# MaxInGaussian/SCFGP

Measured on AMD Instinct MI355X. Metric: NLML+grad evals/sec, higher is better.
Workload: dtype f32

## Files before the change

### scfgp_amd/csrc/api_ctx.h

```cpp
#pragma once
#include "../../include/scfgp_hip.h"
#include "kernels.h"
#include "api_host.h"

#include <dlfcn.h>
#if __has_include(<rccl/rccl.h>)
#include <rccl/rccl.h>
#else
extern "C" {
typedef struct ncclComm* ncclComm_t;
typedef struct { char internal[128]; } ncclUniqueId;
typedef enum { ncclSuccess = 0 } ncclResult_t;
typedef enum { ncclFloat64 = 8 } ncclDataType_t;
typedef enum { ncclSum = 0 } ncclRedOp_t;
ncclResult_t ncclGetUniqueId(ncclUniqueId*);
ncclResult_t ncclCommInitRank(ncclComm_t*, int, ncclUniqueId, int);
ncclResult_t ncclAllReduce(const void*, void*, size_t, ncclDataType_t, ncclRedOp_t, ncclComm_t, hipStream_t);
ncclResult_t ncclCommDestroy(ncclComm_t);
const char* ncclGetErrorString(ncclResult_t);
}
#endif

#include <algorithm>
#include <cmath>
#include <cstdlib>
#include <cstring>
#include <string>
#include <vector>

#define HIPCHK(ctx, call)                                                                           \
    do {                                                                                            \
        hipError_t e_ = (call);                                                                     \
        if (e_ != hipSuccess) {                                                                     \
            (ctx)->err = std::string(#call) + ": " + hipGetErrorString(e_);                         \
            return SCFGP_EHIP;                                                                      \
        }                                                                                           \
    } while (0)

static constexpr int XT = 128;
static constexpr int64_t PRED_ROWS = 32768;
#ifndef SCFGP_COND_THRESHOLD
#define SCFGP_COND_THRESHOLD 10.0
#endif
#ifndef SCFGP_COND_THRESHOLD_W
#define SCFGP_COND_THRESHOLD_W 1000.0
#endif
#ifndef SCFGP_ERR_PER_COND
#define SCFGP_ERR_PER_COND 3.0e-7
#endif

struct Roctx {
    int (*push)(const char*) = nullptr; int (*pop)() = nullptr;
    Roctx() {
        void* h = dlopen("librocprofiler-sdk-roctx.so", RTLD_LAZY | RTLD_LOCAL);
        if (!h) h = dlopen("libroctx64.so", RTLD_LAZY | RTLD_LOCAL);
        if (!h) return;
        push = (int (*)(const char*))dlsym(h, "roctxRangePushA");
        pop = (int (*)())dlsym(h, "roctxRangePop");
        if (!push || !pop) { push = nullptr; pop = nullptr; }
    }
};
inline Roctx& roctx() { static Roctx r; return r; }

struct ProfRec { std::string name; hipEvent_t e0, e1; };

struct scfgp_ctx {
    Geom g{};
    int dtype = 0, device = 0;
    hipStream_t st = nullptr; bool own_stream = false;
    hipStream_t copy_st = nullptr; hipEvent_t ev_factor = nullptr;
    int lowrank_bwd = -1; int Spp = 0, Sq = 0; bool last_lrb = false;
    bool want_lrb() const {
        const bool fits = g.lowrank && g.Jp + (int)round_up(g.S, 64) <= g.Kp;
        return fits && (lowrank_bwd == 1 || (lowrank_bwd < 0 && g.Dp >= 4 * g.Sp));
    }
    double* x3_scalars() { return d_x3 + (int64_t)Dpp * g.Jp; }
    double* xs1() { return d_xp1 + n_pk + g.Kp; }
    double* xs2() { return d_xp2 + n_pk + g.Kp; }
    bool unsettled = false; int test_deny_level = 0, test_fail_stage = 0, test_pd_group = 0, test_sobol_group = 0;
    int cap() const { return esc_denied > 0 ? esc_denied - 1 : 2; }
    double* x3_xu() { return d_x3 + (int64_t)Dpp * g.Jp + 8; }
    hipEvent_t ev_fence = nullptr;
    ncclComm_t comm = nullptr; int comm_ranks = 0, comm_rank = 0;
    double* h_pin = nullptr;
    int64_t Ncap = 0, Nglobal = 0, Nglobal_full = 0;
    bool have_params = false, have_data = false;
    int stage = 0, last_want_grad = 0;
    std::vector<double> h_params;
    double *d_params = nullptr, *d_F = nullptr, *d_Fall = nullptr, *d_Lall = nullptr, *d_Rall = nullptr; Scal* d_sc = nullptr;
    double *d_Tt = nullptr, *p_Tt = nullptr;
    double *d_Xraw = nullptr, *d_yraw = nullptr; int64_t Nstore = 0, store_cap = 0; bool work_full = false;
    int64_t* d_idx = nullptr; int64_t idx_cap = 0;
    double *d_Xt = nullptr, *d_y = nullptr, *d_p = nullptr, *d_q = nullptr, *d_mu = nullptr, *d_vpart = nullptr;
    void *d_Phi = nullptr, *d_V = nullptr;
    bool split16 = false; unsigned* d_Phi16 = nullptr; char* d_B16 = nullptr; float* d_f16scale = nullptr;
    unsigned* d_V16g = nullptr; unsigned* d_qV16g = nullptr; double* d_f16side = nullptr; float* d_f16tmp = nullptr;
    int f16gram = 1;
    bool f16_on() const { return split16 && dma() == 2; }
    int64_t f16_chunk() const {
        const int64_t top = gram_chunk > 0 ? 2 * gram_chunk : 8192, fill = g.Np * F16x3Kernels::gram_tiles(g) / 512 / 512 * 512;
        return std::max<int64_t>(std::min(top, fill), 1024);
    }
    bool f16_gram() const { return f16_on() && f16gram && !last_cform; }
    F16Operands f16ops() const { return F16Operands{d_Phi16, d_B16, d_f16scale, nullptr, d_f16tmp + 5}; }
    double *d_xp1 = nullptr, *d_xp2 = nullptr; int64_t n_xp = 0, n_pk = 0;
    double *d_x1 = nullptr, *d_x2 = nullptr, *d_x3 = nullptr; int64_t n_x1 = 0, n_x2 = 0, n_x3 = 0; int Dpp = 0;
    double *d_Li = nullptr, *d_B = nullptr, *d_T1 = nullptr, *d_T2 = nullptr, *d_Abar = nullptr;
    void *d_BT = nullptr, *d_AbarT = nullptr;
    int apply_dma = -1;
    double *d_vecs = nullptr;
    double *d_scalars = nullptr, *d_yy = nullptr; int* d_flag = nullptr;
    float* d_ws2 = nullptr;
    double *d_slabs = nullptr; size_t slabs_bytes = 0;
    double *d_partial = nullptr; int64_t n_partial = 0;
    double *d_work = nullptr, *d_grad = nullptr;
    int xs_mode = 0; double* d_xscale = nullptr;
    int ys_mode = 0; double* d_yscale = nullptr;
    double *p_Xt = nullptr, *p_vpart = nullptr, *p_mupart = nullptr; void *p_Phi = nullptr;
    int64_t p_rows = 0;
    void *p_FT = nullptr, *p_C = nullptr, *p_V = nullptr, *p_Li = nullptr;
    double *u_Li = nullptr, *u_S = nullptr, *u_Lm = nullptr, *u_Mi = nullptr, *u_Si = nullptr, *u_vec = nullptr, *u_acc = nullptr, *u_part = nullptr;
    double *u_y = nullptr, *u_r = nullptr, *u_slabs = nullptr; size_t u_slabs_bytes = 0;
    void* u_LiT = nullptr; float* u_ws2 = nullptr; int* u_flag = nullptr;
    double *l_y = nullptr, *l_r = nullptr, *l_rec = nullptr, *l_out = nullptr, *l_acc = nullptr; unsigned long long* l_bad = nullptr;
    double *f_out = nullptr, *f_w = nullptr;
    int opt_algo = -1; OptHyper opt_h{}; double *d_opt = nullptr, *d_tctr = nullptr, *d_hist = nullptr; int hist_cap = 0;
    hipGraph_t graph = nullptr; hipGraphExec_t gexec = nullptr; int64_t graph_N = -1; bool in_train = false, warm = false;
    int use_graph = 1;
    int gram_nsplit = 0, gram_taper = 1, xtz_nsplit = 0; int64_t gram_chunk = 4096;
    RowSplits splits{};
    int gram64 = 2, esc_level = 0, esc_denied = 0; double esc_thr = SCFGP_COND_THRESHOLD, escw_thr = SCFGP_COND_THRESHOLD_W; bool last_used64 = false;
    int last_level = 0; bool cond_valid = false;
    double cond[3] = {0, 0, 0};
    void* d_Phi64 = nullptr; int64_t phi64_cap = 0; RowSplits splits64{};
    int factor_form = -1; bool last_cform = false; void* d_C = nullptr; int64_t c_cap = 0;
    bool want_cform() const { return factor_form == 1 || (factor_form < 0 && level() >= 2); }
    int level() const { return dtype != SCFGP_F32 || gram64 == 0 ? 0 : (gram64 == 1 ? 1 : (gram64 == 3 ? 2 : esc_level)); }
    bool use64() const { return level() >= 1; }
    double cond_est() const { return cond[1] * cond[2]; }
    double alpha_err_fp32() const { return SCFGP_ERR_PER_COND * cond_est(); }
    int want_level(double est, double slack) const { return est > escw_thr * slack ? 2 : (est > esc_thr * slack ? 1 : 0); }
    bool roctx_on = false;
    bool prof = false; std::vector<ProfRec> recs; std::vector<hipEvent_t> pool; size_t pool_used = 0;
    std::string err;

    double* beta() { return d_vecs; }
    double* alpha() { return d_vecs + g.Kp; }
    int dma() const {
        const int auto_dma = g.K > 256 && g.Np >= 16384 ? (dtype == SCFGP_F32 && g.K >= 1024 && g.Np >= 65536 ? 2 : 1) : 0;
        return apply_dma < 0 ? auto_dma : apply_dma;
    }
    double* u() { return d_vecs + 2 * g.Kp; }
    double* ut() { return d_vecs + 3 * g.Kp; }
    double* alpha_pred() { return d_vecs + 4 * g.Kp; }
    size_t tsize() const { return dtype == SCFGP_F32 ? 4 : 8; }
    KStage kstage() {
        KStage k; k.K = g.K; k.Kp = g.Kp; k.A = d_x1; k.Li = d_Li; k.B = d_B; k.T1 = d_T1; k.T2 = d_T2;
        k.g = d_x1 + (int64_t)g.Kp * g.Kp; k.beta = beta(); k.alpha = alpha(); k.h = d_x2 + (int64_t)g.Kp * g.Kp;
        k.u = u(); k.ut = ut(); k.scalars = d_scalars; k.flag = d_flag;
        return k;
    }
};

struct ProfScope {
    scfgp_ctx* c; size_t idx = (size_t)-1; bool ranged = false;
    ProfScope(scfgp_ctx* c_, const char* name) : c(c_) {
        if (g_scfgp_capturing) return;
        if (c->roctx_on && roctx().push) { roctx().push(name); ranged = true; }
        if (!c->prof) return;
        auto get = [&]() {
            if (c->pool_used == c->pool.size()) { hipEvent_t e; hipEventCreate(&e); c->pool.push_back(e); }
            return c->pool[c->pool_used++];
        };
        ProfRec r; r.name = name; r.e0 = get(); r.e1 = get();
        hipEventRecord(r.e0, c->st);
        c->recs.push_back(r); idx = c->recs.size() - 1;
    }
    ~ProfScope() {
        if (idx != (size_t)-1) hipEventRecord(c->recs[idx].e1, c->st);
        if (ranged) roctx().pop();
    }
};

template <typename P> static int dmalloc(scfgp_ctx* c, P** p, size_t bytes) {
    HIPCHK(c, hipMalloc((void**)p, bytes ? bytes : 16));
    return SCFGP_OK;
}
template <typename P> static void dfree(P*& p) { if (p) { hipFree((void*)p); p = nullptr; } }
struct DevTmp {
    double* p = nullptr;
    ~DevTmp() { if (p) hipFree(p); }
    operator double*() const { return p; }
};

#define DISPATCH_TO(I, c, fn, ...) ((c)->dtype == SCFGP_F32 ? I<float>::fn(__VA_ARGS__) : I<double>::fn(__VA_ARGS__))
```

### scfgp_amd/csrc/apply.hip

```cpp
#include "kernels.h"
#include "tile_cfgs.h"

#include <algorithm>

#ifdef SCFGP_TRACE
constexpr int ATRACE_CAP = 1 << 16;
__device__ unsigned long long g_atrace[5 * ATRACE_CAP][5];
int64_t apply_trace_read(void* host, int64_t max_bytes) {
    const int64_t n = max_bytes < (int64_t)sizeof(g_atrace) ? max_bytes : (int64_t)sizeof(g_atrace);
    return hipMemcpyFromSymbol(host, HIP_SYMBOL(g_atrace), n) == hipSuccess ? n : -2;
}
#else
int64_t apply_trace_read(void*, int64_t) { return -1; }
#endif
template <typename T, int TILE> struct ApplyCfg {
    typedef TileCfg<T, Tune<T>::APPLY_BM, TILE, SCFGP_BK, Tune<T>::APPLY_WGM, Tune<T>::apply_wgn(TILE), Tune<T>::MS,
                    SCFGP_BK == 16 && Tune<T>::MS == 16> type;
};

#include "apply_epilogue.h"

template <class Cfg, int EPI>
__device__ __forceinline__ void apply_tile(
    const typename Cfg::T* __restrict__ Phi, const typename Cfg::T* __restrict__ Bm, typename Cfg::T* V,
    double* __restrict__ vpart, const double* __restrict__ p, const double* __restrict__ q, const double* __restrict__ y,
    const double* __restrict__ alpha, const double* __restrict__ ut, int K, int Kp, int64_t Np, int njt,
    int col0, int jt0, double* __restrict__ mu, int ntot, int jt, int64_t rb, char* smem_raw) {
    typedef typename Cfg::T T;
    T* smem = reinterpret_cast<T*>(smem_raw);
    const int cbase = col0 + jt * Cfg::BN;
    const bool want_mu = (EPI == 0 || EPI == 2 || EPI == 3) && mu != nullptr;
    const int nkt_all = (K + Cfg::BK - 1) / Cfg::BK;
    const int nkt_tri = (cbase + Cfg::BN + Cfg::BK - 1) / Cfg::BK;
    const int kt0 = EPI == 4 ? cbase / Cfg::BK : 0;
    const int nkt = ((EPI == 2 || EPI == 3) && nkt_tri < nkt_all ? nkt_tri : nkt_all) - kt0;
    typename Cfg::MTr::acc_t acc[Cfg::TM][Cfg::TN];
    acc_zero<Cfg>(acc);
    TrLoader<T, T, Cfg::BM, Cfg::BK, Cfg::LDA, Cfg::THREADS, EPI != 1 && EPI != 4, Cfg::SWZA> la(
        Phi + rb * Cfg::BM * Kp + kt0 * Cfg::BK, Kp, threadIdx.x, want_mu ? alpha : nullptr, jt0 + jt, ntot);
    if (EPI == 2 || EPI == 3) la.dot_range(cbase / Cfg::BK, nkt);
    else if (ntot == 0) {
        const int hi = (cbase + Cfg::BN) / Cfg::BK;
        la.dot_range(cbase / Cfg::BK, hi < nkt ? hi : nkt);
    }
    NatLoader<T, T, Cfg::BN, Cfg::BK, Cfg::LDB, Cfg::THREADS, false, false> lb(Bm + (int64_t)kt0 * Cfg::BK * Kp + cbase, Kp, threadIdx.x);
    tile_mainloop<Cfg>(la, lb, nkt, acc, smem);
    if constexpr (EPI != 1 && EPI != 4) { if (want_mu) la.dot_reduce(mu + (int64_t)(jt0 + jt) * Np + rb * Cfg::BM); }
    apply_epilogue<Cfg, EPI>(acc, Phi, V, vpart, p, q, y, alpha, ut, K, Kp, Np, rb, cbase, jt0 + jt, smem_raw);
}

template <class Cfg, int EPI>
__global__ __launch_bounds__(Cfg::THREADS) __attribute__((amdgpu_waves_per_eu(1, 8)))
void apply_kernel(
    const typename Cfg::T* __restrict__ Phi, const typename Cfg::T* __restrict__ Bm, typename Cfg::T* V,
    double* __restrict__ vpart, const double* __restrict__ p, const double* __restrict__ q, const double* __restrict__ y,
    const double* __restrict__ alpha, const double* __restrict__ ut, int K, int Kp, int64_t Np, int njt,
    int col0, int jt0, double* __restrict__ mu, int ntot) {
    SMEM_DECL;
    const unsigned wid = xcd_remap(blockIdx.x, gridDim.x);
    if constexpr (EPI == 3 || EPI == 4) {
        const int np = (njt + 1) / 2, t = (int)(wid % np), o = njt - 1 - t;
        const int64_t rb = wid / np;
        apply_tile<Cfg, EPI>(Phi, Bm, V, vpart, p, q, y, alpha, ut, K, Kp, Np, njt, col0, jt0, mu, ntot, t, rb, smem_raw);
        if (o != t) {
            __syncthreads();
            apply_tile<Cfg, EPI>(Phi, Bm, V, vpart, p, q, y, alpha, ut, K, Kp, Np, njt, col0, jt0, mu, ntot, o, rb, smem_raw);
        }
    } else
        apply_tile<Cfg, EPI>(Phi, Bm, V, vpart, p, q, y, alpha, ut, K, Kp, Np, njt, col0, jt0, mu, ntot, (int)(wid % njt), wid / njt, smem_raw);
}

typedef __attribute__((address_space(3))) void lds_void;
typedef const __attribute__((address_space(1))) void gbl_void;
template <typename T, int BN_>
struct ApplyDma {
    static constexpr int ES = (int)sizeof(T), BM = 256, BN = BN_, ROWB = 16 * ES, CPR = ROWB / 16;
    static constexpr int WN = ES == 4 ? 64 : 32;
    static constexpr int WAVES = 4 * (BN / WN), STAGE = (BM + BN) * ROWB, STAGES = 3, LDS_BYTES = STAGES * STAGE,
                         DMA_PER_WAVE = STAGE / 1024 / WAVES, ROWS_PER_DMA = 1024 / ROWB;
    static constexpr int PRE = 2;
    static constexpr int WAVES_PER_EU = WAVES == 4 ? 2 : 4;
    typedef TileCfg<T, BM, BN, 16, 4, BN / WN, 16, true> Cfg;
    static_assert(STAGE / 1024 % WAVES == 0 && LDS_BYTES <= 160 * 1024, "whole DMA instructions per wave; the ring fits the LDS");
    static __device__ __forceinline__ int swz(int x) {
        if constexpr (ES == 4) return (0x78 >> (2 * ((x >> 2) & 3))) & 3;
        else return (int)((0x6BEB08u >> (3 * ((x >> 1) & 7))) & 7);
    }
};
static_assert(((0x6BEB08u >> 0) & 7) == 0 && ((0x6BEB08u >> 3) & 7) == 1 && ((0x6BEB08u >> 6) & 7) == 4 && ((0x6BEB08u >> 9) & 7) == 5 &&
              ((0x6BEB08u >> 12) & 7) == 6 && ((0x6BEB08u >> 15) & 7) == 7 && ((0x6BEB08u >> 18) & 7) == 2 && ((0x6BEB08u >> 21) & 7) == 3,
              "fp64 swizzle table");

template <typename T, int EPI, int BN>
__global__ __launch_bounds__((64 * ApplyDma<T, BN>::WAVES)) __attribute__((amdgpu_waves_per_eu(ApplyDma<T, BN>::WAVES_PER_EU, ApplyDma<T, BN>::WAVES_PER_EU)))
void apply_dma_kernel(const T* __restrict__ Phi, const T* __restrict__ Bm, T* V,
                      double* __restrict__ vpart, const double* __restrict__ p, const double* __restrict__ q,
                      const double* __restrict__ y, const double* __restrict__ alpha, const double* __restrict__ ut,
                      int K, int Kp, int64_t Np, int njt, double* __restrict__ mu, int col0, int slot0, int64_t rb0) {
    typedef ApplyDma<T, BN> D;
    typedef typename D::Cfg Cfg;
    typedef T half_t __attribute__((ext_vector_type(2)));
    typedef std::integral_constant<int, 0> H0;
    typedef std::integral_constant<int, 1> H1;
    constexpr int DPW = D::DMA_PER_WAVE, NRD = Cfg::TM + Cfg::TN, NM = 2 * Cfg::TM * Cfg::TN, PRE = D::PRE;
    static_assert(Cfg::TM == 4 && (Cfg::TN == 4 || Cfg::TN == 2), "fragment lists of the wait statements");
    static_assert(PRE + DPW + NRD <= NM, "one fetch or read per MFMA behind the barrier");
    SMEM_DECL;
    char* smem = smem_raw;
#ifdef SCFGP_TRACE
    const unsigned long long tr_t0 = __builtin_amdgcn_s_memrealtime();
#endif
    const unsigned wid = xcd_remap(blockIdx.x, gridDim.x);
    const int jt = EPI == 3 || EPI == 4 ? (int)((wid % njt + wid / njt) % njt) : (int)(wid % njt);
    const int64_t rb = rb0 + wid / njt;
    const int cbase = col0 + jt * D::BN;
    const int lane = threadIdx.x & 63, wave = __builtin_amdgcn_readfirstlane(threadIdx.x >> 6);
    const char* src[DPW]; unsigned loff[DPW]; int dst[DPW];
#pragma unroll
    for (int u = 0; u < DPW; ++u) {
        const int t = wave * DPW + u, x0 = D::ROWS_PER_DMA * t, l = lane / D::CPR, c = (lane % D::CPR) ^ D::swz(x0 + l);
        const int xb = x0 - D::BM, xcol = (xb & ~(D::WN - 1)) + Cfg::TN * (xb & 15) + ((xb >> 4) & (Cfg::TN - 1));
        const T* rowp = x0 < D::BM ? Phi + (rb * D::BM + x0) * Kp : Bm + (int64_t)(cbase + xcol) * Kp;
        src[u] = reinterpret_cast<const char*>(rowp) + (EPI == 4 ? (cbase / 16) * D::ROWB : 0);
        loff[u] = (unsigned)((x0 < D::BM ? l : Cfg::TN * l) * Kp * D::ES + c * 16);
        dst[u] = t * 1024;
    }
    const auto fetch_one = [&](auto uc, int slot) {
        constexpr int u = decltype(uc)::value;
        __builtin_amdgcn_global_load_lds((gbl_void*)(src[u] + loff[u]), (lds_void*)(smem + slot * D::STAGE + dst[u]), 16, 0, 0);
        src[u] += D::ROWB;
    };
    const int i = lane & 15, qg = lane >> 4;
    const int wm0 = (wave / Cfg::WGN) * Cfg::WM, wn0 = (wave % Cfg::WGN) * Cfg::WN;
    const int hoff0 = sizeof(T) == 4 ? (((qg >> 1) ^ D::swz(i)) << 4) + 8 * (qg & 1) : ((2 * qg) ^ D::swz(i)) << 4;
    const int hoff1 = sizeof(T) == 4 ? (((2 + (qg >> 1)) ^ D::swz(i)) << 4) + 8 * (qg & 1) : ((2 * qg + 1) ^ D::swz(i)) << 4;
    const int ring = (int)(uintptr_t)smem, aoff = ring + (wm0 + i) * D::ROWB, boff = ring + D::BM * D::ROWB + (wn0 + i) * D::ROWB;
    const int ra[2] = {aoff + hoff0, aoff + hoff1}, rbb[2] = {boff + hoff0, boff + hoff1};
    half_t ha[2][Cfg::TM], hb[2][Cfg::TN];
    typename Cfg::MTr::acc_t acc[Cfg::TM][Cfg::TN];
    acc_zero<Cfg>(acc);
    const int nst_all = (K + 15) / 16, nst_tri = (cbase + D::BN + 15) / 16;
    const int nst = (EPI == 3 && nst_tri < nst_all ? nst_tri : nst_all) - (EPI == 4 ? cbase / 16 : 0);
#define SCFGP_LDS_READ(dst, addr, off)                                                                              \
    do {                                                                                                             \
        if constexpr (sizeof(T) == 4) asm volatile("ds_read_b64 %0, %1 offset:%2" : "=v"(dst) : "v"(addr), "n"(off));   \
        else asm volatile("ds_read_b128 %0, %1 offset:%2" : "=v"(dst) : "v"(addr), "n"(off));                           \
    } while (0)
    const auto read_one = [&](auto hc, auto rc, int stage) {
        constexpr int h = decltype(hc)::value, R = decltype(rc)::value;
        if constexpr (R < Cfg::TM) SCFGP_LDS_READ(ha[h][R], stage + ra[h], R * 16 * D::ROWB);
        else SCFGP_LDS_READ(hb[h][R - Cfg::TM], stage + rbb[h], (R - Cfg::TM) * 16 * D::ROWB);
    };
#undef SCFGP_LDS_READ
#define SCFGP_WAIT_FRAGS(what, h)                                                                                                   \
    do {                                                                                                                            \
        if constexpr (Cfg::TN == 4)                                                                                                 \
            asm volatile("s_waitcnt " what : "+v"(ha[h][0]), "+v"(ha[h][1]), "+v"(ha[h][2]), "+v"(ha[h][3]),                        \
                                             "+v"(hb[h][0]), "+v"(hb[h][1]), "+v"(hb[h][2]), "+v"(hb[h][3]) :: "memory");           \
        else                                                                                                                        \
            asm volatile("s_waitcnt " what : "+v"(ha[h][0]), "+v"(ha[h][1]), "+v"(ha[h][2]), "+v"(ha[h][3]),                        \
                                             "+v"(hb[h][0]), "+v"(hb[h][1]) :: "memory");                                           \
    } while (0)
    const auto mfma_one = [&](auto hc, auto ic) {
        constexpr int h = decltype(hc)::value, I = decltype(ic)::value, j = I / (Cfg::TM * Cfg::TN), tm = I / Cfg::TN % Cfg::TM, tn = I % Cfg::TN;
        Cfg::MTr::mfma(acc[tm][tn], ha[h][tm][j], hb[h][tn][j]);
        __builtin_amdgcn_sched_barrier(0);
    };
    const auto second_half_pre = [&]() { static_for<PRE>([&](auto ic) { mfma_one(H1(), ic); }); };
    const auto second_half = [&](auto fc, int fslot, int next) {
        static_for<NM - PRE>([&](auto ic) {
            constexpr int I = decltype(ic)::value;
            mfma_one(H1(), std::integral_constant<int, I + PRE>());
            if constexpr (I < DPW) {
                if constexpr (decltype(fc)::value) { fetch_one(ic, fslot); __builtin_amdgcn_sched_barrier(0); }
            } else if constexpr (I - DPW < NRD) {
                read_one(H0(), std::integral_constant<int, I - DPW>(), next);
                __builtin_amdgcn_sched_barrier(0);
            }
        });
    };
    const auto first_half = [&](int next) {
        static_for<NM>([&](auto ic) {
            mfma_one(H0(), ic);
            if constexpr (decltype(ic)::value < NRD) { read_one(H1(), ic, next); __builtin_amdgcn_sched_barrier(0); }
        });
    };
    static_for<DPW>([&](auto uc) { fetch_one(uc, 0); });
    if (nst > 1) static_for<DPW>([&](auto uc) { fetch_one(uc, 1); });
    if (nst > 2) static_for<DPW>([&](auto uc) { fetch_one(uc, 2); });
    if (nst > 2) asm volatile("s_waitcnt vmcnt(%0)" :: "n"(2 * DPW) : "memory");
    else if (nst > 1) asm volatile("s_waitcnt vmcnt(%0)" :: "n"(DPW) : "memory");
    else asm volatile("s_waitcnt vmcnt(0)" ::: "memory");
    __builtin_amdgcn_s_barrier();
    asm volatile("" ::: "memory");
#ifdef SCFGP_TRACE
    const unsigned long long tr_l0 = __builtin_amdgcn_s_memrealtime();
#endif
    static_for<NRD>([&](auto rc) { read_one(H0(), rc, 0); });
    static_for<NRD>([&](auto rc) { read_one(H1(), rc, 0); });
    SCFGP_WAIT_FRAGS("lgkmcnt(0)", 0);
    __builtin_amdgcn_sched_barrier(0);
    static_for<NM>([&](auto ic) { mfma_one(H0(), ic); });
    int slot = 0, s = 0;
    for (; s + 3 < nst; ++s) {
        asm volatile("s_waitcnt vmcnt(%0)" :: "n"(DPW) : "memory");
        SCFGP_WAIT_FRAGS("lgkmcnt(0)", 1);
        __builtin_amdgcn_sched_barrier(0);
        second_half_pre();
        __builtin_amdgcn_s_barrier();
        asm volatile("" ::: "memory");
        const int fslot = slot;
        slot = slot == 2 ? 0 : slot + 1;
        __builtin_amdgcn_sched_barrier(0);
        second_half(std::true_type(), fslot, slot * D::STAGE);
        SCFGP_WAIT_FRAGS("lgkmcnt(0)", 0);
        __builtin_amdgcn_sched_barrier(0);
        first_half(slot * D::STAGE);
    }
    SCFGP_WAIT_FRAGS("lgkmcnt(0)", 1);
    for (; s + 1 < nst; ++s) {
        if (s + 2 < nst) asm volatile("s_waitcnt vmcnt(%0)" :: "n"(DPW) : "memory");
        else asm volatile("s_waitcnt vmcnt(0)" ::: "memory");
        SCFGP_WAIT_FRAGS("lgkmcnt(0)", 1);
        __builtin_amdgcn_sched_barrier(0);
        second_half_pre();
        __builtin_amdgcn_s_barrier();
        asm volatile("" ::: "memory");
        slot = slot == 2 ? 0 : slot + 1;
        __builtin_amdgcn_sched_barrier(0);
        second_half(std::false_type(), 0, slot * D::STAGE);
        SCFGP_WAIT_FRAGS("lgkmcnt(0)", 0);
        __builtin_amdgcn_sched_barrier(0);
        first_half(slot * D::STAGE);
    }
    SCFGP_WAIT_FRAGS("lgkmcnt(0)", 1);
    __builtin_amdgcn_sched_barrier(0);
    static_for<NM>([&](auto ic) { mfma_one(H1(), ic); });
#undef SCFGP_WAIT_FRAGS
    __syncthreads();
#ifdef SCFGP_TRACE
    const unsigned long long tr_l1 = __builtin_amdgcn_s_memrealtime();
#endif
    constexpr int SLOTS = BN >= 128 ? BN / 128 : 1;
    const int vslot = slot0 + SLOTS * jt;
    int tid = (int)threadIdx.x;
    asm volatile("" : "+v"(tid));
    apply_epilogue<Cfg, EPI, EPI == 0 || EPI == 3, true>(acc, Phi, V, vpart, p, q, y, alpha, ut, K, Kp, Np, rb, cbase, vslot, smem_raw, mu, tid);
    if (SLOTS == 2 && (EPI == 0 || EPI == 3) && tid < D::BM) {
        vpart[(int64_t)(vslot + 1) * Np + rb * D::BM + tid] = 0.0;
        if (mu) mu[(int64_t)(vslot + 1) * Np + rb * D::BM + tid] = 0.0;
    }
#ifdef SCFGP_TRACE
    __syncthreads();
    if (threadIdx.x == 0 && blockIdx.x < ATRACE_CAP) {
        unsigned long long* rec = g_atrace[EPI * ATRACE_CAP + blockIdx.x];
        rec[0] = tr_t0; rec[1] = __builtin_amdgcn_s_memrealtime();
        rec[2] = ((unsigned long long)__builtin_amdgcn_s_getreg((20 << 0) | (0 << 6) | (3 << 11)) & 0xF) | ((unsigned long long)jt << 8) |
                                  ((unsigned long long)nst << 20);
        rec[3] = tr_l0; rec[4] = tr_l1;
    }
#endif
}

template <typename T> struct ApplyPlan {
    static constexpr int NW = 2;
    int width[NW], count[NW], col0[NW], jt0[NW], total;
    explicit ApplyPlan(int K) {
        const int w[NW] = {128, 64};
        int col = 0, jt = 0;
        const bool small = K <= 256;
        for (int i = 0; i < NW; ++i) {
            width[i] = w[i];
            const bool last = i == NW - 1;
            count[i] = small && !last ? 0 : (last ? (K - col + w[i] - 1) / w[i] : (K - col) / w[i]);
            col0[i] = col; jt0[i] = jt;
            col += count[i] * w[i]; jt += count[i];
        }
        total = jt;
    }
};
bool F16x3Kernels::apply_runs(const Geom& g) { return ApplyPlan<float>(g.K).count[0] > 0; }
template <class Cfg, int EPI, typename T>
static int apply_launch_cfg(const Geom& g, int njt, int col0, int jt0, const T* Phi, const T* Bm, T* V, double* vpart,
                            const double* p, const double* q, const double* y, const double* alpha, const double* ut,
                            double* mu, int ntot, hipStream_t st) {
    if (njt <= 0) return 0;
    const int64_t nrb = g.Np / Cfg::BM;
    const int wgs_per_rb = EPI == 3 || EPI == 4 ? (njt + 1) / 2 : njt;
    allow_big_lds(apply_kernel<Cfg, EPI>, Cfg::LDS_BYTES);
    hipLaunchKernelGGL((apply_kernel<Cfg, EPI>), dim3((unsigned)(wgs_per_rb * nrb)), dim3(Cfg::THREADS), Cfg::LDS_BYTES, st,
                       Phi, Bm, V, vpart, p, q, y, alpha, ut, g.K, g.Kp, g.Np, njt, col0, jt0, mu, ntot);
    return (int)(njt * nrb);
}
template <typename T, int EPI, int BN>
static int apply_dma_launch(const Geom& g, int njt, int col0, int slot0, const T* Phi, const T* Bm, T* V, double* vpart,
                            const double* p, const double* q, const double* y, const double* alpha, const double* ut,
                            double* mu, hipStream_t st, int64_t rb0 = 0, int64_t nrb = -1) {
    typedef ApplyDma<T, BN> D;
    if (nrb < 0) nrb = g.Np / D::BM;
    if (njt <= 0 || nrb <= 0) return 0;
    allow_big_lds(apply_dma_kernel<T, EPI, BN>, D::LDS_BYTES);
    hipLaunchKernelGGL((apply_dma_kernel<T, EPI, BN>), dim3((unsigned)(njt * nrb)), dim3(64 * D::WAVES), D::LDS_BYTES, st,
                       Phi, Bm, V, vpart, p, q, y, alpha, ut, g.K, g.Kp, g.Np, njt, mu, col0, slot0, rb0);
    return (int)(njt * nrb);
}
static int apply_num_cus() {
    static int n = 0;
    if (n == 0) {
        int dev = 0; hipDeviceProp_t prop;
        if (hipGetDevice(&dev) == hipSuccess && hipGetDeviceProperties(&prop, dev) == hipSuccess) n = prop.multiProcessorCount;
        if (n <= 0) n = 256;
    }
    return n;
}
template <typename T, int EPI>
static int apply_launch(const Geom& g, const T* Phi, const T* Bm, T* V, double* vpart, const double* p, const double* q,
                        const double* y, const double* alpha, const double* ut, double* mu, hipStream_t st,
                        int dma = 0, const T* BmT = nullptr, const F16Operands* f16 = nullptr) {
    if (!BmT) BmT = Bm;
    const ApplyPlan<T> pl(g.K);
    int nb = 0;
    if constexpr (EPI != 2) {
        if (dma && pl.count[0] > 0) {
            int n256 = 0;
            const int64_t nrb = g.Np / 256;
            int64_t tail_rb = 0;
            if constexpr (sizeof(T) == 4) {
                n256 = dma == 2 ? pl.count[0] / 2 : 0;
                if (n256 > 0 && EPI != 3 && EPI != 4) {
                    const int64_t ncu = apply_num_cus(), tiles = nrb * n256, rem = tiles % ncu;
                    if (tiles > ncu && rem > 0 && 20 * rem <= 9 * ncu) tail_rb = (rem + n256 - 1) / n256;
                }
                if (f16 && (EPI == 0 || EPI == 1)) {
                    constexpr int E = EPI == 1 ? 1 : 0;
                    nb += F16x3Kernels::apply<E, 256>(g, n256, 0, 0, Phi, *f16, V, vpart, p, q, y, alpha, ut, mu, st, 0, nrb - tail_rb);
                    nb += F16x3Kernels::apply<E, 128>(g, pl.count[0] - 2 * n256, 256 * n256, 2 * n256, Phi, *f16, V, vpart, p, q, y, alpha, ut, mu, st, 0, nrb - tail_rb);
                    nb += F16x3Kernels::apply<E, 64>(g, pl.count[1], pl.col0[1], pl.jt0[1], Phi, *f16, V, vpart, p, q, y, alpha, ut, mu, st, 0, nrb - tail_rb);
                    if (tail_rb > 0) {
                        nb += F16x3Kernels::apply<E, 128>(g, pl.count[0], 0, 0, Phi, *f16, V, vpart, p, q, y, alpha, ut, mu, st, nrb - tail_rb, tail_rb);
                        nb += F16x3Kernels::apply<E, 64>(g, pl.count[1], pl.col0[1], pl.jt0[1], Phi, *f16, V, vpart, p, q, y, alpha, ut, mu, st, nrb - tail_rb, tail_rb);
                    }
                    return nb;
                }
                nb += apply_dma_launch<T, EPI, 256>(g, n256, 0, 0, Phi, BmT, V, vpart, p, q, y, alpha, ut, mu, st, 0, nrb - tail_rb);
            }
            nb += apply_dma_launch<T, EPI, 128>(g, pl.count[0] - 2 * n256, 256 * n256, 2 * n256, Phi, BmT, V, vpart, p, q, y, alpha, ut, mu, st, 0, nrb - tail_rb);
            nb += apply_dma_launch<T, EPI, 64>(g, pl.count[1], pl.col0[1], pl.jt0[1], Phi, BmT, V, vpart, p, q, y, alpha, ut, mu, st, 0, nrb - tail_rb);
            if (tail_rb > 0) {
                nb += apply_dma_launch<T, EPI, 128>(g, pl.count[0], 0, 0, Phi, BmT, V, vpart, p, q, y, alpha, ut, mu, st, nrb - tail_rb, tail_rb);
                nb += apply_dma_launch<T, EPI, 64>(g, pl.count[1], pl.col0[1], pl.jt0[1], Phi, BmT, V, vpart, p, q, y, alpha, ut, mu, st, nrb - tail_rb, tail_rb);
            }
            return nb;
        }
    }
    nb += apply_launch_cfg<typename ApplyCfg<T, 128>::type, EPI, T>(g, pl.count[0], pl.col0[0], pl.jt0[0], Phi, Bm, V, vpart, p, q, y, alpha, ut, mu, pl.total, st);
    nb += apply_launch_cfg<typename ApplyCfg<T, 64>::type, EPI, T>(g, pl.count[1], pl.col0[1], pl.jt0[1], Phi, Bm, V, vpart, p, q, y, alpha, ut, mu, pl.total, st);
    return nb;
}

template <typename T>
void ApplyKernels<T>::apply_v(const Geom& g, const T* Phi, const T* Bm, T* V, double* vpart, const double* alpha, double* mu,
                              hipStream_t st, int dma, const F16Operands* f16) {
    apply_launch<T, 0>(g, Phi, Bm, V, vpart, nullptr, nullptr, nullptr, alpha, nullptr, mu, st, dma, nullptr, f16);
}
template <typename T>
void ApplyKernels<T>::apply_predict(const Geom& g, const T* Phi, const T* LiT, double* vpart, const double* alpha, double* mu,
                                    hipStream_t st) {
    apply_launch<T, 2>(g, Phi, LiT, (T*)nullptr, vpart, nullptr, nullptr, nullptr, alpha, nullptr, mu, st);
}
template <typename T>
void ApplyKernels<T>::apply_plain(const Geom& g, const T* A, const T* Bm, T* Out, int Kc, int ncols, hipStream_t st) {
    Geom gk = g; gk.K = Kc;
    apply_launch_cfg<typename ApplyCfg<T, 64>::type, 4, T>(gk, (ncols + 63) / 64, 0, 0, A, Bm, Out, nullptr, nullptr, nullptr, nullptr, nullptr,
                                                           nullptr, nullptr, ApplyPlan<T>(Kc).total, st);
}

template <typename T>
void ApplyKernels<T>::apply_c(const Geom& g, const T* Phi, const T* LiT, const T* Li, T* C, double* vpart, const double* alpha,
                              const double* beta, double* mu, hipStream_t st, int dma) {
    const bool by_dma = dma && ApplyPlan<T>(g.K).count[0] > 0;
    apply_launch<T, 3>(g, Phi, LiT, C, vpart, nullptr, nullptr, nullptr, by_dma ? beta : alpha, nullptr, mu, st, dma, Li);
}
template <typename T>
void ApplyKernels<T>::apply_vc(const Geom& g, const T* C, const T* Li, const T* LiT, T* V, hipStream_t st, int dma) {
    apply_launch<T, 4>(g, C, Li, V, nullptr, nullptr, nullptr, nullptr, nullptr, nullptr, nullptr, st, dma, LiT);
}
template <typename T>
void ApplyKernels<T>::apply_phibar(const Geom& g, const T* Phi, const T* Abar, T* V, const double* p, const double* q,
                                   const double* y, const double* alpha, const double* ut, hipStream_t st, int dma, const F16Operands* f16) {
    apply_launch<T, 1>(g, Phi, Abar, V, nullptr, p, q, y, alpha, ut, nullptr, st, dma, nullptr, f16);
}

template <typename T> static int apply_njt(const Geom& g) { return ApplyPlan<T>(g.K).total; }


template <int MODE>
__global__ __launch_bounds__(256) void rowstats_kernel(const double* __restrict__ mupart, const double* __restrict__ vpart, int njt,
                                                       const double* __restrict__ y, const Scal* __restrict__ sc,
                                                       double* __restrict__ o1, double* __restrict__ o2,
                                                       double* __restrict__ partial, int64_t N, int64_t Np) {
    __shared__ double red[4][256];
    const double kappa = sc->kappa;
    double t2 = 0, kb = 0, qv = 0, pm = 0;
    for (int64_t n = (int64_t)blockIdx.x * 256 + threadIdx.x; n < Np; n += (int64_t)gridDim.x * 256) {
        double v = 0, mu = 0;
        for (int t = 0; t < njt; ++t) { v += vpart[(int64_t)t * Np + n]; mu += mupart[(int64_t)t * Np + n]; }
        const double d = kappa * (v + 1.0);
        if (MODE == 0) {
            double pn = 0, qn = 0;
            if (n < N) {
                const double r = mu - y[n];
                const double rv = r * r + v;
                const double e = 1.0 / d - rv / (d * d);
                pn = 2.0 * r / d;
                qn = 1.0 / d + kappa * e;
                t2 += rv / d + log(2.0 * M_PI * d);
                kb += e * (v + 1.0);
                qv += qn * v; pm += pn * mu;
            }
            o1[n] = pn; o2[n] = qn;
        } else if (n < N) {
            o1[n] = mu; o2[n] = sqrt(d);
        }
    }
    if (MODE == 0) {
        red[0][threadIdx.x] = t2; red[1][threadIdx.x] = kb; red[2][threadIdx.x] = qv; red[3][threadIdx.x] = pm;
        __syncthreads();
        for (int w = 128; w >= 1; w >>= 1) {
            if ((int)threadIdx.x < w)
                for (int k = 0; k < 4; ++k) red[k][threadIdx.x] += red[k][threadIdx.x + w];
            __syncthreads();
        }
        if (threadIdx.x < 4) partial[blockIdx.x * 4 + threadIdx.x] = red[threadIdx.x][0];
    }
}

template <typename T>
void ApplyKernels<T>::rowstats(const Geom& g, const double* mupart, const double* vpart, const double* y,
                               const Scal* sc, double* p, double* q, double* partial, int nblocks, hipStream_t st) {
    hipLaunchKernelGGL((rowstats_kernel<0>), dim3(nblocks), dim3(256), 0, st, mupart, vpart, apply_njt<T>(g), y, sc, p, q,
                       partial, g.N, g.Np);
}

template <typename T>
void ApplyKernels<T>::rowpredict(const Geom& g, const double* mupart, const double* vpart, const Scal* sc, double* mu, double* sd,
                                 hipStream_t st) {
    const int nblocks = (int)((g.Np + 255) / 256 < 1024 ? (g.Np + 255) / 256 : 1024);
    hipLaunchKernelGGL((rowstats_kernel<1>), dim3(nblocks), dim3(256), 0, st, mupart, vpart, apply_njt<T>(g),
                       (const double*)nullptr, sc, mu, sd, (double*)nullptr, g.N, g.Np);
}
template <typename T> int ApplyKernels<T>::partials(const Geom& g) { return apply_njt<T>(g); }
__global__ __launch_bounds__(256) void rowresidual_kernel(const double* __restrict__ mupart, int njt, const double* __restrict__ y,
                                                          double* __restrict__ r, int64_t N, int64_t Np) {
    for (int64_t n = (int64_t)blockIdx.x * 256 + threadIdx.x; n < Np; n += (int64_t)gridDim.x * 256) {
        double mu = 0;
        for (int t = 0; t < njt; ++t) mu += mupart[(int64_t)t * Np + n];
        r[n] = n < N ? y[n] - mu : 0.0;
    }
}
template <typename T>
void ApplyKernels<T>::rowresidual(const Geom& g, const double* mupart, const double* y, double* r, hipStream_t st) {
    const int nblocks = (int)((g.Np + 255) / 256 < 1024 ? (g.Np + 255) / 256 : 1024);
    hipLaunchKernelGGL(rowresidual_kernel, dim3(nblocks), dim3(256), 0, st, mupart, apply_njt<T>(g), y, r, g.N, g.Np);
}
template struct ApplyKernels<double>;
template struct ApplyKernels<float>;

__global__ __launch_bounds__(256) void reduce_scalars_kernel(const double* __restrict__ partial, int nblocks, int width,
                                                             double* __restrict__ scalars, int slot0) {
    __shared__ double red[256];
    for (int k = 0; k < width; ++k) {
        double s = 0;
        for (int b = threadIdx.x; b < nblocks; b += 256) s += partial[(int64_t)b * width + k];
        red[threadIdx.x] = s;
        __syncthreads();
        for (int m = 128; m >= 1; m >>= 1) {
            if (threadIdx.x < m) red[threadIdx.x] += red[threadIdx.x + m];
            __syncthreads();
        }
        if (threadIdx.x == 0) scalars[slot0 + k] = red[0];
        __syncthreads();
    }
}
__global__ __launch_bounds__(256) void reduce_chunks_kernel(double* __restrict__ partial, int n, int chunk) {
    __shared__ double red[256];
    const int64_t b0 = (int64_t)blockIdx.x * chunk;
    const int len = b0 + chunk <= n ? chunk : (int)(n - b0);
    double s = 0;
    for (int b = threadIdx.x; b < len; b += 256) s += partial[b0 + b];
    red[threadIdx.x] = s;
    __syncthreads();
    for (int m = 128; m >= 1; m >>= 1) {
        if (threadIdx.x < m) red[threadIdx.x] += red[threadIdx.x + m];
        __syncthreads();
    }
    if (threadIdx.x == 0 && len > 0) partial[b0] = red[0];
}
__global__ __launch_bounds__(128) void reduce_strided_kernel(const double* __restrict__ partial, int nchunks, int chunk,
                                                             double* __restrict__ scalars, int slot0) {
    __shared__ double red[128];
    red[threadIdx.x] = (int)threadIdx.x < nchunks ? partial[(int64_t)threadIdx.x * chunk] : 0.0;
    __syncthreads();
    for (int m = 64; m >= 1; m >>= 1) {
        if ((int)threadIdx.x < m) red[threadIdx.x] += red[threadIdx.x + m];
        __syncthreads();
    }
    if (threadIdx.x == 0) scalars[slot0] = red[0];
}
void reduce_scalars(double* partial, int nblocks, int width, double* scalars, int slot0, hipStream_t st) {
    if (width == 1 && nblocks > 8192) {
        const int chunk = (nblocks + 127) / 128, nchunks = (nblocks + chunk - 1) / chunk;
        hipLaunchKernelGGL(reduce_chunks_kernel, dim3(nchunks), dim3(256), 0, st, partial, nblocks, chunk);
        hipLaunchKernelGGL(reduce_strided_kernel, dim3(1), dim3(128), 0, st, partial, nchunks, chunk, scalars, slot0);
        return;
    }
    hipLaunchKernelGGL(reduce_scalars_kernel, dim3(1), dim3(256), 0, st, partial, nblocks, width, scalars, slot0);
}

__global__ __launch_bounds__(256) void sumsq_kernel(const double* __restrict__ y, int64_t n, double* __restrict__ partial) {
    __shared__ double red[256];
    double s = 0;
    for (int64_t i = (int64_t)blockIdx.x * 256 + threadIdx.x; i < n; i += (int64_t)gridDim.x * 256) s += y[i] * y[i];
    red[threadIdx.x] = s;
    __syncthreads();
    for (int m = 128; m >= 1; m >>= 1) {
        if (threadIdx.x < m) red[threadIdx.x] += red[threadIdx.x + m];
        __syncthreads();
    }
    if (threadIdx.x == 0) partial[blockIdx.x] = red[0];
}
void sum_squares(const double* y, int64_t n, double* scalars, int slot, double* scratch, hipStream_t st) {
    const int nb = 256;
    hipLaunchKernelGGL(sumsq_kernel, dim3(nb), dim3(256), 0, st, y, n, scratch);
    reduce_scalars(scratch, nb, 1, scalars, slot, st);
}
```

### scfgp_amd/csrc/apply_epilogue.h

```cpp
#pragma once
#include "kernels.h"
#include "tile_cfgs.h"

template <int CTRL> __device__ __forceinline__ double dpp_mov_f64(double x) {
    int lo = __double2loint(x), hi = __double2hiint(x);
    lo = __builtin_amdgcn_update_dpp(0, lo, CTRL, 0xF, 0xF, true);
    hi = __builtin_amdgcn_update_dpp(0, hi, CTRL, 0xF, 0xF, true);
    return __hiloint2double(hi, lo);
}
__device__ __forceinline__ double row16_sum(double x) {
    x += dpp_mov_f64<0xB1>(x);
    x += dpp_mov_f64<0x4E>(x);
    x += dpp_mov_f64<0x141>(x);
    x += dpp_mov_f64<0x140>(x);
    return x;
}
template <class Cfg, int EPI, bool MU>
__device__ __forceinline__ void apply_epilogue_vec2(
    const typename Cfg::MTr::acc_t (&acc)[Cfg::TM][Cfg::TN], const double* __restrict__ Phi, double* V,
    double* __restrict__ vpart, const double* __restrict__ p, const double* __restrict__ q, const double* __restrict__ y,
    const double* __restrict__ alpha, const double* __restrict__ ut, int K, int Kp, int64_t Np, int64_t rb, int cbase, int jtg,
    char* smem_raw, double* __restrict__ mupart, int tid) {
    static_assert(Cfg::TN == 2 && Cfg::MS == 16 && sizeof(typename Cfg::T) == 8 && (EPI == 0 || EPI == 1 || EPI == 3 || EPI == 4), "VEC2 layout");
    AccCoord<Cfg> co(tid);
    const int jg = cbase + co.wn0 + 2 * (co.lane & 15);
    if constexpr (EPI == 4) {
#pragma unroll
        for (int tm = 0; tm < Cfg::TM; ++tm)
#pragma unroll
            for (int r = 0; r < 4; ++r)
                *reinterpret_cast<v2d*>(V + (rb * Cfg::BM + co.row(tm, r)) * Kp + jg) = v2d{acc[tm][0][r], acc[tm][1][r]};
    } else if constexpr (EPI == 0 || EPI == 3) {
        double* red = reinterpret_cast<double*>(smem_raw);
        double* red2 = red + Cfg::WGN * Cfg::BM;
        const int wn = (tid >> 6) % Cfg::WGN;
        double al[2], live[2];
#pragma unroll
        for (int k = 0; k < 2; ++k) { live[k] = jg + k < K ? 1.0 : 0.0; al[k] = MU && jg + k < K ? alpha[jg + k] : 0.0; }
#pragma unroll
        for (int tm = 0; tm < Cfg::TM; ++tm) {
            v2d ph[4];
            int64_t off[4];
#pragma unroll
            for (int r = 0; r < 4; ++r) {
                off[r] = (rb * Cfg::BM + co.row(tm, r)) * Kp + jg;
                if (EPI == 0) ph[r] = *reinterpret_cast<const v2d*>(Phi + off[r]);
            }
#pragma unroll
            for (int r = 0; r < 4; ++r) {
                const int row = co.row(tm, r);
                const double c0 = acc[tm][0][r], c1 = acc[tm][1][r];
                *reinterpret_cast<v2d*>(V + off[r]) = v2d{c0, c1};
                double part, mup = 0;
                if (EPI == 3) part = fma(c0, c0, c1 * c1);
                else part = fma(ph[r][0] * live[0], c0, ph[r][1] * live[1] * c1);
                if (MU) mup = EPI == 3 ? fma(c0, al[0], c1 * al[1]) : fma(ph[r][0], al[0], ph[r][1] * al[1]);
                part = row16_sum(part);
                if ((co.lane & 15) == 0) red[wn * Cfg::BM + row] = part;
                if (MU) {
                    mup = row16_sum(mup);
                    if ((co.lane & 15) == 0) red2[wn * Cfg::BM + row] = mup;
                }
            }
        }
        __syncthreads();
        if (tid < Cfg::BM) {
            double s = 0, s2 = 0;
#pragma unroll
            for (int k = 0; k < Cfg::WGN; ++k) { s += red[k * Cfg::BM + tid]; if (MU) s2 += red2[k * Cfg::BM + tid]; }
            vpart[(int64_t)jtg * Np + rb * Cfg::BM + tid] = s;
            if (MU && mupart) mupart[(int64_t)jtg * Np + rb * Cfg::BM + tid] = s2;
        }
    } else {
        double al[2], u2[2];
#pragma unroll
        for (int k = 0; k < 2; ++k) { al[k] = alpha[jg + k]; u2[k] = ut[jg + k]; }
        double* rowsc = reinterpret_cast<double*>(smem_raw);
        for (int i = tid; i < Cfg::BM; i += Cfg::THREADS) {
            const int64_t n = rb * Cfg::BM + i;
            rowsc[3 * i] = 2.0 * q[n]; rowsc[3 * i + 1] = p[n]; rowsc[3 * i + 2] = y[n];
        }
        __syncthreads();
#pragma unroll
        for (int tm = 0; tm < Cfg::TM; ++tm) {
            v2d vv[4];
            int64_t off[4];
#pragma unroll
            for (int r = 0; r < 4; ++r) {
                off[r] = (rb * Cfg::BM + co.row(tm, r)) * Kp + jg;
                vv[r] = *reinterpret_cast<const v2d*>(V + off[r]);
            }
#pragma unroll
            for (int r = 0; r < 4; ++r) {
                const int row = co.row(tm, r);
                const double qn = rowsc[3 * row], pn = rowsc[3 * row + 1], yn = rowsc[3 * row + 2];
                v2d o;
#pragma unroll
                for (int k = 0; k < 2; ++k) o[k] = 2.0 * acc[tm][k][r] + qn * vv[r][k] + pn * al[k] + yn * u2[k];
                *reinterpret_cast<v2d*>(V + off[r]) = o;
            }
        }
    }
}
template <class Cfg, int EPI, bool MU = false, bool VEC4 = false>
__device__ __forceinline__ void apply_epilogue(
    const typename Cfg::MTr::acc_t (&acc)[Cfg::TM][Cfg::TN], const typename Cfg::T* __restrict__ Phi, typename Cfg::T* V,
    double* __restrict__ vpart, const double* __restrict__ p, const double* __restrict__ q, const double* __restrict__ y,
    const double* __restrict__ alpha, const double* __restrict__ ut, int K, int Kp, int64_t Np, int64_t rb, int cbase, int jtg,
    char* smem_raw, double* __restrict__ mupart = nullptr, int tid = (int)threadIdx.x) {
    typedef typename Cfg::T T;
    if constexpr (VEC4 && sizeof(T) == 8) {
        apply_epilogue_vec2<Cfg, EPI, MU>(acc, Phi, V, vpart, p, q, y, alpha, ut, K, Kp, Np, rb, cbase, jtg, smem_raw, mupart, tid);
        return;
    }
    AccCoord<Cfg> co(tid);
    if constexpr (VEC4 && sizeof(T) == 4) {
        static_assert(Cfg::TN == 4 && Cfg::MS == 16 && sizeof(T) == 4 && (EPI == 0 || EPI == 1 || EPI == 3 || EPI == 4), "VEC4 layout");
        const int c4 = co.wn0 + 4 * (co.lane & 15);
        const int jg = cbase + c4;
        if constexpr (EPI == 4) {
#pragma unroll
            for (int tm = 0; tm < Cfg::TM; ++tm)
#pragma unroll
                for (int r = 0; r < 4; ++r)
                    *reinterpret_cast<v4f*>(V + (rb * Cfg::BM + co.row(tm, r)) * Kp + jg) = v4f{acc[tm][0][r], acc[tm][1][r], acc[tm][2][r], acc[tm][3][r]};
        } else if constexpr (EPI == 0 || EPI == 3) {
            double* red = reinterpret_cast<double*>(smem_raw);
            double* red2 = red + Cfg::WGN * Cfg::BM;
            const int wn = (tid >> 6) % Cfg::WGN;
            double al[4], live[4];
#pragma unroll
            for (int k = 0; k < 4; ++k) { live[k] = jg + k < K ? 1.0 : 0.0; al[k] = MU && jg + k < K ? alpha[jg + k] : 0.0; }
#pragma unroll
            for (int tm = 0; tm < Cfg::TM; ++tm) {
                v4f ph[4];
                int64_t off[4];
#pragma unroll
                for (int r = 0; r < 4; ++r) {
                    off[r] = (rb * Cfg::BM + co.row(tm, r)) * Kp + jg;
                    if (EPI == 0) ph[r] = *reinterpret_cast<const v4f*>(Phi + off[r]);
                }
#pragma unroll
                for (int r = 0; r < 4; ++r) {
                    const int row = co.row(tm, r);
                    const v4f c = v4f{acc[tm][0][r], acc[tm][1][r], acc[tm][2][r], acc[tm][3][r]};
                    *reinterpret_cast<v4f*>(V + off[r]) = c;
                    double part = 0, mup = 0;
                    if (EPI == 3) {
                        part = (double)(c[0] * c[0]) + (double)(c[1] * c[1]) + (double)(c[2] * c[2]) + (double)(c[3] * c[3]);
                        if (MU) mup = (double)c[0] * al[0] + (double)c[1] * al[1] + (double)c[2] * al[2] + (double)c[3] * al[3];
                    } else {
#pragma unroll
                        for (int k = 0; k < 4; ++k) { part += (double)ph[r][k] * (double)c[k] * live[k]; if (MU) mup += (double)ph[r][k] * al[k]; }
                    }
                    part = row16_sum(part);
                    if ((co.lane & 15) == 0) red[wn * Cfg::BM + row] = part;
                    if (MU) {
                        mup = row16_sum(mup);
                        if ((co.lane & 15) == 0) red2[wn * Cfg::BM + row] = mup;
                    }
                }
            }
            __syncthreads();
            if (tid < Cfg::BM) {
                double s = 0, s2 = 0;
#pragma unroll
                for (int k = 0; k < Cfg::WGN; ++k) { s += red[k * Cfg::BM + tid]; if (MU) s2 += red2[k * Cfg::BM + tid]; }
                vpart[(int64_t)jtg * Np + rb * Cfg::BM + tid] = s;
                if (MU && mupart) mupart[(int64_t)jtg * Np + rb * Cfg::BM + tid] = s2;
            }
        } else {
            float alf[4], u4f[4];
#pragma unroll
            for (int k = 0; k < 4; ++k) { alf[k] = (float)alpha[jg + k]; u4f[k] = (float)ut[jg + k]; }
            float* rowsc = reinterpret_cast<float*>(smem_raw);
            for (int i = tid; i < Cfg::BM; i += Cfg::THREADS) {
                const int64_t n = rb * Cfg::BM + i;
                rowsc[3 * i] = (float)(2.0 * q[n]); rowsc[3 * i + 1] = (float)p[n]; rowsc[3 * i + 2] = (float)y[n];
            }
            __syncthreads();
#pragma unroll
            for (int tm = 0; tm < Cfg::TM; ++tm) {
                v4f vv[4];
                int64_t off[4];
#pragma unroll
                for (int r = 0; r < 4; ++r) {
                    off[r] = (rb * Cfg::BM + co.row(tm, r)) * Kp + jg;
                    vv[r] = *reinterpret_cast<const v4f*>(V + off[r]);
                }
#pragma unroll
                for (int r = 0; r < 4; ++r) {
                    const int row = co.row(tm, r);
                    const float qn = rowsc[3 * row], pn = rowsc[3 * row + 1], yn = rowsc[3 * row + 2];
                    v4f o;
#pragma unroll
                    for (int k = 0; k < 4; ++k) o[k] = fmaf(qn, vv[r][k], fmaf(pn, alf[k], fmaf(yn, u4f[k], 2.0f * acc[tm][k][r])));
                    *reinterpret_cast<v4f*>(V + off[r]) = o;
                }
            }
        }
        return;
    }
    if (EPI == 4) {
#pragma unroll
        for (int tm = 0; tm < Cfg::TM; ++tm)
#pragma unroll
            for (int r = 0; r < Cfg::MTr::NACC; ++r) {
                const int64_t off = (rb * Cfg::BM + co.row(tm, r)) * Kp + cbase;
#pragma unroll
                for (int tn = 0; tn < Cfg::TN; ++tn) V[off + co.col(tn)] = acc[tm][tn][r];
            }
    } else if (EPI == 0 || EPI == 2 || EPI == 3) {
        double* red = reinterpret_cast<double*>(smem_raw);
        double* red2 = red + Cfg::WGN * Cfg::BM;
        const int wn = (tid >> 6) % Cfg::WGN;
        double al[Cfg::TN];
        if (MU) {
#pragma unroll
            for (int tn = 0; tn < Cfg::TN; ++tn) al[tn] = cbase + co.col(tn) < K ? alpha[cbase + co.col(tn)] : 0.0;
        }
#pragma unroll
        for (int tm = 0; tm < Cfg::TM; ++tm)
#pragma unroll
            for (int r = 0; r < Cfg::MTr::NACC; ++r) {
                const int row = co.row(tm, r);
                const int64_t off = (rb * Cfg::BM + row) * Kp + cbase;
                double part = 0, mup = 0;
#pragma unroll
                for (int tn = 0; tn < Cfg::TN; ++tn) {
                    const T c = acc[tm][tn][r];
                    if (EPI != 2) V[off + co.col(tn)] = c;
                    if (EPI != 0) {
                        part += (double)c * (double)c;
                        if (MU && cbase + co.col(tn) < K) mup += (EPI == 3 ? (double)c : (double)Phi[off + co.col(tn)]) * al[tn];
                    } else if (cbase + co.col(tn) < K) {
                        const double ph = (double)Phi[off + co.col(tn)];
                        part += ph * (double)c;
                        if (MU) mup += ph * al[tn];
                    }
                }
                if constexpr (Cfg::MS == 16) part = row16_sum(part);
                else {
#pragma unroll
                    for (int m = 1; m < Cfg::MS; m <<= 1) part += __shfl_xor(part, m);
                }
                if ((co.lane % Cfg::MS) == 0) red[wn * Cfg::BM + row] = part;
                if (MU) {
                    if constexpr (Cfg::MS == 16) mup = row16_sum(mup);
                    else {
#pragma unroll
                        for (int m = 1; m < Cfg::MS; m <<= 1) mup += __shfl_xor(mup, m);
                    }
                    if ((co.lane % Cfg::MS) == 0) red2[wn * Cfg::BM + row] = mup;
                }
            }
        __syncthreads();
        if (tid < Cfg::BM) {
            double s = 0, s2 = 0;
#pragma unroll
            for (int k = 0; k < Cfg::WGN; ++k) { s += red[k * Cfg::BM + tid]; if (MU) s2 += red2[k * Cfg::BM + tid]; }
            vpart[(int64_t)jtg * Np + rb * Cfg::BM + tid] = s;
            if (MU && mupart) mupart[(int64_t)jtg * Np + rb * Cfg::BM + tid] = s2;
        }
    } else {
        [[maybe_unused]] float alf[Cfg::TN], utf[Cfg::TN];
        if constexpr (sizeof(T) == 4) {
#pragma unroll
            for (int tn = 0; tn < Cfg::TN; ++tn) { alf[tn] = (float)alpha[cbase + co.col(tn)]; utf[tn] = (float)ut[cbase + co.col(tn)]; }
        }
#pragma unroll
        for (int tm = 0; tm < Cfg::TM; ++tm)
#pragma unroll
            for (int r = 0; r < Cfg::MTr::NACC; ++r) {
                const int64_t n = rb * Cfg::BM + co.row(tm, r);
                const int64_t off = n * Kp + cbase;
                const double qn = 2.0 * q[n], pn = p[n], yn = y[n];
                if constexpr (sizeof(T) == 4) {
                    const float qf = (float)qn, pf = (float)pn, yf = (float)yn;
#pragma unroll
                    for (int tn = 0; tn < Cfg::TN; ++tn)
                        V[off + co.col(tn)] = fmaf(qf, V[off + co.col(tn)], fmaf(pf, alf[tn], fmaf(yf, utf[tn], 2.0f * acc[tm][tn][r])));
                } else {
#pragma unroll
                    for (int tn = 0; tn < Cfg::TN; ++tn) {
                        const int j = cbase + co.col(tn);
                        V[off + co.col(tn)] = (T)(2.0 * (double)acc[tm][tn][r] + qn * (double)V[off + co.col(tn)] + pn * alpha[j] + yn * ut[j]);
                    }
                }
            }
    }
}
```

### scfgp_amd/csrc/kernels.h

```cpp
#pragma once
#include "common.h"

struct Geom {
    int D, S, M, J, K, P;
    int Dp;
    int Jp;
    int Sp;
    int lowrank;
    int Kp;
    int tile;
    int gfull;
    int gstrip;
    int64_t N;
    int64_t Np;
};

struct RowSplits {
    int nsplit;
    int groups;
    int units;
    int taper;
    int gran;
    int64_t nrb;
    __host__ __device__ int per_group() const { return units + taper; }
    __host__ __device__ void range(int s, int64_t& r0, int64_t& r1) const {
        const int pg = per_group(), grp = s / pg, i = s % pg;
        const int64_t g0 = nrb * grp / groups, g1 = nrb * (grp + 1) / groups, len = g1 - g0;
        const int64_t den = (int64_t)1 << taper;
        const int k = i - (units - 1);
        int64_t e0, e1;
        if (taper == 0 || k < 0) { e0 = den * i; e1 = e0 + den; }
        else {
            const int64_t base = den * (units - 1);
            e0 = base + den - (den >> k);
            e1 = k == taper ? base + den : base + den - (den >> (k + 1));
        }
        r0 = (g0 + len * e0 / (den * units)) * gran;
        r1 = (g0 + len * e1 / (den * units)) * gran;
    }
};
RowSplits gram_row_splits(int jobs_per_split, int64_t Np, bool f32, int nsplit_override, int taper);

struct Projection { const double* Fall; const double* Lall; const double* Rall; double* Tt; };

template <typename T>
struct FmapKernels {
    static void featuremap(const Geom& g, const double* Xt, const Projection& pr, const Scal* sc, T* Phi, hipStream_t st);
    static void convert(const double* src, T* dst, int K, int Kp, hipStream_t st);
    static void convert_transposed(const double* src, T* dst, int K, int Kp, hipStream_t st);
};

template <typename T>
struct GramKernels {
    static void gram(const Geom& g, const T* Phi, const double* w, const double* side, const RowSplits& rs, int64_t chunk,
                     double* slabs, double* sidepart, int* qhead, float* ws2, hipStream_t st);
    static int gram_jobs(const Geom& g);
    static void xtz(const Geom& g, const double* Xt, const T* Phi, const T* Phibar, int nsplit, int64_t chunk, double* slabs,
                    hipStream_t st);
    static void zbar_inplace(const Geom& g, const T* Phi, T* Phibar, hipStream_t st);
    static void rsel(const Geom& g, const double* params, T* out, hipStream_t st);
    static void tn_plain(const double* A, int Dp, const T* Bm, int64_t ldb, int J, int64_t Np, int nsplit, int64_t chunk, double* slabs,
                         hipStream_t st);
};

struct F16Operands { const unsigned* Phi16; const char* B16; const float* scale; unsigned* V16; const float* vbound; };

template <typename T>
struct ApplyKernels {
    static void apply_v(const Geom& g, const T* Phi, const T* Bm, T* V, double* vpart, const double* alpha, double* mupart,
                        hipStream_t st, int dma = 0, const F16Operands* f16 = nullptr);
    static void apply_predict(const Geom& g, const T* Phi, const T* LiT, double* vpart, const double* alpha, double* mupart,
                              hipStream_t st);
    static void apply_c(const Geom& g, const T* Phi, const T* LiT, const T* Li, T* C, double* vpart, const double* alpha,
                        const double* beta, double* mupart, hipStream_t st, int dma = 0);
    static void apply_vc(const Geom& g, const T* C, const T* Li, const T* LiT, T* V, hipStream_t st, int dma = 0);
    static void apply_phibar(const Geom& g, const T* Phi, const T* Abar, T* V, const double* p, const double* q,
                             const double* y, const double* alpha, const double* ut, hipStream_t st, int dma = 0, const F16Operands* f16 = nullptr);
    static void apply_plain(const Geom& g, const T* A, const T* Bm, T* Out, int Kc, int ncols, hipStream_t st);
    static void rowstats(const Geom& g, const double* mupart, const double* vpart, const double* y,
                         const Scal* sc, double* p, double* q, double* partial, int nblocks, hipStream_t st);
    static void rowpredict(const Geom& g, const double* mupart, const double* vpart, const Scal* sc, double* mu, double* sd,
                           hipStream_t st);
    static void rowresidual(const Geom& g, const double* mupart, const double* y, double* r, hipStream_t st);
    static int partials(const Geom& g);
};

struct F16x3Kernels {
    static void split_operand(const Geom& g, const double* M, char* B16, float* scale, double* part, const Scal* sc, hipStream_t st);
    template <int EPI, int BN>
    static int apply(const Geom& g, int njt, int col0, int slot0, const float* Phi, const F16Operands& f, float* V,
                     double* vpart, const double* p, const double* q, const double* y, const double* alpha, const double* ut, double* mu,
                     hipStream_t st, int64_t rb0, int64_t nrb);
    static bool apply_runs(const Geom& g);
    static constexpr size_t F16_PAD = 1024;
    static int side_blocks(const Geom& g);
    static void split_phi(const Geom& g, const float* Phi, const double* y, const Scal* sc, unsigned* Phi16, double* sidepart, float* tmp,
                          hipStream_t st);
    static void v_bound(const Geom& g, const double* B, const Scal* sc, float* tmp, hipStream_t st);
    static void split_v(const Geom& g, const float* V, const double* q, const double* p, unsigned* V16g, unsigned* qV16g, double* sidepart,
                        float* tmp, hipStream_t st);
    static int gram_chunks(const Geom& g, int64_t chunk);
    static int gram_tiles(const Geom& g);
    static void gram(const Geom& g, const unsigned* A16g, const unsigned* B16g, const float* scale, int64_t chunk, double* slabs, hipStream_t st);
};

template <typename T> struct SweepKernels : FmapKernels<T>, GramKernels<T>, ApplyKernels<T> {};

int64_t trace_read(void* host, int64_t max_bytes);
int64_t apply_trace_read(void* host, int64_t max_bytes);
int64_t chol_trace_read(void* host, int64_t max_bytes);

void reduce_tri_tiles(const double* slabs, int nsplit, int nts, int tile, double* packed, hipStream_t st);
void unpack_tri_tiles(const double* packed, int nts, int tile, double* full, int64_t ld, hipStream_t st);
void reduce_full_tiles(const double* slabs, int nsplit, int ntm, int ntn, double* out, int64_t ldo, hipStream_t st);
void reduce_side(const double* sidepart, int nsplit, int Kp, int ncov, double* vec, hipStream_t st);
void reduce_scalars(double* partial, int nblocks, int width, double* scalars, int slot0, hipStream_t st);
void sum_squares(const double* y, int64_t n, double* scalars, int slot, double* scratch, hipStream_t st);

void unpack_params(const Geom& g, const double* params, double* F, double* Fall, double* Lall, double* Rall, Scal* sc, hipStream_t st);
void grad_epilogue(const Geom& g, const double* params, const double* F, const double* XZ, int64_t ldxz,
                   double* work, double* scalars, int64_t Nglobal, double* grad, hipStream_t st,
                   const double* TZ = nullptr, int64_t ldtz = 0, const double* XU = nullptr, int64_t ldxu = 0);
void finalize_cost(const Geom& g, const Scal* sc, double* scalars, const double* yy, const double* t2kb,
                   int64_t Nglobal, double* grad, int want_grad, hipStream_t st);
void write_status(double* xs, double ran1, double cap1, double cap2, double fail, hipStream_t st);
void pack_data(const Geom& g, const double* Xraw, const double* yraw, const int64_t* idx, double* Xt, double* y, hipStream_t st,
               int mode = 0, const double* sp = nullptr);
void pad_square(const double* src, int K, int Kp, double* dst, hipStream_t st);

constexpr int YPOST_BLOCKS = 64;
void ypost_mean(const double* ys, int64_t n, double* out, hipStream_t st);
void ypost_chunk(double* mu, double* sd, const double* ys, int64_t n, int mode, const double* sp, const double* ymean,
                 double* part, hipStream_t st);
void ypost_metrics(const double* part, int nparts, int64_t n, double* out, hipStream_t st);

int predgrad_ft_cols(int D);
template <typename T> void predgrad_operand(const Geom& g, const double* Fall, T* FT, hipStream_t st);
template <typename T>
void predgrad(const Geom& g, const T* Phi, const T* V, const double* alpha, const T* FT, const double* sd, const Scal* sc, double* dmu,
              double* dstd, hipStream_t st);
void xgrad_chunk(const double* Xraw, int64_t n, int D, int mode, const double* sp, double* dmu, double* dstd, hipStream_t st);
void ygrad_chunk(const double* mu, const double* sd, int64_t n, int D, int mode, const double* sp, double* dmu, double* dstd, hipStream_t st);

inline int64_t sample_w_rows(int K) { return round_up(K, 64); }
inline int sample_w_cols(int nsamp) { return (int)round_up(nsamp, 64); }
template <typename T>
void sample_weights(const Geom& g, const double* Li, const double* alpha, const Scal* sc, int nsamp, uint64_t seed, double* Z, double* W,
                    T* Wt, hipStream_t st);
template <typename T>
void sample_product(const Geom& g, const T* Phi, const T* Wt, int nsamp, int64_t t0, uint64_t seed, int noise, int ymode, const double* ysp,
                    const Scal* sc, double* out, hipStream_t st);
constexpr int sample_block_rows(size_t tsize) { return tsize == 4 ? 128 : 64; }
inline int64_t sample_blocks(int64_t Np, size_t tsize) { return Np / sample_block_rows(tsize); }
struct SampleArgmaxBufs { double* pv; long long* pt; double* bestv; long long* bestt; int* flag; };
template <typename T>
void sample_argmax_product(const Geom& g, const T* Phi, const T* Wt, int nsamp, const double* w, int minimize, int64_t t0, int first,
                           const SampleArgmaxBufs& b, hipStream_t st);
void sample_argmax_finalize(double* bestv, int nsamp, int ymode, const double* ysp, const Scal* sc, hipStream_t st);

struct AcquireSpec { int kind; double par[2]; const double* fstar; int nstar; int noise; int minimize; };
inline int64_t acquire_blocks(int64_t Np) { return Np / 256; }
struct AcquireBufs { double* mu; double* sd; double* acq; double* au; double* as; double* pv; long long* pt; double* bestv; long long* bestt; int* flag; };
void acquire_rows(const Geom& g, int njt, const double* mupart, const double* vpart, const Scal* sc, const AcquireSpec& a, const AcquireBufs& b,
                  hipStream_t st);
void acquire_argmax(const Geom& g, const double* w, int64_t t0, int first, const AcquireBufs& b, hipStream_t st);
void acquire_grad(const Geom& g, const AcquireBufs& b, int minimize, const double* dsd, double* grad, hipStream_t st);

struct KgBufs { double *d, *zf, *sd, *st_m, *st_s, *st_b, *kg, *kg_hi, *m, *s; };
int64_t kg_state_rows();
void kg_reference(int njt, const double* mupart, int64_t Np, int64_t R, int minimize, const double* z, int J, double* d, double* zf, int* flag,
                  hipStream_t st);
void kg_sigma(const Geom& g, int njt, const double* vpart, const Scal* sc, int noise, double* sd, hipStream_t st);
template <typename T>
void kg_nodes(const Geom& g, const T* Ca, const T* Cb, int64_t R, int J, const KgBufs& b, const Scal* sc, hipStream_t st);

int samplegrad_w_ld(int K);
void samplegrad_weights(const double* W, int K, int nsamp, double* WT, hipStream_t st);
template <typename T>
void samplegrad(const Geom& g, const T* Phi, const double* WT, const double* sidx, int64_t t0, int nsamp, const T* FT, double* val,
                double* grad, hipStream_t st);

template <typename T>
void predcov(const Geom& g, const T* Ca, const T* Cb, int64_t nrows, int64_t Tb, int64_t row_base, int noise, const Scal* sc, double* out,
             hipStream_t st);

struct OptHyper { double lr, b1, b2, eps, momentum; };
void opt_update(int algo, const OptHyper& h, int P, double* theta, const double* grad, double* st, double* tctr,
                const double* scalars, double* hist, int hist_cap, hipStream_t stream);

struct KStage {
    int K, Kp;
    double *A;
    double *Li;
    double *B;
    double *T1, *T2;
    double *g, *beta, *alpha, *h, *u, *ut;
    double *scalars; int* flag;
};
void kstage_factor(const KStage& k, const double* packed, const Scal* sc, hipStream_t st);
void kstage_adjoint(const KStage& k, const double* BWB, double* Abar, const Scal* sc, hipStream_t st);
void kstage_adjoint_factor_form(const KStage& k, double* McBWB, double* Abar, const Scal* sc, hipStream_t st);
void kstage_bbar(const KStage& k, const double* packed, const double* Abar, double* part, hipStream_t st);

struct KUpdate {
    int K, Kp;
    const double* packed;
    int64_t n_pk;
    const double* Li;
    const double* alpha;
    double *S;
    double *Lm, *Mi, *Si;
    double *gamma, *alpha_out, *part;
    int* flag;
};
void kstage_update(const KUpdate& k, hipStream_t st);
void kstage_downdate(const KUpdate& k, const double* rr, double n, const Scal* sc, double* out, hipStream_t st);
void update_sumsq(const double* r, int64_t n, double* acc, hipStream_t st);
void forget_stats(const double* mu, const double* sd, const double* y, int64_t n, int64_t ldr, double* rec, double* acc, hipStream_t st);
void update_load_factor(const double* Li_host_layout, int K, int Kp, double* Li, hipStream_t st);
void update_store_factor(const double* Li, int K, int Kp, double* Li_host_layout, hipStream_t st);
void update_check_finite(const double* x, int64_t n, int* flag, hipStream_t st);
void update_accumulate(double* acc, const double* part, int64_t n, hipStream_t st);

template <typename T>
void loo_blocks(const Geom& g, const T* C, const double* r, const double* y, int block, int64_t blk0, const Scal* sc, double* mu,
                double* sd, double* lev, double* rec, double* acc, unsigned long long* bad, hipStream_t st);

template <typename T> void gradcov_operand(const Geom& g, const double* params, const double* Fall, T* Qt, hipStream_t st);
template <typename T> void gradfeat(const Geom& gr, const Geom& g, const T* Phi, const T* Qt, T* Psi, hipStream_t st);
void gradcov_ones(double* x, int64_t n, hipStream_t st);
template <typename T>
void gradcov_blocks(const Geom& gr, const Geom& g, const T* C, const double* params, const Scal* sc, const double* gfac, const double* m,
                    const double* wgt, double* dvar, double* dcov, double* rec, hipStream_t st);
void gradcov_reduce(const double* rec, int64_t n, int D, double* acc, hipStream_t st);

struct GradObs { const int* dims; int nd; const double *gfac, *y, *G, *rho; };
template <typename T>
void gradobs_rows(const Geom& gr, const Geom& g, const T* Phi, const double* Fall, const GradObs& a, T* Psi, double* tg, hipStream_t st);

constexpr int SOBOL_T = 8;
constexpr int SOBOL_COLS = 32;
constexpr int SOBOL_GROUP = 16;
void sobol_tables(const Geom& g, const double* Fall, const Scal* sc, const double* meas, int Jt, double* psi1, double* Ed, double* E,
                  double* Eb, double* phibar, hipStream_t st);
void sobol_weights(const Geom& g, const double* W, const Scal* sc, const double* E, int Jt, int nw, double* A, double* f0, hipStream_t st);
void sobol_pairs(const Geom& g, const double* Fall, const double* meas, const double* psi1, const double* Ed, const double* E,
                 const double* Eb, const double* A, const int* units, int nunits, int Jt, int nw, int w0, int ncols, int G, int flags,
                 double* rec, hipStream_t st);
void sobol_reduce(const double* rec, int nunits, int D, int ncols, int nw, int w0, int flags, double* sums, hipStream_t st);

inline int pd_grid_rows(int G) { return (int)round_up(G, 128); }
int64_t pd_record_len(const Geom& g, int ng);
template <typename T>
void pd_sums(const Geom& g, const double* Xt, const double* Fall, const Scal* sc, const double* wgt, const int* dims, int ng, double* rec,
             double* acc, hipStream_t st);
void pd_grid(double* grid, const int* dims, int ndim, int G, int D, int mode, const double* sp, hipStream_t st);
template <typename T>
void pd_mean_rows(const Geom& gr, const Geom& g, const double* acc, double W, const double* Fall, const int* dims, const double* grid, int ng,
                  int G, T* Phibar, hipStream_t st);
template <typename T>
void pd_ice_weights(const Geom& g, const double* alpha, const double* Fall, int d, const double* grid_d, int G, T* R, hipStream_t st);
void pd_column(const Geom& g, double* Xt, int d, int save, double* keep, hipStream_t st);

struct SelectBufs {
    int Kp; int64_t Trows;
    double *w, *d, *pval; long long* pidx;
    double *U, *cp, *a, *part;
    long long* idx; double *var, *gain; int* flag;
};
int select_partials(int64_t Trows);
void select_ones(double* w, int64_t Trows, hipStream_t st);
template <typename T> void select_init(const SelectBufs& b, const T* C, hipStream_t st);
template <typename T> void select_step(const SelectBufs& b, const T* C, int j, const Scal* sc, hipStream_t st);
void select_std(const SelectBufs& b, const Scal* sc, double* sd, hipStream_t st);

struct SelectIvBufs {
    const double* Q;
    double *a, *apart, *h, *v, *red, *ivar;
};
int select_iv_tiles(int Kp);
template <typename T>
void select_iv_init(const SelectBufs& b, const SelectIvBufs& iv, const T* C, const T* Qt, int K, const Scal* sc, hipStream_t st);
template <typename T> void select_iv_step(const SelectBufs& b, const SelectIvBufs& iv, const T* C, int j, const Scal* sc, hipStream_t st);

struct SelectQeiBufs {
    const double* F; int64_t T; int nsamp; double sgn;
    double *w, *ms, *score0, *pval; long long* pidx;
    long long* idx; double *gain, *qei; int* flag;
};
int selectqei_blocks(int64_t T);
void selectqei_state(const SelectQeiBufs& b, const double* pend, double base, int start, hipStream_t st);
void selectqei_sweep(const SelectQeiBufs& b, int j, hipStream_t st);
void selectqei_commit(const SelectQeiBufs& b, int j, hipStream_t st);
```

### scfgp_amd/csrc/scfgp_api.hip

```cpp
#include "api_ctx.h"

static void derive_geom(Geom& g, int D, int S, int M);

thread_local bool g_scfgp_capturing = false;

struct Rccl {
    void* h = nullptr;
    decltype(&ncclGetUniqueId) get_id = nullptr; decltype(&ncclCommInitRank) init_rank = nullptr;
    decltype(&ncclAllReduce) all_reduce = nullptr; decltype(&ncclCommDestroy) destroy = nullptr;
    decltype(&ncclGetErrorString) err_string = nullptr;
    bool resolved = false;
    bool bind(void* from) {
        get_id = (decltype(get_id))dlsym(from, "ncclGetUniqueId"); init_rank = (decltype(init_rank))dlsym(from, "ncclCommInitRank");
        all_reduce = (decltype(all_reduce))dlsym(from, "ncclAllReduce"); destroy = (decltype(destroy))dlsym(from, "ncclCommDestroy");
        err_string = (decltype(err_string))dlsym(from, "ncclGetErrorString");
        return get_id && init_rank && all_reduce && destroy && err_string;
    }
    Rccl() {
        if (dlsym(RTLD_DEFAULT, "ncclAllReduce") && bind(RTLD_DEFAULT)) { resolved = true; return; }
        const char* names[] = {"librccl.so", "librccl.so.1", "/opt/rocm/lib/librccl.so.1"};
        for (const char* n : names) if (!h) h = dlopen(n, RTLD_NOW | RTLD_NOLOAD | RTLD_LOCAL);
        for (const char* n : names) if (!h) h = dlopen(n, RTLD_NOW | RTLD_LOCAL);
        if (!h) return;
        if (bind(h)) resolved = true;
        else { dlclose(h); h = nullptr; }
    }
    bool ok() const { return resolved; }
};
static Rccl& rccl() { static Rccl r; return r; }

static int xtz_split(int ntiles, int64_t Np) {
    int64_t s = std::max(1, 512 / ntiles);
    int64_t smax = std::max<int64_t>(Np / 2048, 1);
    if (ntiles * smax < 256) smax = std::max<int64_t>(Np / 64, 1);
    if (s > smax) s = smax;
    if (s < 1) s = 1;
    return (int)s;
}

static void free_rows(scfgp_ctx* c) {
    dfree(c->d_Xt); dfree(c->d_y); dfree(c->d_p); dfree(c->d_q); dfree(c->d_ws2); dfree(c->d_mu); dfree(c->d_vpart); dfree(c->d_Tt);
    dfree(c->d_Phi); dfree(c->d_V); dfree(c->d_Phi16); dfree(c->d_V16g); dfree(c->d_qV16g); dfree(c->d_f16side); dfree(c->d_slabs);
    c->Ncap = 0; c->slabs_bytes = 0;
}

static int ensure_aux_rows(scfgp_ctx* c) {
    const Geom& g = c->g;
    if (c->use64() && c->phi64_cap < g.Np) {
        dfree(c->d_Phi64); c->phi64_cap = 0;
        if (int rc = dmalloc(c, &c->d_Phi64, sizeof(double) * g.Np * g.Kp)) return rc;
        HIPCHK(c, hipMemsetAsync(c->d_Phi64, 0, sizeof(double) * g.Np * g.Kp, c->st));
        c->phi64_cap = g.Np;
    }
    if (c->want_cform() && c->c_cap < g.Np) {
        dfree(c->d_C); c->c_cap = 0;
        if (int rc = dmalloc(c, &c->d_C, c->tsize() * g.Np * g.Kp)) return rc;
        HIPCHK(c, hipMemsetAsync(c->d_C, 0, c->tsize() * g.Np * g.Kp, c->st));
        c->c_cap = g.Np;
    }
    return SCFGP_OK;
}

static int ensure_rows(scfgp_ctx* c, int64_t N) {
    Geom& g = c->g;
    if (c->gexec) { hipGraphExecDestroy(c->gexec); c->gexec = nullptr; }
    if (c->graph) { hipGraphDestroy(c->graph); c->graph = nullptr; }
    const int64_t Np = round_up(N > 0 ? N : 1, 256);
    g.N = N; g.Np = Np;
    const int nts = g.Kp / g.tile, ntiles = nts * (nts + 1) / 2;
    const int ntx = ((g.Dp + XT - 1) / XT) * (g.Jp / XT);
    const int gjobs = c->dtype == SCFGP_F32 ? SweepKernels<float>::gram_jobs(g) : SweepKernels<double>::gram_jobs(g);
    c->splits = gram_row_splits(gjobs, Np, c->dtype == SCFGP_F32, c->gram_nsplit, c->gram_taper);
    int gs = c->splits.nsplit;
    if (c->dtype == SCFGP_F32 && c->gram64 != 0) {
        c->splits64 = gram_row_splits(SweepKernels<double>::gram_jobs(g), Np, false, c->gram_nsplit, c->gram_taper);
        gs = std::max(gs, c->splits64.nsplit);
    }
    const int xs = c->xtz_nsplit > 0 ? (int)std::min<int64_t>(c->xtz_nsplit, Np / 64) : xtz_split(ntx, Np);
    const int nt1 = (c->Spp / XT) * (g.Jp / XT), nt2 = (c->Dpp / XT) * (c->Sq / XT);
    const size_t lrb = std::max<size_t>((size_t)xtz_split(nt1, Np) * nt1, (size_t)xtz_split(nt2, Np) * nt2);
    if (c->split16) gs = std::max(gs, F16x3Kernels::gram_chunks(g, c->f16_chunk()));
    const size_t need = sizeof(double) * std::max<size_t>((size_t)gs * ntiles * g.tile * g.tile + (size_t)gs * g.Kp,
                                                          std::max<size_t>((size_t)xs * ntx, lrb) * XT * XT);
    if (need > c->slabs_bytes) {
        dfree(c->d_slabs);
        if (int rc = dmalloc(c, &c->d_slabs, need)) return rc;
        c->slabs_bytes = need;
    }
    if (int rc = ensure_aux_rows(c)) return rc;
    if (Np <= c->Ncap) return SCFGP_OK;
    dfree(c->d_Xt); dfree(c->d_y); dfree(c->d_p); dfree(c->d_q); dfree(c->d_ws2); dfree(c->d_mu); dfree(c->d_vpart); dfree(c->d_Tt);
    dfree(c->d_Phi); dfree(c->d_V); dfree(c->d_Phi16); dfree(c->d_V16g); dfree(c->d_qV16g); dfree(c->d_f16side);
    c->Ncap = 0;
    const size_t ts = c->tsize();
    int rc;
    if ((rc = dmalloc(c, &c->d_Xt, sizeof(double) * Np * g.Dp))) return rc;
    if (g.lowrank && (rc = dmalloc(c, &c->d_Tt, sizeof(double) * Np * g.Sp))) return rc;
    if ((rc = dmalloc(c, &c->d_y, sizeof(double) * Np))) return rc;
    if ((rc = dmalloc(c, &c->d_p, sizeof(double) * Np))) return rc;
    if ((rc = dmalloc(c, &c->d_q, sizeof(double) * Np))) return rc;
    if (c->dtype == SCFGP_F32 && (rc = dmalloc(c, &c->d_ws2, sizeof(float) * 2 * (Np + 32)))) return rc;
    if ((rc = dmalloc(c, &c->d_mu, sizeof(double) * Np * (g.Kp / 64)))) return rc;
    if ((rc = dmalloc(c, &c->d_vpart, sizeof(double) * Np * (g.Kp / 64)))) return rc;
    if ((rc = dmalloc(c, &c->d_Phi, ts * Np * g.Kp))) return rc;
    if ((rc = dmalloc(c, &c->d_V, ts * Np * g.Kp))) return rc;
    if (c->split16) {
        const size_t plane = sizeof(unsigned) * Np * g.Kp + F16x3Kernels::F16_PAD;
        if ((rc = dmalloc(c, &c->d_Phi16, plane)) || (rc = dmalloc(c, &c->d_V16g, plane)) || (rc = dmalloc(c, &c->d_qV16g, plane))) return rc;
        if ((rc = dmalloc(c, &c->d_f16side, sizeof(double) * F16x3Kernels::side_blocks(g) * g.Kp))) return rc;
        HIPCHK(c, hipMemsetAsync(c->d_Phi16, 0, plane, c->st));
        HIPCHK(c, hipMemsetAsync(c->d_V16g, 0, plane, c->st));
        HIPCHK(c, hipMemsetAsync(c->d_qV16g, 0, plane, c->st));
    }
    HIPCHK(c, hipMemsetAsync(c->d_Phi, 0, ts * Np * g.Kp, c->st));
    HIPCHK(c, hipMemsetAsync(c->d_V, 0, ts * Np * g.Kp, c->st));
    c->Ncap = Np;
    return SCFGP_OK;
}

extern "C" int scfgp_create(scfgp_ctx** out, int D, int S, int M, int dtype, int device, void* stream) {
    if (!out || D < 1 || S < 1 || M < 1 || (dtype != SCFGP_F64 && dtype != SCFGP_F32 && dtype != SCFGP_F16X3)) return SCFGP_EARG;
    scfgp_ctx* c = new scfgp_ctx();
    *out = c;
    c->split16 = dtype == SCFGP_F16X3;
    if (c->split16) dtype = SCFGP_F32;
    c->dtype = dtype; c->device = device;
    Geom& g = c->g;
    derive_geom(g, D, S, M);
    if (const char* e = getenv("SCFGP_LOWRANK")) g.lowrank = atoi(e) != 0;
    if (const char* e = getenv("SCFGP_ROCTX")) c->roctx_on = atoi(e) != 0;
    c->Dpp = (int)round_up(g.Dp, XT);
    HIPCHK(c, hipSetDevice(device));
    if (stream) c->st = (hipStream_t)stream;
    else { HIPCHK(c, hipStreamCreate(&c->st)); c->own_stream = true; }
    HIPCHK(c, hipStreamCreateWithFlags(&c->copy_st, hipStreamNonBlocking));
    HIPCHK(c, hipEventCreateWithFlags(&c->ev_factor, hipEventDisableTiming));
    HIPCHK(c, hipEventCreateWithFlags(&c->ev_fence, hipEventDisableTiming));
    const int64_t Kp = g.Kp, K2 = Kp * Kp;
    c->Spp = (int)round_up(g.Sp, XT); c->Sq = (int)round_up(g.S, XT);
    c->n_x1 = K2 + Kp + 8; c->n_x2 = K2 + Kp + 8; c->n_x3 = (int64_t)std::max(c->Dpp, c->Spp) * g.Jp + 8 + (int64_t)c->Dpp * c->Sq;
    { const int64_t nts = Kp / g.tile; c->n_pk = nts * (nts + 1) / 2 * g.tile * g.tile; c->n_xp = c->n_pk + Kp + 8; }
    int rc;
    if ((rc = dmalloc(c, &c->d_params, sizeof(double) * g.P))) return rc;
    if ((rc = dmalloc(c, &c->d_F, sizeof(double) * D * M))) return rc;
    if ((rc = dmalloc(c, &c->d_Fall, sizeof(double) * g.Dp * g.Jp))) return rc;
    if ((rc = dmalloc(c, &c->d_Lall, sizeof(double) * g.Dp * round_up(g.Sp, 64)))) return rc;
    if ((rc = dmalloc(c, &c->d_Rall, sizeof(double) * g.Sp * g.Jp))) return rc;
    if ((rc = dmalloc(c, &c->d_sc, sizeof(Scal)))) return rc;
    if ((rc = dmalloc(c, &c->d_xp1, sizeof(double) * c->n_xp))) return rc;
    if ((rc = dmalloc(c, &c->d_xp2, sizeof(double) * c->n_xp))) return rc;
    HIPCHK(c, hipMemsetAsync(c->d_xp1, 0, sizeof(double) * c->n_xp, c->st));
    HIPCHK(c, hipMemsetAsync(c->d_xp2, 0, sizeof(double) * c->n_xp, c->st));
    if ((rc = dmalloc(c, &c->d_x1, sizeof(double) * c->n_x1))) return rc;
    if ((rc = dmalloc(c, &c->d_x2, sizeof(double) * c->n_x2))) return rc;
    if ((rc = dmalloc(c, &c->d_x3, sizeof(double) * c->n_x3))) return rc;
    if ((rc = dmalloc(c, &c->d_Li, sizeof(double) * K2))) return rc;
    if ((rc = dmalloc(c, &c->d_B, sizeof(double) * K2))) return rc;
    if ((rc = dmalloc(c, &c->d_T1, sizeof(double) * K2))) return rc;
    if ((rc = dmalloc(c, &c->d_T2, sizeof(double) * K2))) return rc;
    if ((rc = dmalloc(c, &c->d_Abar, sizeof(double) * K2))) return rc;
    if ((rc = dmalloc(c, &c->d_BT, c->tsize() * K2))) return rc;
    if ((rc = dmalloc(c, &c->d_AbarT, c->tsize() * K2))) return rc;
    if (c->split16) {
        if ((rc = dmalloc(c, &c->d_B16, 4 * (size_t)K2))) return rc;
        if ((rc = dmalloc(c, &c->d_f16scale, sizeof(float) * 4))) return rc;
        if ((rc = dmalloc(c, &c->d_f16tmp, sizeof(float) * 8))) return rc;
    }
    if ((rc = dmalloc(c, &c->d_vecs, sizeof(double) * 5 * Kp))) return rc;
    if ((rc = dmalloc(c, &c->d_scalars, sizeof(double) * 32))) return rc;
    if ((rc = dmalloc(c, &c->d_yy, sizeof(double) * 8))) return rc;
    if ((rc = dmalloc(c, &c->d_flag, sizeof(int) * 16))) return rc;
    c->n_partial = 16384;
    if ((rc = dmalloc(c, &c->d_partial, sizeof(double) * c->n_partial))) return rc;
    if ((rc = dmalloc(c, &c->d_work, sizeof(double) * (4 * D + 4 + (int64_t)D * M)))) return rc;
    if ((rc = dmalloc(c, &c->d_grad, sizeof(double) * g.P))) return rc;
    HIPCHK(c, hipMemsetAsync(c->d_x1, 0, sizeof(double) * c->n_x1, c->st));
    HIPCHK(c, hipMemsetAsync(c->d_x2, 0, sizeof(double) * c->n_x2, c->st));
    HIPCHK(c, hipMemsetAsync(c->d_x3, 0, sizeof(double) * c->n_x3, c->st));
    HIPCHK(c, hipMemsetAsync(c->d_Li, 0, sizeof(double) * K2, c->st));
    HIPCHK(c, hipMemsetAsync(c->d_vecs, 0, sizeof(double) * 5 * Kp, c->st));
    HIPCHK(c, hipMemsetAsync(c->d_scalars, 0, sizeof(double) * 32, c->st));
    HIPCHK(c, hipStreamSynchronize(c->st));
    return SCFGP_OK;
}

extern "C" void scfgp_destroy(scfgp_ctx* c) {
    if (!c) return;
    hipSetDevice(c->device);
    if (c->st) hipStreamSynchronize(c->st);
    free_rows(c);
    dfree(c->d_Phi64); dfree(c->d_C); dfree(c->d_Xraw); dfree(c->d_yraw); dfree(c->d_idx); dfree(c->d_xscale); dfree(c->d_yscale);
    dfree(c->d_params); dfree(c->d_F); dfree(c->d_Fall); dfree(c->d_Lall); dfree(c->d_Rall); dfree(c->d_sc); dfree(c->p_Tt);
    dfree(c->d_xp1); dfree(c->d_xp2); dfree(c->d_x1); dfree(c->d_x2); dfree(c->d_x3); dfree(c->d_Li); dfree(c->d_B); dfree(c->d_T1); dfree(c->d_T2);
    dfree(c->d_Abar); dfree(c->d_BT); dfree(c->d_AbarT); dfree(c->d_B16); dfree(c->d_f16scale); dfree(c->d_f16tmp); dfree(c->d_vecs); dfree(c->d_scalars); dfree(c->d_yy);
    dfree(c->d_flag); dfree(c->d_partial); dfree(c->d_work); dfree(c->d_grad);
    dfree(c->p_Xt); dfree(c->p_vpart); dfree(c->p_mupart); dfree(c->p_Phi);
    dfree(c->p_FT); dfree(c->p_C); dfree(c->p_V); dfree(c->p_Li);
    dfree(c->u_Li); dfree(c->u_S); dfree(c->u_Lm); dfree(c->u_Mi); dfree(c->u_Si); dfree(c->u_vec); dfree(c->u_acc); dfree(c->u_part);
    dfree(c->u_y); dfree(c->u_r); dfree(c->u_slabs); dfree(c->u_LiT); dfree(c->u_ws2); dfree(c->u_flag);
    dfree(c->l_y); dfree(c->l_r); dfree(c->l_rec); dfree(c->l_out); dfree(c->l_acc); dfree(c->l_bad);
    dfree(c->f_out); dfree(c->f_w);
    if (c->gexec) hipGraphExecDestroy(c->gexec);
    if (c->graph) hipGraphDestroy(c->graph);
    dfree(c->d_opt); dfree(c->d_tctr); dfree(c->d_hist);
    for (hipEvent_t e : c->pool) hipEventDestroy(e);
    if (c->copy_st) { hipStreamSynchronize(c->copy_st); hipStreamDestroy(c->copy_st); }
    if (c->comm && rccl().ok()) rccl().destroy(c->comm);
    if (c->ev_factor) hipEventDestroy(c->ev_factor);
    if (c->ev_fence) hipEventDestroy(c->ev_fence);
    if (c->h_pin) hipHostFree(c->h_pin);
    if (c->own_stream && c->st) hipStreamDestroy(c->st);
    delete c;
}

extern "C" const char* scfgp_last_error(const scfgp_ctx* c) { return c ? c->err.c_str() : "null context"; }

extern "C" int scfgp_set_params(scfgp_ctx* c, const double* params, int P) {
    if (!c || !params || P != c->g.P) { if (c) c->err = "set_params: wrong parameter count"; return SCFGP_EARG; }
    HIPCHK(c, hipSetDevice(c->device));
    c->h_params.assign(params, params + P);
    HIPCHK(c, hipMemcpyAsync(c->d_params, c->h_params.data(), sizeof(double) * P, hipMemcpyHostToDevice, c->st));
    unpack_params(c->g, c->d_params, c->d_F, c->d_Fall, c->d_Lall, c->d_Rall, c->d_sc, c->st);
    HIPCHK(c, hipGetLastError());
    c->have_params = true; c->cond_valid = false;
    return SCFGP_OK;
}

extern "C" int scfgp_get_params(scfgp_ctx* c, double* params, int P) {
    if (!c || !params || P != c->g.P || !c->have_params) return SCFGP_EARG;
    memcpy(params, c->h_params.data(), sizeof(double) * P);
    return SCFGP_OK;
}

static int load_working_set(scfgp_ctx* c, const int64_t* d_idx, int64_t n, int64_t n_global) {
    if (int rc = ensure_rows(c, n)) return rc;
    c->Nglobal = n_global > 0 ? n_global : n;
    pack_data(c->g, c->d_Xraw, c->d_yraw, d_idx, c->d_Xt, c->d_y, c->st);
    sum_squares(c->d_y, c->g.Np, c->d_yy, 0, c->d_partial, c->st);
    HIPCHK(c, hipGetLastError());
    c->work_full = d_idx == nullptr;
    c->have_data = true; c->stage = 0; c->cond_valid = false; c->esc_denied = 0;
    return SCFGP_OK;
}

extern "C" int scfgp_set_data(scfgp_ctx* c, const double* X, const double* y, int64_t N, int64_t n_global) {
    if (!c || !X || !y || N < 1) { if (c) c->err = "set_data: bad arguments"; return SCFGP_EARG; }
    HIPCHK(c, hipSetDevice(c->device));
    if (N > c->store_cap) {
        HIPCHK(c, hipStreamSynchronize(c->st));
        dfree(c->d_Xraw); dfree(c->d_yraw); c->store_cap = 0;
        if (int rc = dmalloc(c, &c->d_Xraw, sizeof(double) * N * c->g.D)) return rc;
        if (int rc = dmalloc(c, &c->d_yraw, sizeof(double) * N)) return rc;
        c->store_cap = N;
    }
    c->Nstore = N; c->Nglobal_full = n_global > 0 ? n_global : N;
    HIPCHK(c, hipMemcpyAsync(c->d_Xraw, X, sizeof(double) * N * c->g.D, hipMemcpyHostToDevice, c->st));
    HIPCHK(c, hipMemcpyAsync(c->d_yraw, y, sizeof(double) * N, hipMemcpyHostToDevice, c->st));
    if (int rc = load_working_set(c, nullptr, N, n_global)) return rc;
    HIPCHK(c, hipStreamSynchronize(c->st));
    return SCFGP_OK;
}

static void unpack_exchange(scfgp_ctx* c, const double* xp, double* x) {
    const Geom& g = c->g;
    unpack_tri_tiles(xp, g.Kp / g.tile, g.tile, x, g.Kp, c->st);
    hipMemcpyAsync(x + (int64_t)g.Kp * g.Kp, xp + c->n_pk, sizeof(double) * (g.Kp + 8), hipMemcpyDeviceToDevice, c->st);
}

template <typename T> struct Impl {
    typedef SweepKernels<T> SK;
    static void gram_to(scfgp_ctx* c, const T* Mx, const double* w, const double* side, double* out, const char* name) {
        const Geom& g = c->g;
        const int nts = g.Kp / g.tile, ntiles = nts * (nts + 1) / 2;
        if constexpr (sizeof(T) == 4) {
            if (c->f16_gram()) {
                const int nch = F16x3Kernels::gram_chunks(g, c->f16_chunk());
                { ProfScope ps(c, w ? "split_v" : "split_phi");
                  if (w) F16x3Kernels::split_v(g, (const float*)Mx, w, side, F16x3Kernels::apply_runs(g) ? nullptr : c->d_V16g, c->d_qV16g,
                                               c->d_f16side, c->d_f16tmp, c->st);
                  else F16x3Kernels::split_phi(g, (const float*)Mx, side, c->d_sc, c->d_Phi16, c->d_f16side, c->d_f16tmp, c->st); }
                { ProfScope ps(c, name);
                  F16x3Kernels::gram(g, w ? c->d_V16g : c->d_Phi16, w ? c->d_qV16g : c->d_Phi16, c->d_f16tmp + 4, c->f16_chunk(), c->d_slabs, c->st); }
                { ProfScope ps(c, "reduce_tiles"); reduce_tri_tiles(c->d_slabs, nch, nts, g.tile, out, c->st);
                  reduce_side(c->d_f16side, F16x3Kernels::side_blocks(g), g.Kp, g.gfull * g.tile + g.gstrip * 64, out + c->n_pk, c->st); }
                return;
            }
        }
        const int gs = c->splits.nsplit;
        double* sidepart = c->d_slabs + (size_t)gs * ntiles * g.tile * g.tile;
        { ProfScope ps(c, name);
          SK::gram(g, Mx, w, side, c->splits, c->dtype == SCFGP_F32 ? c->gram_chunk : 0, c->d_slabs, sidepart, c->d_flag + 8, c->d_ws2, c->st); }
        { ProfScope ps(c, "reduce_tiles"); reduce_tri_tiles(c->d_slabs, gs, nts, g.tile, out, c->st);
          reduce_side(sidepart, gs, g.Kp, g.gfull * g.tile + g.gstrip * 64, out + c->n_pk, c->st); }
    }
    static int pass1(scfgp_ctx* c) {
        const Geom& g = c->g;
        if (!c->in_train) HIPCHK(c, hipMemsetAsync(c->d_flag, 0, sizeof(int) * 4, c->st));
        const bool use64 = sizeof(T) == 4 && c->use64();
        c->last_cform = c->want_cform();
        if ((use64 && c->phi64_cap < g.Np) || (c->last_cform && c->c_cap < g.Np)) {
            c->err = "pass1: auxiliary row buffer missing"; return SCFGP_EARG;
        }
        const Projection proj{c->d_Fall, c->d_Lall, c->d_Rall, c->d_Tt};
        if constexpr (sizeof(T) == 4) {
            if (use64) {
                typedef SweepKernels<double> SK64;
                const int nts = g.Kp / g.tile, ntiles = nts * (nts + 1) / 2, gs = c->splits64.nsplit;
                double* sidepart = c->d_slabs + (size_t)gs * ntiles * g.tile * g.tile;
                { ProfScope ps(c, "featuremap64"); SK64::featuremap(g, c->d_Xt, proj, c->d_sc, (double*)c->d_Phi64, c->st); }
                { ProfScope ps(c, "gram64");
                  SK64::gram(g, (const double*)c->d_Phi64, nullptr, c->d_y, c->splits64, 0, c->d_slabs, sidepart, c->d_flag + 8, nullptr, c->st); }
                { ProfScope ps(c, "reduce_tiles"); reduce_tri_tiles(c->d_slabs, gs, nts, g.tile, c->d_xp1, c->st);
                  reduce_side(sidepart, gs, g.Kp, g.gfull * g.tile + g.gstrip * 64, c->d_xp1 + c->n_pk, c->st); }
            }
        }
        { ProfScope ps(c, "featuremap"); SK::featuremap(g, c->d_Xt, proj, c->d_sc, (T*)c->d_Phi, c->st); }
        if constexpr (sizeof(T) == 4) {
            if (c->f16_on() && (use64 || !c->f16_gram())) {
                ProfScope ps(c, "split_phi");
                F16x3Kernels::split_phi(g, (const float*)c->d_Phi, c->d_y, c->d_sc, c->d_Phi16, c->d_f16side, c->d_f16tmp, c->st);
            }
        }
        if (!use64) gram_to(c, (const T*)c->d_Phi, nullptr, c->d_y, c->d_xp1, "gram");
        c->last_used64 = use64 || sizeof(T) == 8; c->last_level = sizeof(T) == 8 ? 0 : c->level();
        HIPCHK(c, hipMemcpyAsync(c->xs1(), c->d_yy, sizeof(double), hipMemcpyDeviceToDevice, c->st));
        write_status(c->xs1(), c->last_level >= 1 ? 1.0 : 0.0, c->cap() < 1 ? 1.0 : 0.0, c->cap() < 2 ? 1.0 : 0.0, 0.0, c->st);
        HIPCHK(c, hipGetLastError());
        return SCFGP_OK;
    }
    static int factor(scfgp_ctx* c) {
        const Geom& g = c->g;
        { ProfScope ps(c, "kstage_factor");
          hipMemcpyAsync(c->d_x1 + (int64_t)g.Kp * g.Kp, c->d_xp1 + c->n_pk, sizeof(double) * (g.Kp + 8), hipMemcpyDeviceToDevice, c->st);
          kstage_factor(c->kstage(), c->d_xp1, c->d_sc, c->st); }
        if (c->last_cform) {
            SK::convert(c->d_Li, (T*)c->d_BT, g.K, g.Kp, c->st);
            SK::convert_transposed(c->d_Li, (T*)c->d_AbarT, g.K, g.Kp, c->st);
        } else {
            SK::convert(c->d_B, (T*)c->d_BT, g.K, g.Kp, c->st);
            if (c->f16_on()) {
                F16x3Kernels::split_operand(g, c->d_B, c->d_B16, c->d_f16scale, c->d_partial, c->d_sc, c->st);
                F16x3Kernels::v_bound(g, c->d_B, c->d_sc, c->d_f16tmp, c->st);
            }
        }
        HIPCHK(c, hipGetLastError());
        return SCFGP_OK;
    }
    static int pass2(scfgp_ctx* c, int want_grad) {
        const Geom& g = c->g;
        if (c->last_cform) {
            const int dma = c->dma() ? 1 : 0;
            { ProfScope ps(c, "apply_c");
              SK::apply_c(g, (const T*)c->d_Phi, (const T*)c->d_AbarT, (const T*)c->d_BT, (T*)c->d_C, c->d_vpart, c->alpha(), c->beta(), c->d_mu, c->st, dma); }
            { ProfScope ps(c, "apply_vc");
              SK::apply_vc(g, (const T*)c->d_C, (const T*)c->d_BT, (const T*)c->d_AbarT, (T*)c->d_V, c->st, dma); }
        } else {
            ProfScope ps(c, "apply_v");
            F16Operands f16 = c->f16ops();
            if (want_grad && c->f16_gram()) f16.V16 = c->d_V16g;
            SK::apply_v(g, (const T*)c->d_Phi, (const T*)c->d_BT, (T*)c->d_V, c->d_vpart, c->alpha(), c->d_mu, c->st, c->dma(), c->f16_on() ? &f16 : nullptr);
        }
        const int nb = (int)std::min<int64_t>(g.Np / 4, 2048);
        { ProfScope ps(c, "rowstats");
          SK::rowstats(g, c->d_mu, c->d_vpart, c->d_y, c->d_sc, c->d_p, c->d_q, c->d_partial, nb, c->st);
          reduce_scalars(c->d_partial, nb, 4, c->xs2(), 0, c->st);
          write_status(c->xs2(), 0.0, 0.0, 0.0, 0.0, c->st); }
        if (want_grad) {
            gram_to(c, c->last_cform ? (const T*)c->d_C : (const T*)c->d_V, c->d_q, c->d_p, c->d_xp2, "gram_w");
        }
        HIPCHK(c, hipGetLastError());
        return SCFGP_OK;
    }
    static int adjoint(scfgp_ctx* c) {
        const Geom& g = c->g;
        { ProfScope ps(c, "kstage_adjoint"); unpack_exchange(c, c->d_xp2, c->d_x2);
          if (c->last_cform) kstage_adjoint_factor_form(c->kstage(), c->d_x2, c->d_Abar, c->d_sc, c->st);
          else kstage_adjoint(c->kstage(), c->d_x2, c->d_Abar, c->d_sc, c->st);
          kstage_bbar(c->kstage(), c->d_xp1, c->d_Abar, c->d_partial, c->st); }
        SK::convert(c->d_Abar, (T*)c->d_AbarT, g.K, g.Kp, c->st);
        if (c->f16_on()) F16x3Kernels::split_operand(g, c->d_Abar, c->d_B16, c->d_f16scale, c->d_partial, c->d_sc, c->st);
        HIPCHK(c, hipGetLastError());
        return SCFGP_OK;
    }
    static int pass3(scfgp_ctx* c) {
        const Geom& g = c->g;
        { ProfScope ps(c, "apply_phibar");
          const F16Operands f16 = c->f16ops();
          SK::apply_phibar(g, (const T*)c->d_Phi, (const T*)c->d_AbarT, (T*)c->d_V, c->d_p, c->d_q, c->d_y, c->alpha(), c->ut(), c->st, c->dma(),
                           c->f16_on() ? &f16 : nullptr);
          write_status(c->x3_scalars(), 0.0, 0.0, 0.0, 0.0, c->st); }
        const int ntm = c->Dpp / XT, ntn = g.Jp / XT;
        const int64_t chunk = c->dtype == SCFGP_F32 ? c->gram_chunk : 0;
        c->last_lrb = c->want_lrb();
        if (c->last_lrb) {
            ProfScope ps(c, "xtz");
            T* Zb = (T*)c->d_V; T* U = (T*)c->d_V + g.Jp;
            SK::zbar_inplace(g, (const T*)c->d_Phi, Zb, c->st);
            SK::rsel(g, c->d_params, (T*)c->d_AbarT, c->st);
            SK::apply_plain(g, Zb, (const T*)c->d_AbarT, U, g.J, g.S, c->st);
            const int nt1 = (c->Spp / XT) * ntn, xs1 = xtz_split(nt1, g.Np);
            SK::tn_plain(c->d_Tt, g.Sp, Zb, g.Kp, g.J, g.Np, xs1, chunk, c->d_slabs, c->st);
            reduce_full_tiles(c->d_slabs, xs1, c->Spp / XT, ntn, c->d_x3, g.Jp, c->st);
            const int nt2 = ntm * (c->Sq / XT), xs2 = xtz_split(nt2, g.Np);
            SK::tn_plain(c->d_Xt, g.Dp, U, g.Kp, g.S, g.Np, xs2, chunk, c->d_slabs, c->st);
            reduce_full_tiles(c->d_slabs, xs2, ntm, c->Sq / XT, c->x3_xu(), c->Sq, c->st);
            HIPCHK(c, hipGetLastError());
            return SCFGP_OK;
        }
        const int xs = c->xtz_nsplit > 0 ? (int)std::min<int64_t>(c->xtz_nsplit, g.Np / 64) : xtz_split(ntm * ntn, g.Np);
        { ProfScope ps(c, "xtz");
          SK::xtz(g, c->d_Xt, (const T*)c->d_Phi, (const T*)c->d_V, xs, chunk, c->d_slabs, c->st);
          reduce_full_tiles(c->d_slabs, xs, ntm, ntn, c->d_x3, g.Jp, c->st); }
        HIPCHK(c, hipGetLastError());
        return SCFGP_OK;
    }
};

#define DISPATCH(c, fn, ...) DISPATCH_TO(Impl, c, fn, __VA_ARGS__)

static int ready(scfgp_ctx* c) {
    if (!c) return SCFGP_EARG;
    if (!c->have_params || !c->have_data) { c->err = "parameters and data must be set first"; return SCFGP_EARG; }
    if (hipSetDevice(c->device) != hipSuccess) { c->err = "hipSetDevice failed"; return SCFGP_EHIP; }
    return SCFGP_OK;
}

static int restore_full_set(scfgp_ctx* c) {
    if (!c->have_data || c->work_full) return SCFGP_OK;
    return load_working_set(c, nullptr, c->Nstore, c->Nglobal_full);
}

static int comm_sum(scfgp_ctx* c, int stage, const char* name) {
    if (!c->comm) return SCFGP_OK;
    void* p = nullptr; int64_t n = 0;
    if (int rc = scfgp_exchange(c, stage, &p, &n)) return rc;
    ProfScope ps(c, name);
    const ncclResult_t r = rccl().all_reduce(p, p, (size_t)n, ncclFloat64, ncclSum, c->comm, c->st);
    if (r != ncclSuccess) { c->err = std::string("ncclAllReduce: ") + rccl().err_string(r); return SCFGP_EHIP; }
    return SCFGP_OK;
}

static int injected_failure(scfgp_ctx* c, int stage) {
    if (c->test_fail_stage != stage) return SCFGP_OK;
    c->test_fail_stage = 0;
    c->err = "pass" + std::to_string(stage) + ": injected failure (option test_fail_stage)";
    return SCFGP_EHIP;
}

static int settle_level(scfgp_ctx* c) {
    if (!c->unsettled || c->dtype != SCFGP_F32 || c->gram64 != 2) { c->unsettled = false; return SCFGP_OK; }
    double xs[8];
    HIPCHK(c, hipMemcpyAsync(xs, c->xs1(), sizeof(xs), hipMemcpyDeviceToHost, c->st));
    HIPCHK(c, hipStreamSynchronize(c->st));
    c->unsettled = false;
    const int agreed = xs[XS_CAP1] > 0.5 ? 0 : (xs[XS_CAP2] > 0.5 ? 1 : 2);
    if (agreed < c->cap()) {
        c->esc_denied = agreed + 1;
        c->err = "precision level " + std::to_string(agreed + 1) + " refused on another rank; every rank stays at level " + std::to_string(agreed) + " or below";
    }
    if (c->esc_level > agreed) {
        c->esc_level = agreed;
        if (c->gexec) { hipGraphExecDestroy(c->gexec); c->gexec = nullptr; }
        if (c->graph) { hipGraphDestroy(c->graph); c->graph = nullptr; }
        c->warm = false;
    }
    if (agreed < 1 && xs[XS_RAN1] > 0.5) { c->stage = 0; return SCFGP_REDO; }
    c->last_cform = c->want_cform(); c->last_level = c->level();
    return SCFGP_OK;
}

extern "C" int scfgp_pass1(scfgp_ctx* c) {
    if (int rc = ready(c)) return rc;
    if (int rc = restore_full_set(c)) return rc;
    if (c->prof) { c->recs.clear(); c->pool_used = 0; }
    if (int rc = injected_failure(c, 1)) return rc;
    if (int rc = DISPATCH(c, pass1, c)) return rc;
    c->stage = 1;
    return comm_sum(c, 1, "exchange1");
}
extern "C" int scfgp_factor(scfgp_ctx* c) {
    if (int rc = ready(c)) return rc;
    if (c->stage != 1) { c->err = "factor: call pass1 first"; return SCFGP_EARG; }
    if (int rc = settle_level(c)) return rc;
    if (int rc = DISPATCH(c, factor, c)) return rc;
    if (!g_scfgp_capturing) HIPCHK(c, hipEventRecord(c->ev_factor, c->st));
    c->stage = 2; return SCFGP_OK;
}
extern "C" int scfgp_pass2(scfgp_ctx* c, int want_grad) {
    if (int rc = ready(c)) return rc;
    if (c->stage != 2) { c->err = "pass2: call factor first"; return SCFGP_EARG; }
    if (int rc = injected_failure(c, 2)) return rc;
    if (int rc = DISPATCH(c, pass2, c, want_grad)) return rc;
    c->last_want_grad = want_grad; c->stage = 3;
    return comm_sum(c, 2, "exchange2");
}
extern "C" int scfgp_adjoint(scfgp_ctx* c) {
    if (int rc = ready(c)) return rc;
    if (c->stage != 3 || !c->last_want_grad) { c->err = "adjoint: call pass2(want_grad=1) first"; return SCFGP_EARG; }
    if (int rc = DISPATCH(c, adjoint, c)) return rc;
    c->stage = 4; return SCFGP_OK;
}
extern "C" int scfgp_pass3(scfgp_ctx* c) {
    if (int rc = ready(c)) return rc;
    if (c->stage != 4) { c->err = "pass3: call adjoint first"; return SCFGP_EARG; }
    if (int rc = injected_failure(c, 3)) return rc;
    if (int rc = DISPATCH(c, pass3, c)) return rc;
    c->stage = 5;
    return comm_sum(c, 3, "exchange3");
}

extern "C" int scfgp_fail_stage(scfgp_ctx* c, int stage, int want_grad) {
    if (!c || stage < 1 || stage > 3 || (stage == 3 && !want_grad)) return SCFGP_EARG;
    const std::string keep = c->err;
    if (hipSetDevice(c->device) != hipSuccess) return SCFGP_EHIP;
    c->last_want_grad = want_grad;
    double* xs = stage == 1 ? c->xs1() : (stage == 2 ? c->xs2() : c->x3_scalars());
    write_status(xs, 0.0, c->cap() < 1 ? 1.0 : 0.0, c->cap() < 2 ? 1.0 : 0.0, 1.0, c->st);
    const int rc = comm_sum(c, stage, stage == 1 ? "exchange1" : (stage == 2 ? "exchange2" : "exchange3"));
    c->stage = 0;
    if (rc == SCFGP_OK) c->err = keep;
    return rc;
}
static void fail_rest(scfgp_ctx* c, int want_grad) {
    const int st = c->stage, next = st < 1 ? 1 : (st < 3 ? 2 : (st < 5 ? 3 : 4));
    for (int s = next; s <= (want_grad ? 3 : 2); ++s)
        if (scfgp_fail_stage(c, s, want_grad) != SCFGP_OK) return;
}

extern "C" int scfgp_exchange(scfgp_ctx* c, int stage, void** dev_ptr, int64_t* count) {
    if (!c || !dev_ptr || !count) return SCFGP_EARG;
    if (stage == 1) { *dev_ptr = c->d_xp1; *count = c->n_xp; }
    else if (stage == 2) {
        if (c->last_want_grad) { *dev_ptr = c->d_xp2; *count = c->n_xp; }
        else { *dev_ptr = c->d_xp2 + c->n_pk + c->g.Kp; *count = 8; }
    }
    else if (stage == 3) { *dev_ptr = c->d_x3; *count = c->n_x3; }
    else return SCFGP_EARG;
    return SCFGP_OK;
}

extern "C" int scfgp_stream_fence(scfgp_ctx* c, void* peer_stream, int direction) {
    if (!c || (direction != 0 && direction != 1)) return SCFGP_EARG;
    HIPCHK(c, hipSetDevice(c->device));
    hipStream_t peer = (hipStream_t)peer_stream;
    if (peer == c->st) return SCFGP_OK;
    hipStream_t from = direction == 0 ? c->st : peer, to = direction == 0 ? peer : c->st;
    HIPCHK(c, hipEventRecord(c->ev_fence, from));
    HIPCHK(c, hipStreamWaitEvent(to, c->ev_fence, 0));
    return SCFGP_OK;
}

extern "C" int scfgp_fetch_factors(scfgp_ctx* c, double* alpha, double* Li) {
    if (int rc = ready(c)) return rc;
    if (c->stage < 2) { c->err = "fetch_factors: call factor first"; return SCFGP_EARG; }
    const Geom& g = c->g;
    const size_t K = (size_t)g.K;
    if (!c->h_pin) HIPCHK(c, hipHostMalloc((void**)&c->h_pin, sizeof(double) * (K * K + K), hipHostMallocDefault));
    HIPCHK(c, hipStreamWaitEvent(c->copy_st, c->ev_factor, 0));
    if (alpha) HIPCHK(c, hipMemcpyAsync(c->h_pin + K * K, c->alpha(), sizeof(double) * K, hipMemcpyDeviceToHost, c->copy_st));
    if (Li) HIPCHK(c, hipMemcpy2DAsync(c->h_pin, sizeof(double) * K, c->d_Li, sizeof(double) * g.Kp, sizeof(double) * K, K,
                                       hipMemcpyDeviceToHost, c->copy_st));
    HIPCHK(c, hipStreamSynchronize(c->copy_st));
    if (alpha) memcpy(alpha, c->h_pin + K * K, sizeof(double) * K);
    if (Li) memcpy(Li, c->h_pin, sizeof(double) * K * K);
    return SCFGP_OK;
}

static void enqueue_epilogue(scfgp_ctx* c, int want_grad) {
    const Geom& g = c->g;
    ProfScope ps(c, "epilogue");
    if (want_grad && c->last_lrb)
        grad_epilogue(g, c->d_params, c->d_F, nullptr, 0, c->d_work, c->d_scalars, c->Nglobal, c->d_grad, c->st, c->d_x3, g.Jp, c->x3_xu(), c->Sq);
    else
        grad_epilogue(g, c->d_params, c->d_F, c->d_x3, g.Jp, c->d_work, c->d_scalars, c->Nglobal, want_grad ? c->d_grad : nullptr, c->st);
    finalize_cost(g, c->d_sc, c->d_scalars, c->xs1(), c->xs2(), c->Nglobal, c->d_grad, want_grad, c->st);
}

static int update_level(scfgp_ctx* c, bool notpd, bool want_grad, bool may_redo = true) {
    if (c->dtype != SCFGP_F32 || c->gram64 != 2) return SCFGP_OK;
    const double est = c->cond_est();
    int want = notpd || !std::isfinite(est) ? 2 : c->want_level(est, 1.0);
    const int top = c->esc_denied > 0 ? std::min(want, c->esc_denied - 1) : want;
    if (top > c->esc_level) {
        const int old = c->esc_level;
        c->unsettled = true;
        for (int lvl = top; lvl > old; --lvl) {
            c->esc_level = lvl;
            if (!(c->test_deny_level > 0 && lvl >= c->test_deny_level) && ensure_aux_rows(c) == SCFGP_OK) break;
            if (c->test_deny_level > 0 && lvl >= c->test_deny_level) c->err = "refused by option test_deny_level";
            (void)hipGetLastError();
            c->esc_level = lvl - 1; c->esc_denied = lvl;
            c->err = "precision level " + std::to_string(lvl) + " refused (auxiliary row buffers could not be allocated); staying at level " +
                     std::to_string(lvl - 1) + ": " + c->err;
        }
    }
    want = top;
    if (may_redo && (want_grad ? want : std::min(want, 1)) > c->last_level) {
        if (c->gexec) { hipGraphExecDestroy(c->gexec); c->gexec = nullptr; }
        if (c->graph) { hipGraphDestroy(c->graph); c->graph = nullptr; }
        c->warm = false;
        if (int rc = ensure_aux_rows(c)) return rc;
        if (notpd) HIPCHK(c, hipMemsetAsync(c->d_flag, 0, sizeof(int) * 4, c->st));
        return SCFGP_REDO;
    }
    if ((c->use64() && c->phi64_cap < c->g.Np) || (c->want_cform() && c->c_cap < c->g.Np)) {
        if (c->gexec) { hipGraphExecDestroy(c->gexec); c->gexec = nullptr; }
        if (c->graph) { hipGraphDestroy(c->graph); c->graph = nullptr; }
        c->warm = false;
        if (int rc = ensure_aux_rows(c)) return rc;
    }
    if (!notpd) {
        const int keep = c->want_level(est, 0.25);
        if (keep < c->esc_level) {
            c->esc_level = keep;
            if (c->gexec) { hipGraphExecDestroy(c->gexec); c->gexec = nullptr; }
            if (c->graph) { hipGraphDestroy(c->graph); c->graph = nullptr; }
            c->warm = false;
        }
    }
    return SCFGP_OK;
}

extern "C" int scfgp_finish(scfgp_ctx* c, int want_grad, double* cost, double* grad, double* alpha, double* Li) {
    if (int rc = ready(c)) return rc;
    if ((want_grad && c->stage != 5) || (!want_grad && c->stage != 3)) { c->err = "finish: evaluation incomplete"; return SCFGP_EARG; }
    const Geom& g = c->g;
    enqueue_epilogue(c, want_grad);
    double h_cost = 0, h_fail[3] = {0, 0, 0}; int h_flag[4] = {0, 0, 0, 0};
    {
        ProfScope ps(c, "d2h");
        HIPCHK(c, hipMemcpyAsync(&h_fail[0], c->xs1() + XS_FAIL, sizeof(double), hipMemcpyDeviceToHost, c->st));
        HIPCHK(c, hipMemcpyAsync(&h_fail[1], c->xs2() + XS_FAIL, sizeof(double), hipMemcpyDeviceToHost, c->st));
        if (want_grad) HIPCHK(c, hipMemcpyAsync(&h_fail[2], c->x3_scalars() + XS_FAIL, sizeof(double), hipMemcpyDeviceToHost, c->st));
        HIPCHK(c, hipMemcpyAsync(&h_cost, c->d_scalars + R_COST, sizeof(double), hipMemcpyDeviceToHost, c->st));
        HIPCHK(c, hipMemcpyAsync(c->cond, c->d_scalars + R_LMIN2, sizeof(double) * 3, hipMemcpyDeviceToHost, c->st));
        HIPCHK(c, hipMemcpyAsync(h_flag, c->d_flag, sizeof(int) * 4, hipMemcpyDeviceToHost, c->st));
        if (want_grad && grad) HIPCHK(c, hipMemcpyAsync(grad, c->d_grad, sizeof(double) * g.P, hipMemcpyDeviceToHost, c->st));
        if (alpha) HIPCHK(c, hipMemcpyAsync(alpha, c->alpha(), sizeof(double) * g.K, hipMemcpyDeviceToHost, c->st));
        if (Li) HIPCHK(c, hipMemcpy2DAsync(Li, sizeof(double) * g.K, c->d_Li, sizeof(double) * g.Kp, sizeof(double) * g.K, g.K,
                                           hipMemcpyDeviceToHost, c->st));
    }
    HIPCHK(c, hipStreamSynchronize(c->st));
    HIPCHK(c, hipGetLastError());
    c->stage = 0; c->warm = true;
    if (cost) *cost = h_cost;
    if (h_fail[0] + h_fail[1] + h_fail[2] > 0.5) {
        c->cond_valid = false;
        c->err = "a rank failed in this evaluation (exchange 1 / 2 / 3: " + std::to_string((int)h_fail[0]) + " / " + std::to_string((int)h_fail[1]) +
                 " / " + std::to_string((int)h_fail[2]) + " ranks): its results are not valid on any rank";
        return SCFGP_EPEER;
    }
    if (int rc = update_level(c, h_flag[0] != 0, want_grad != 0)) return rc;
    c->cond_valid = true;
    if (h_flag[0]) { c->err = "Phi^T Phi + (e^{2a}+1e-6) I is not positive definite"; return SCFGP_ENOTPD; }
    if (!std::isfinite(h_cost)) { c->err = "non-finite cost"; return SCFGP_ENONFINITE; }
    return SCFGP_OK;
}

static int pass1_current(scfgp_ctx* c) {
    if (int rc = ready(c)) return rc;
    if (c->prof) { c->recs.clear(); c->pool_used = 0; }
    if (int rc = injected_failure(c, 1)) return rc;
    if (int rc = DISPATCH(c, pass1, c)) return rc;
    c->stage = 1;
    return comm_sum(c, 1, "exchange1");
}
static int run_eval(scfgp_ctx* c, int want_grad, double* cost, double* grad, double* alpha, double* Li, bool subset = false) {
    int rc = SCFGP_OK;
    const auto leave = [&](int code) { if (code < 0 && c->comm) fail_rest(c, want_grad); return code; };
    for (int attempt = 0; attempt < 5; ++attempt) {
        if ((rc = subset ? pass1_current(c) : scfgp_pass1(c))) return leave(rc);
        if ((rc = scfgp_factor(c)) == SCFGP_REDO) continue;
        if (rc) return leave(rc);
        if ((rc = scfgp_pass2(c, want_grad))) return leave(rc);
        if (want_grad) {
            if ((rc = scfgp_adjoint(c))) return leave(rc);
            if ((rc = scfgp_pass3(c))) return leave(rc);
        }
        if ((alpha || Li) && (rc = scfgp_fetch_factors(c, alpha, Li))) return rc;
        rc = scfgp_finish(c, want_grad, cost, grad, nullptr, nullptr);
        if (rc != SCFGP_REDO) return rc;
    }
    return rc;
}

extern "C" int scfgp_eval(scfgp_ctx* c, const double* X, const double* y, int64_t N, int want_grad,
                          double* cost, double* grad, double* alpha, double* Li) {
    if (!c) return SCFGP_EARG;
    int rc;
    if (X) { if ((rc = scfgp_set_data(c, X, y, N, N))) return rc; }
    return run_eval(c, want_grad, cost, grad, alpha, Li);
}

extern "C" int scfgp_eval_rows(scfgp_ctx* c, const int64_t* idx, int64_t n, int want_grad,
                               double* cost, double* grad, double* alpha, double* Li) {
    if (!c || !idx || n < 1) { if (c) c->err = "eval_rows: bad arguments"; return SCFGP_EARG; }
    if (!c->have_data || c->Nstore < 1) { c->err = "eval_rows: no resident data set"; return SCFGP_EARG; }
    for (int64_t i = 0; i < n; ++i)
        if (idx[i] < 0 || idx[i] >= c->Nstore) { c->err = "eval_rows: index out of range"; return SCFGP_EARG; }
    HIPCHK(c, hipSetDevice(c->device));
    if (n > c->idx_cap) {
        HIPCHK(c, hipStreamSynchronize(c->st));
        dfree(c->d_idx);
        if (int rc = dmalloc(c, &c->d_idx, sizeof(int64_t) * n)) return rc;
        c->idx_cap = n;
    }
    HIPCHK(c, hipMemcpyAsync(c->d_idx, idx, sizeof(int64_t) * n, hipMemcpyHostToDevice, c->st));
    if (int rc = load_working_set(c, c->d_idx, n, n)) return rc;
    return run_eval(c, want_grad, cost, grad, alpha, Li, true);
}

extern "C" int scfgp_opt_init(scfgp_ctx* c, int algo, const double* hyper, int nhyper, double momentum) {
    if (!c || algo < 0 || algo > 5 || !hyper || nhyper < 4) { if (c) c->err = "opt_init: bad arguments"; return SCFGP_EARG; }
    HIPCHK(c, hipSetDevice(c->device));
    const int P = c->g.P;
    if (!c->d_opt) {
        if (int rc = dmalloc(c, &c->d_opt, sizeof(double) * 3 * P)) return rc;
        if (int rc = dmalloc(c, &c->d_tctr, sizeof(double) * 8)) return rc;
    }
    HIPCHK(c, hipMemsetAsync(c->d_opt, 0, sizeof(double) * 3 * P, c->st));
    HIPCHK(c, hipMemsetAsync(c->d_tctr, 0, sizeof(double) * 8, c->st));
    c->opt_algo = algo;
    c->opt_h = OptHyper{hyper[0], hyper[1], hyper[2], hyper[3], momentum};
    if (c->gexec) { hipGraphExecDestroy(c->gexec); c->gexec = nullptr; }
    if (c->graph) { hipGraphDestroy(c->graph); c->graph = nullptr; }
    HIPCHK(c, hipStreamSynchronize(c->st));
    return SCFGP_OK;
}

extern "C" int scfgp_opt_state(scfgp_ctx* c, int set, int which, double* buf) {
    if (!c || !buf || c->opt_algo < 0 || which < 0 || which > 3) return SCFGP_EARG;
    HIPCHK(c, hipSetDevice(c->device));
    double* dev = which == 3 ? c->d_tctr : c->d_opt + (int64_t)which * c->g.P;
    const size_t bytes = sizeof(double) * (which == 3 ? 1 : c->g.P);
    HIPCHK(c, hipStreamSynchronize(c->st));
    if (set) HIPCHK(c, hipMemcpy(dev, buf, bytes, hipMemcpyHostToDevice));
    else HIPCHK(c, hipMemcpy(buf, dev, bytes, hipMemcpyDeviceToHost));
    return SCFGP_OK;
}

extern "C" int scfgp_opt_step(scfgp_ctx* c, const double* grad, int P) {
    if (!c || !grad || P != c->g.P) { if (c) c->err = "opt_step: wrong gradient length"; return SCFGP_EARG; }
    if (c->opt_algo < 0 || !c->have_params) { c->err = "opt_step: call scfgp_set_params and scfgp_opt_init first"; return SCFGP_EARG; }
    if (c->stage != 0) { c->err = "opt_step: a staged evaluation is in progress (finish it first: its later stages would run on other parameters)"; return SCFGP_EARG; }
    HIPCHK(c, hipSetDevice(c->device));
    HIPCHK(c, hipMemcpyAsync(c->d_grad, grad, sizeof(double) * P, hipMemcpyHostToDevice, c->st));
    opt_update(c->opt_algo, c->opt_h, P, c->d_params, c->d_grad, c->d_opt, c->d_tctr, c->d_scalars, nullptr, 0, c->st);
    unpack_params(c->g, c->d_params, c->d_F, c->d_Fall, c->d_Lall, c->d_Rall, c->d_sc, c->st);
    HIPCHK(c, hipMemcpyAsync(c->h_params.data(), c->d_params, sizeof(double) * P, hipMemcpyDeviceToHost, c->st));
    HIPCHK(c, hipStreamSynchronize(c->st));
    HIPCHK(c, hipGetLastError());
    c->cond_valid = false;
    return SCFGP_OK;
}

static int enqueue_train_iter(scfgp_ctx* c) {
    int rc;
    c->stage = 0; c->last_want_grad = 1;
    if ((rc = injected_failure(c, 1))) return rc;
    if ((rc = DISPATCH(c, pass1, c))) return rc;
    c->stage = 1;
    if ((rc = comm_sum(c, 1, "exchange1"))) return rc;
    if ((rc = DISPATCH(c, factor, c))) return rc;
    c->stage = 2;
    if ((rc = injected_failure(c, 2))) return rc;
    if ((rc = DISPATCH(c, pass2, c, 1))) return rc;
    c->stage = 3;
    if ((rc = comm_sum(c, 2, "exchange2"))) return rc;
    if ((rc = DISPATCH(c, adjoint, c))) return rc;
    c->stage = 4;
    if ((rc = injected_failure(c, 3))) return rc;
    if ((rc = DISPATCH(c, pass3, c))) return rc;
    c->stage = 5;
    if ((rc = comm_sum(c, 3, "exchange3"))) return rc;
    enqueue_epilogue(c, 1);
    opt_update(c->opt_algo, c->opt_h, c->g.P, c->d_params, c->d_grad, c->d_opt, c->d_tctr, c->d_scalars, c->d_hist, c->hist_cap, c->st);
    unpack_params(c->g, c->d_params, c->d_F, c->d_Fall, c->d_Lall, c->d_Rall, c->d_sc, c->st);
    HIPCHK(c, hipGetLastError());
    return SCFGP_OK;
}

extern "C" int scfgp_train(scfgp_ctx* c, int n_iters, double* cost_hist, double* alpha, double* Li) {
    if (int rc = ready(c)) return rc;
    if (c->opt_algo < 0 || n_iters < 1) { c->err = "train: call scfgp_opt_init first"; return SCFGP_EARG; }
    if (int rc = restore_full_set(c)) return rc;
    if (!c->comm && c->Nglobal != c->g.N) {
        c->err = "train: the resident rows are a shard (n_global != N) but no communicator is attached (scfgp_comm_init); the "
                 "on-device loop needs the sums over ranks inside the library";
        return SCFGP_EARG;
    }
    const Geom& g = c->g;
    if (n_iters > c->hist_cap) {
        dfree(c->d_hist);
        if (int rc = dmalloc(c, &c->d_hist, sizeof(double) * n_iters)) return rc;
        c->hist_cap = n_iters;
        if (c->gexec) { hipGraphExecDestroy(c->gexec); c->gexec = nullptr; }
        if (c->graph) { hipGraphDestroy(c->graph); c->graph = nullptr; }
    }
    for (int round = 0; round < 5 && c->dtype == SCFGP_F32 && c->gram64 == 2 && (!c->cond_valid || c->unsettled); ++round) {
        int rc;
        c->stage = 0;
        if ((rc = injected_failure(c, 1)) || (rc = DISPATCH(c, pass1, c))) {
            if (c->comm) (void)scfgp_fail_stage(c, 1, 1);
            return rc;
        }
        c->stage = 1;
        if ((rc = comm_sum(c, 1, "exchange1"))) return rc;
        if ((rc = settle_level(c)) == SCFGP_REDO) continue;
        if (rc) return rc;
        if ((rc = DISPATCH(c, factor, c))) return rc;
        int h_flag[4] = {0, 0, 0, 0}; double h_fail = 0;
        HIPCHK(c, hipMemcpyAsync(c->cond, c->d_scalars + R_LMIN2, sizeof(double) * 3, hipMemcpyDeviceToHost, c->st));
        HIPCHK(c, hipMemcpyAsync(h_flag, c->d_flag, sizeof(int) * 4, hipMemcpyDeviceToHost, c->st));
        HIPCHK(c, hipMemcpyAsync(&h_fail, c->xs1() + XS_FAIL, sizeof(double), hipMemcpyDeviceToHost, c->st));
        HIPCHK(c, hipStreamSynchronize(c->st));
        c->stage = 0;
        if (h_fail > 0.5) { c->err = "train: a rank failed in the probe evaluation"; return SCFGP_EPEER; }
        if ((rc = update_level(c, h_flag[0] != 0, true, false))) return rc;
        c->cond_valid = true;
    }
    if (c->unsettled) { c->err = "train: the ranks' precision level did not settle"; return SCFGP_EHIP; }
    HIPCHK(c, hipMemsetAsync(c->d_flag, 0, sizeof(int) * 4, c->st));
    HIPCHK(c, hipMemsetAsync(c->d_tctr + 1, 0, sizeof(double), c->st));
    c->in_train = true;
    int rc = SCFGP_OK, done = 0;
    const bool graph_ok = c->use_graph && !c->prof && (!c->comm || c->use_graph >= 2);
    if (graph_ok && !c->warm) {
        rc = enqueue_train_iter(c); done = 1;
        if (rc == SCFGP_OK) c->warm = true;
    }
    if (rc == SCFGP_OK && graph_ok && done < n_iters) {
        if (!c->gexec || c->graph_N != g.N) {
            if (c->gexec) { hipGraphExecDestroy(c->gexec); c->gexec = nullptr; }
            if (c->graph) { hipGraphDestroy(c->graph); c->graph = nullptr; }
            hipError_t e = hipStreamBeginCapture(c->st, hipStreamCaptureModeThreadLocal);
            if (e == hipSuccess) {
                g_scfgp_capturing = true;
                rc = enqueue_train_iter(c);
                g_scfgp_capturing = false;
                e = hipStreamEndCapture(c->st, &c->graph);
                if (rc == SCFGP_OK && e == hipSuccess) e = hipGraphInstantiate(&c->gexec, c->graph, nullptr, nullptr, 0);
            }
            if (e != hipSuccess || rc != SCFGP_OK) {
                if (c->graph) { hipGraphDestroy(c->graph); c->graph = nullptr; }
                c->gexec = nullptr; (void)hipGetLastError(); rc = SCFGP_OK;
            } else c->graph_N = g.N;
        }
        if (c->gexec)
            for (; done < n_iters && rc == SCFGP_OK; ++done)
                if (hipGraphLaunch(c->gexec, c->st) != hipSuccess) { c->err = "hipGraphLaunch failed"; rc = SCFGP_EHIP; }
    }
    for (; done < n_iters && rc == SCFGP_OK; ++done) {
        if (c->prof) { c->recs.clear(); c->pool_used = 0; }
        rc = enqueue_train_iter(c);
    }
    c->in_train = false;
    if (rc != SCFGP_OK) {
        if (c->comm && rc < 0) {
            fail_rest(c, 1);
            for (; done < n_iters; ++done) { c->stage = 0; fail_rest(c, 1); }
        }
        c->stage = 0;
        return rc;
    }
    int h_flag[4] = {0, 0, 0, 0}; double h_fail[3] = {0, 0, 0};
    HIPCHK(c, hipMemcpyAsync(&h_fail[0], c->xs1() + XS_FAIL, sizeof(double), hipMemcpyDeviceToHost, c->st));
    HIPCHK(c, hipMemcpyAsync(&h_fail[1], c->xs2() + XS_FAIL, sizeof(double), hipMemcpyDeviceToHost, c->st));
    HIPCHK(c, hipMemcpyAsync(&h_fail[2], c->x3_scalars() + XS_FAIL, sizeof(double), hipMemcpyDeviceToHost, c->st));
    if (cost_hist) HIPCHK(c, hipMemcpyAsync(cost_hist, c->d_hist, sizeof(double) * n_iters, hipMemcpyDeviceToHost, c->st));
    HIPCHK(c, hipMemcpyAsync(c->h_params.data(), c->d_params, sizeof(double) * g.P, hipMemcpyDeviceToHost, c->st));
    HIPCHK(c, hipMemcpyAsync(h_flag, c->d_flag, sizeof(int) * 4, hipMemcpyDeviceToHost, c->st));
    if (alpha) HIPCHK(c, hipMemcpyAsync(alpha, c->alpha(), sizeof(double) * g.K, hipMemcpyDeviceToHost, c->st));
    if (Li) HIPCHK(c, hipMemcpy2DAsync(Li, sizeof(double) * g.K, c->d_Li, sizeof(double) * g.Kp, sizeof(double) * g.K, g.K,
                                       hipMemcpyDeviceToHost, c->st));
    HIPCHK(c, hipMemcpyAsync(c->cond, c->d_scalars + R_LMIN2, sizeof(double) * 3, hipMemcpyDeviceToHost, c->st));
    HIPCHK(c, hipStreamSynchronize(c->st));
    HIPCHK(c, hipGetLastError());
    c->stage = 0;
    if (h_fail[0] + h_fail[1] + h_fail[2] > 0.5) {
        c->cond_valid = false;
        c->err = "train: a rank failed; parameters and optimiser state of this call are not valid on any rank";
        return SCFGP_EPEER;
    }
    if (int rc = update_level(c, h_flag[0] != 0, true, false)) return rc;
    c->cond_valid = true;
    if (h_flag[0]) { c->err = "Phi^T Phi + (e^{2a}+1e-6) I is not positive definite"; return SCFGP_ENOTPD; }
    if (cost_hist) for (int i = 0; i < n_iters; ++i) if (!std::isfinite(cost_hist[i])) { c->err = "non-finite cost"; return SCFGP_ENONFINITE; }
    return SCFGP_OK;
}

extern "C" int scfgp_comm_unique_id(void* id128) {
    if (!id128) return SCFGP_EARG;
    if (!rccl().ok()) return SCFGP_EHIP;
    static_assert(sizeof(ncclUniqueId) == 128, "ncclUniqueId is 128 bytes");
    return rccl().get_id((ncclUniqueId*)id128) == ncclSuccess ? SCFGP_OK : SCFGP_EHIP;
}
extern "C" int scfgp_comm_init(scfgp_ctx* c, int nranks, int rank, const void* id128) {
    if (!c || !id128 || nranks < 1 || rank < 0 || rank >= nranks) { if (c) c->err = "comm_init: bad arguments"; return SCFGP_EARG; }
    if (c->comm) { c->err = "comm_init: this context already has a communicator"; return SCFGP_EARG; }
    if (!rccl().ok()) { c->err = "comm_init: librccl.so could not be loaded"; return SCFGP_EHIP; }
    HIPCHK(c, hipSetDevice(c->device));
    ncclUniqueId id; memcpy(&id, id128, sizeof(id));
    const ncclResult_t r = rccl().init_rank(&c->comm, nranks, id, rank);
    if (r != ncclSuccess) { c->comm = nullptr; c->err = std::string("ncclCommInitRank: ") + rccl().err_string(r); return SCFGP_EHIP; }
    c->comm_ranks = nranks; c->comm_rank = rank;
    if (c->gexec) { hipGraphExecDestroy(c->gexec); c->gexec = nullptr; }
    if (c->graph) { hipGraphDestroy(c->graph); c->graph = nullptr; }
    return SCFGP_OK;
}
extern "C" int scfgp_comm_destroy(scfgp_ctx* c) {
    if (!c) return SCFGP_EARG;
    if (c->comm) {
        HIPCHK(c, hipSetDevice(c->device));
        HIPCHK(c, hipStreamSynchronize(c->st));
        rccl().destroy(c->comm); c->comm = nullptr; c->comm_ranks = 0;
    }
    return SCFGP_OK;
}

extern "C" int scfgp_get_dims(scfgp_ctx* c, int64_t* out, int n) {
    if (!c || !out || n < 6) return SCFGP_EARG;
    out[0] = c->g.K; out[1] = c->g.Kp; out[2] = c->g.Jp; out[3] = c->g.Dp; out[4] = c->g.Np; out[5] = c->g.P;
    if (n >= 7) out[6] = c->g.tile;
    if (n >= 8) out[7] = c->have_data ? c->Nstore : 0;
    return SCFGP_OK;
}

extern "C" int scfgp_set_profiling(scfgp_ctx* c, int enable) {
    if (!c) return SCFGP_EARG;
    c->prof = enable != 0; c->recs.clear(); c->pool_used = 0;
    return SCFGP_OK;
}

extern "C" int scfgp_get_timings(scfgp_ctx* c, double* ms, const char** names, int n) {
    if (!c) return SCFGP_EARG;
    hipStreamSynchronize(c->st);
    int k = 0;
    for (const ProfRec& r : c->recs) {
        if (k >= n) break;
        float t = 0;
        if (hipEventElapsedTime(&t, r.e0, r.e1) != hipSuccess) t = -1;
        if (ms) ms[k] = t;
        if (names) names[k] = r.name.c_str();
        ++k;
    }
    return k;
}

static void derive_geom(Geom& g, int D, int S, int M) {
    g.D = D; g.S = S; g.M = M; g.J = S + M; g.K = 2 * g.J; g.P = 3 + D * S + M * S + S + M;
    g.Dp = (int)round_up(D + 1, 16); g.Jp = (int)round_up(g.J, XT);
    g.Sp = (int)round_up(S + 1, 16); g.lowrank = g.Sp < g.Dp;
    g.tile = 128;
    g.gfull = (int)(round_up(g.K, 64) / 128);
    g.gstrip = (int)(round_up(g.K, 64) / 64 % 2);
    g.Kp = (g.gfull + g.gstrip) * g.tile;
}
extern "C" int scfgp_selftest_row_splits(int D, int S, int M, int64_t N, int dtype, int nsplit, int taper) {
    if (D < 1 || S < 1 || M < 1 || N < 1) return SCFGP_EARG;
    Geom g{};
    derive_geom(g, D, S, M);
    g.N = N; g.Np = round_up(N, 256);
    const int jobs = dtype == SCFGP_F32 ? SweepKernels<float>::gram_jobs(g) : SweepKernels<double>::gram_jobs(g);
    const RowSplits rs = gram_row_splits(jobs, g.Np, dtype == SCFGP_F32, nsplit, taper);
    if (rs.nsplit < 1 || rs.nsplit != rs.groups * rs.per_group()) return 1;
    int64_t at = 0;
    for (int s = 0; s < rs.nsplit; ++s) {
        int64_t r0, r1; rs.range(s, r0, r1);
        if (r0 != at || r1 < r0 || r0 % rs.gran || r1 % rs.gran || (rs.gran != 64 && rs.gran != 256)) return 2;
        at = r1;
    }
    return at == g.Np ? 0 : 3;
}

extern "C" int scfgp_set_option(scfgp_ctx* c, const char* name, int64_t value) {
    if (!c || !name) return SCFGP_EARG;
    const std::string s(name);
    if (s == "gram_nsplit") c->gram_nsplit = (int)value;
    else if (s == "gram_taper") c->gram_taper = (int)value;
    else if (s == "apply_dma") { if (value < -1 || value > 2) { c->err = "apply_dma: -1 auto, 0 off, 1 = 128-wide tiles, 2 = 256-wide (fp32)"; return SCFGP_EARG; }
                                 c->apply_dma = (int)value; }
    else if (s == "gram_chunk") c->gram_chunk = value;
    else if (s == "f16_gram") c->f16gram = (int)value;
    else if (s == "lowrank_bwd") c->lowrank_bwd = (int)value;
    else if (s == "xtz_nsplit") c->xtz_nsplit = (int)value;
    else if (s == "use_graph") c->use_graph = (int)value;
    else if (s == "gram64") { if (value < 0 || value > 3) { c->err = "gram64: 0 never, 1 always level 1, 2 auto, 3 always level 2"; return SCFGP_EARG; }
                              c->gram64 = (int)value; c->esc_level = 0; c->esc_denied = 0; }
    else if (s == "factor_form") { if (value < -1 || value > 1) { c->err = "factor_form: -1 auto, 0 never, 1 always"; return SCFGP_EARG; } c->factor_form = (int)value; }
    else if (s == "cond_threshold") c->esc_thr = (double)value;
    else if (s == "cond_threshold_w") c->escw_thr = (double)value;
    else if (s == "roctx") c->roctx_on = value != 0;
    else if (s == "test_deny_level") { c->test_deny_level = (int)value; return SCFGP_OK; }
    else if (s == "test_pd_group") { c->test_pd_group = (int)value; return SCFGP_OK; }
    else if (s == "test_sobol_group") { c->test_sobol_group = (int)value; return SCFGP_OK; }
    else if (s == "test_fail_stage") { c->test_fail_stage = (int)value; return SCFGP_OK; }
    else { c->err = "unknown option " + s; return SCFGP_EARG; }
    c->warm = false; c->cond_valid = false;
    if (c->gexec) { hipGraphExecDestroy(c->gexec); c->gexec = nullptr; }
    if (c->graph) { hipGraphDestroy(c->graph); c->graph = nullptr; }
    if (c->have_data) return ensure_rows(c, c->g.N);
    return SCFGP_OK;
}

extern "C" int scfgp_get_condition(scfgp_ctx* c, double* out, int n) {
    if (!c || !out || n < 4) return SCFGP_EARG;
    const double v[9] = {c->cond_est(), (double)c->last_level, c->last_used64 ? 1.0 : 0.0, c->alpha_err_fp32(),
                         c->esc_thr, c->escw_thr, c->cond[0], c->cond[1], c->cond[2]};
    for (int i = 0; i < n && i < 9; ++i) out[i] = v[i];
    return SCFGP_OK;
}

extern "C" int64_t scfgp_debug_read(scfgp_ctx* c, const char* name, void* host, int64_t max_bytes) {
    if (!c || !name || !host) return SCFGP_EARG;
    const Geom& g = c->g;
    const std::string s(name);
    if (s == "chol_trace") { if (hipStreamSynchronize(c->st) != hipSuccess) return SCFGP_EHIP; return chol_trace_read(host, max_bytes); }
    if (s == "apply_trace") { if (hipStreamSynchronize(c->st) != hipSuccess) return SCFGP_EHIP; return apply_trace_read(host, max_bytes); }
    if (s == "trace") { if (hipStreamSynchronize(c->st) != hipSuccess) return SCFGP_EHIP; return trace_read(host, max_bytes); }
    const int64_t K2 = (int64_t)g.Kp * g.Kp;
    const size_t ts = c->tsize();
    const void* src = nullptr; int64_t bytes = 0;
    DevTmp tmp;
    if (s == "Phi") { src = c->d_Phi; bytes = ts * g.Np * g.Kp; }
    else if (s == "V") { src = c->d_V; bytes = ts * g.Np * g.Kp; }
    else if (s == "G") {
        if (dmalloc(c, &tmp.p, 8 * c->n_x1)) return SCFGP_EHIP;
        unpack_exchange(c, c->d_xp1, tmp.p); src = tmp.p; bytes = 8 * c->n_x1;
    }
    else if (s == "W") { if (c->stage == 3) unpack_exchange(c, c->d_xp2, c->d_x2); src = c->d_x2; bytes = 8 * c->n_x2; }
    else if (s == "XZ") { src = c->d_x3; bytes = 8 * c->n_x3; }
    else if (s == "Li") { src = c->d_Li; bytes = 8 * K2; }
    else if (s == "B") { src = c->d_B; bytes = 8 * K2; }
    else if (s == "Abar") { src = c->d_Abar; bytes = 8 * K2; }
    else if (s == "p") { src = c->d_p; bytes = 8 * g.Np; }
    else if (s == "q") { src = c->d_q; bytes = 8 * g.Np; }
    else if (s == "vecs") { src = c->d_vecs; bytes = 8 * 5 * g.Kp; }
    else if (s == "Fall") { src = c->d_Fall; bytes = 8 * (int64_t)g.Dp * g.Jp; }
    else if (s == "Lall") { src = c->d_Lall; bytes = 8 * (int64_t)g.Dp * round_up(g.Sp, 64); }
    else if (s == "Rall") { src = c->d_Rall; bytes = 8 * (int64_t)g.Sp * g.Jp; }
    else if (s == "Xt") { src = c->d_Xt; bytes = 8 * g.Np * g.Dp; }
    else if (s == "pXt") {
        if (!c->p_Xt || !c->p_rows) { c->err = "debug_read: pXt exists only after a posterior call"; return SCFGP_EARG; }
        src = c->p_Xt; bytes = 8 * c->p_rows * g.Dp;
    }
    else if (s == "scalars") { src = c->d_scalars; bytes = 8 * 32; }
    else if (s == "C") {
        if (!c->d_C || c->c_cap < g.Np || !c->last_cform) { c->err = "debug_read: C exists only after a pass 2 in the factor form (level 2)"; return SCFGP_EARG; }
        src = c->d_C; bytes = ts * g.Np * g.Kp;
    }
    else if (s == "Phi64") {
        if (!c->d_Phi64 || c->phi64_cap < g.Np) { c->err = "debug_read: Phi64 exists only in fp32 mode at a raised level"; return SCFGP_EARG; }
        src = c->d_Phi64; bytes = 8 * g.Np * g.Kp;
    }
    else if (s == "Tt") {
        if (!c->d_Tt) { c->err = "debug_read: Tt exists only where the projection goes through the S columns"; return SCFGP_EARG; }
        src = c->d_Tt; bytes = 8 * g.Np * g.Sp;
    }
    else if (s == "Phi16" || s == "V16g" || s == "qV16g" || s == "B16" || s == "f16scale" || s == "f16tmp") {
        if (!c->split16) { c->err = "debug_read: " + s + " exists in compute mode SCFGP_F16X3 only"; return SCFGP_EARG; }
        const int64_t plane = 4 * g.Np * g.Kp;
        if (s == "Phi16") { src = c->d_Phi16; bytes = plane; }
        else if (s == "V16g") { src = c->d_V16g; bytes = plane; }
        else if (s == "qV16g") { src = c->d_qV16g; bytes = plane; }
        else if (s == "B16") { src = c->d_B16; bytes = 4 * K2; }
        else if (s == "f16scale") { src = c->d_f16scale; bytes = sizeof(float) * 4; }
        else { src = c->d_f16tmp; bytes = sizeof(float) * 8; }
    }
    else { c->err = "debug_read: unknown buffer " + s; return SCFGP_EARG; }
    if (!src) return SCFGP_EARG;
    if (bytes > max_bytes) bytes = max_bytes;
    if (hipStreamSynchronize(c->st) != hipSuccess) return SCFGP_EHIP;
    if (hipMemcpy(host, src, bytes, hipMemcpyDeviceToHost) != hipSuccess) return SCFGP_EHIP;
    return bytes;
}
```

Baseline: 4.945.

## Stage apply epilogue's Phi/V tile reads through an async LDS image

Adds a variant of the fp32 256-wide DMA apply kernel for epilogues 0 and 1 that prefetches the Phi or V rows the epilogue needs into spare LDS with global_load_lds, double-buffered per row-group, instead of re-reading them from global memory after the MMA loop. The kernel body moves into a shared header so both variants compile from one source. The aim is to hide epilogue global-load latency behind the MMA tail. In exchange it uses more LDS per block, which can lower occupancy, and adds hand-written waitcnt/m0 assembly that is fragile. It is on by default through a new option.

After: 4.945. Within noise of the previous version (-0.0%).

```diff
diff --git a/scfgp_amd/csrc/api_ctx.h b/scfgp_amd/csrc/api_ctx.h
--- a/scfgp_amd/csrc/api_ctx.h
+++ b/scfgp_amd/csrc/api_ctx.h
@@ -108,6 +108,7 @@
     double *d_Li = nullptr, *d_B = nullptr, *d_T1 = nullptr, *d_T2 = nullptr, *d_Abar = nullptr;
     void *d_BT = nullptr, *d_AbarT = nullptr;
     int apply_dma = -1;
+    int apply_epi_lds = 1;
     double *d_vecs = nullptr;
     double *d_scalars = nullptr, *d_yy = nullptr; int* d_flag = nullptr;
     float* d_ws2 = nullptr;
diff --git a/scfgp_amd/csrc/apply.hip b/scfgp_amd/csrc/apply.hip
--- a/scfgp_amd/csrc/apply.hip
+++ b/scfgp_amd/csrc/apply.hip
@@ -81,7 +81,9 @@
     static constexpr int PRE = 2;
     static constexpr int WAVES_PER_EU = WAVES == 4 ? 2 : 4;
     typedef TileCfg<T, BM, BN, 16, 4, BN / WN, 16, true> Cfg;
-    static_assert(STAGE / 1024 % WAVES == 0 && LDS_BYTES <= 160 * 1024, "whole DMA instructions per wave; the ring fits the LDS");
+    static constexpr int EPI_AREA = EpiLdsImage::PIECES * EpiLdsImage::PIECE_BYTES, EPI_SPARE = ES == 4 && BN == 256 ? WAVES * EPI_AREA : 0;
+    static_assert(STAGE / 1024 % WAVES == 0 && LDS_BYTES + EPI_SPARE <= 160 * 1024, "whole DMA instructions per wave; the ring (and the image) fit the LDS");
+    static_assert(EPI_SPARE == 0 || (WAVES / 2 * EPI_AREA <= STAGE && 2 * WAVES / 4 * BM * 8 <= STAGE), "half the waves' areas, or the staging area, per ring slot");
     static __device__ __forceinline__ int swz(int x) {
         if constexpr (ES == 4) return (0x78 >> (2 * ((x >> 2) & 3))) & 3;
         else return (int)((0x6BEB08u >> (3 * ((x >> 1) & 7))) & 7);
@@ -91,176 +93,29 @@
               ((0x6BEB08u >> 12) & 7) == 6 && ((0x6BEB08u >> 15) & 7) == 7 && ((0x6BEB08u >> 18) & 7) == 2 && ((0x6BEB08u >> 21) & 7) == 3,
               "fp64 swizzle table");
 
+#define SCFGP_APPLY_DMA_ATTRS(T, BN) __global__ __launch_bounds__((64 * ApplyDma<T, BN>::WAVES)) \
+    __attribute__((amdgpu_waves_per_eu(ApplyDma<T, BN>::WAVES_PER_EU, ApplyDma<T, BN>::WAVES_PER_EU)))
 template <typename T, int EPI, int BN>
-__global__ __launch_bounds__((64 * ApplyDma<T, BN>::WAVES)) __attribute__((amdgpu_waves_per_eu(ApplyDma<T, BN>::WAVES_PER_EU, ApplyDma<T, BN>::WAVES_PER_EU)))
+SCFGP_APPLY_DMA_ATTRS(T, BN)
 void apply_dma_kernel(const T* __restrict__ Phi, const T* __restrict__ Bm, T* V,
                       double* __restrict__ vpart, const double* __restrict__ p, const double* __restrict__ q,
                       const double* __restrict__ y, const double* __restrict__ alpha, const double* __restrict__ ut,
                       int K, int Kp, int64_t Np, int njt, double* __restrict__ mu, int col0, int slot0, int64_t rb0) {
-    typedef ApplyDma<T, BN> D;
-    typedef typename D::Cfg Cfg;
-    typedef T half_t __attribute__((ext_vector_type(2)));
-    typedef std::integral_constant<int, 0> H0;
-    typedef std::integral_constant<int, 1> H1;
-    constexpr int DPW = D::DMA_PER_WAVE, NRD = Cfg::TM + Cfg::TN, NM = 2 * Cfg::TM * Cfg::TN, PRE = D::PRE;
-    static_assert(Cfg::TM == 4 && (Cfg::TN == 4 || Cfg::TN == 2), "fragment lists of the wait statements");
-    static_assert(PRE + DPW + NRD <= NM, "one fetch or read per MFMA behind the barrier");
-    SMEM_DECL;
-    char* smem = smem_raw;
-#ifdef SCFGP_TRACE
-    const unsigned long long tr_t0 = __builtin_amdgcn_s_memrealtime();
-#endif
-    const unsigned wid = xcd_remap(blockIdx.x, gridDim.x);
-    const int jt = EPI == 3 || EPI == 4 ? (int)((wid % njt + wid / njt) % njt) : (int)(wid % njt);
-    const int64_t rb = rb0 + wid / njt;
-    const int cbase = col0 + jt * D::BN;
-    const int lane = threadIdx.x & 63, wave = __builtin_amdgcn_readfirstlane(threadIdx.x >> 6);
-    const char* src[DPW]; unsigned loff[DPW]; int dst[DPW];
-#pragma unroll
-    for (int u = 0; u < DPW; ++u) {
-        const int t = wave * DPW + u, x0 = D::ROWS_PER_DMA * t, l = lane / D::CPR, c = (lane % D::CPR) ^ D::swz(x0 + l);
-        const int xb = x0 - D::BM, xcol = (xb & ~(D::WN - 1)) + Cfg::TN * (xb & 15) + ((xb >> 4) & (Cfg::TN - 1));
-        const T* rowp = x0 < D::BM ? Phi + (rb * D::BM + x0) * Kp : Bm + (int64_t)(cbase + xcol) * Kp;
-        src[u] = reinterpret_cast<const char*>(rowp) + (EPI == 4 ? (cbase / 16) * D::ROWB : 0);
-        loff[u] = (unsigned)((x0 < D::BM ? l : Cfg::TN * l) * Kp * D::ES + c * 16);
-        dst[u] = t * 1024;
-    }
-    const auto fetch_one = [&](auto uc, int slot) {
-        constexpr int u = decltype(uc)::value;
-        __builtin_amdgcn_global_load_lds((gbl_void*)(src[u] + loff[u]), (lds_void*)(smem + slot * D::STAGE + dst[u]), 16, 0, 0);
-        src[u] += D::ROWB;
-    };
-    const int i = lane & 15, qg = lane >> 4;
-    const int wm0 = (wave / Cfg::WGN) * Cfg::WM, wn0 = (wave % Cfg::WGN) * Cfg::WN;
-    const int hoff0 = sizeof(T) == 4 ? (((qg >> 1) ^ D::swz(i)) << 4) + 8 * (qg & 1) : ((2 * qg) ^ D::swz(i)) << 4;
-    const int hoff1 = sizeof(T) == 4 ? (((2 + (qg >> 1)) ^ D::swz(i)) << 4) + 8 * (qg & 1) : ((2 * qg + 1) ^ D::swz(i)) << 4;
-    const int ring = (int)(uintptr_t)smem, aoff = ring + (wm0 + i) * D::ROWB, boff = ring + D::BM * D::ROWB + (wn0 + i) * D::ROWB;
-    const int ra[2] = {aoff + hoff0, aoff + hoff1}, rbb[2] = {boff + hoff0, boff + hoff1};
-    half_t ha[2][Cfg::TM], hb[2][Cfg::TN];
-    typename Cfg::MTr::acc_t acc[Cfg::TM][Cfg::TN];
-    acc_zero<Cfg>(acc);
-    const int nst_all = (K + 15) / 16, nst_tri = (cbase + D::BN + 15) / 16;
-    const int nst = (EPI == 3 && nst_tri < nst_all ? nst_tri : nst_all) - (EPI == 4 ? cbase / 16 : 0);
-#define SCFGP_LDS_READ(dst, addr, off)                                                                              \
-    do {                                                                                                             \
-        if constexpr (sizeof(T) == 4) asm volatile("ds_read_b64 %0, %1 offset:%2" : "=v"(dst) : "v"(addr), "n"(off));   \
-        else asm volatile("ds_read_b128 %0, %1 offset:%2" : "=v"(dst) : "v"(addr), "n"(off));                           \
-    } while (0)
-    const auto read_one = [&](auto hc, auto rc, int stage) {
-        constexpr int h = decltype(hc)::value, R = decltype(rc)::value;
-        if constexpr (R < Cfg::TM) SCFGP_LDS_READ(ha[h][R], stage + ra[h], R * 16 * D::ROWB);
-        else SCFGP_LDS_READ(hb[h][R - Cfg::TM], stage + rbb[h], (R - Cfg::TM) * 16 * D::ROWB);
-    };
-#undef SCFGP_LDS_READ
-#define SCFGP_WAIT_FRAGS(what, h)                                                                                                   \
-    do {                                                                                                                            \
-        if constexpr (Cfg::TN == 4)                                                                                                 \
-            asm volatile("s_waitcnt " what : "+v"(ha[h][0]), "+v"(ha[h][1]), "+v"(ha[h][2]), "+v"(ha[h][3]),                        \
-                                             "+v"(hb[h][0]), "+v"(hb[h][1]), "+v"(hb[h][2]), "+v"(hb[h][3]) :: "memory");           \
-        else                                                                                                                        \
-            asm volatile("s_waitcnt " what : "+v"(ha[h][0]), "+v"(ha[h][1]), "+v"(ha[h][2]), "+v"(ha[h][3]),                        \
-                                             "+v"(hb[h][0]), "+v"(hb[h][1]) :: "memory");                                           \
-    } while (0)
-    const auto mfma_one = [&](auto hc, auto ic) {
-        constexpr int h = decltype(hc)::value, I = decltype(ic)::value, j = I / (Cfg::TM * Cfg::TN), tm = I / Cfg::TN % Cfg::TM, tn = I % Cfg::TN;
-        Cfg::MTr::mfma(acc[tm][tn], ha[h][tm][j], hb[h][tn][j]);
-        __builtin_amdgcn_sched_barrier(0);
-    };
-    const auto second_half_pre = [&]() { static_for<PRE>([&](auto ic) { mfma_one(H1(), ic); }); };
-    const auto second_half = [&](auto fc, int fslot, int next) {
-        static_for<NM - PRE>([&](auto ic) {
-            constexpr int I = decltype(ic)::value;
-            mfma_one(H1(), std::integral_constant<int, I + PRE>());
-            if constexpr (I < DPW) {
-                if constexpr (decltype(fc)::value) { fetch_one(ic, fslot); __builtin_amdgcn_sched_barrier(0); }
-            } else if constexpr (I - DPW < NRD) {
-                read_one(H0(), std::integral_constant<int, I - DPW>(), next);
-                __builtin_amdgcn_sched_barrier(0);
-            }
-        });
-    };
-    const auto first_half = [&](int next) {
-        static_for<NM>([&](auto ic) {
-            mfma_one(H0(), ic);
-            if constexpr (decltype(ic)::value < NRD) { read_one(H1(), ic, next); __builtin_amdgcn_sched_barrier(0); }
-        });
-    };
-    static_for<DPW>([&](auto uc) { fetch_one(uc, 0); });
-    if (nst > 1) static_for<DPW>([&](auto uc) { fetch_one(uc, 1); });
-    if (nst > 2) static_for<DPW>([&](auto uc) { fetch_one(uc, 2); });
-    if (nst > 2) asm volatile("s_waitcnt vmcnt(%0)" :: "n"(2 * DPW) : "memory");
-    else if (nst > 1) asm volatile("s_waitcnt vmcnt(%0)" :: "n"(DPW) : "memory");
-    else asm volatile("s_waitcnt vmcnt(0)" ::: "memory");
-    __builtin_amdgcn_s_barrier();
-    asm volatile("" ::: "memory");
-#ifdef SCFGP_TRACE
-    const unsigned long long tr_l0 = __builtin_amdgcn_s_memrealtime();
-#endif
-    static_for<NRD>([&](auto rc) { read_one(H0(), rc, 0); });
-    static_for<NRD>([&](auto rc) { read_one(H1(), rc, 0); });
-    SCFGP_WAIT_FRAGS("lgkmcnt(0)", 0);
-    __builtin_amdgcn_sched_barrier(0);
-    static_for<NM>([&](auto ic) { mfma_one(H0(), ic); });
-    int slot = 0, s = 0;
-    for (; s + 3 < nst; ++s) {
-        asm volatile("s_waitcnt vmcnt(%0)" :: "n"(DPW) : "memory");
-        SCFGP_WAIT_FRAGS("lgkmcnt(0)", 1);
-        __builtin_amdgcn_sched_barrier(0);
-        second_half_pre();
-        __builtin_amdgcn_s_barrier();
-        asm volatile("" ::: "memory");
-        const int fslot = slot;
-        slot = slot == 2 ? 0 : slot + 1;
-        __builtin_amdgcn_sched_barrier(0);
-        second_half(std::true_type(), fslot, slot * D::STAGE);
-        SCFGP_WAIT_FRAGS("lgkmcnt(0)", 0);
-        __builtin_amdgcn_sched_barrier(0);
-        first_half(slot * D::STAGE);
-    }
-    SCFGP_WAIT_FRAGS("lgkmcnt(0)", 1);
-    for (; s + 1 < nst; ++s) {
-        if (s + 2 < nst) asm volatile("s_waitcnt vmcnt(%0)" :: "n"(DPW) : "memory");
-        else asm volatile("s_waitcnt vmcnt(0)" ::: "memory");
-        SCFGP_WAIT_FRAGS("lgkmcnt(0)", 1);
-        __builtin_amdgcn_sched_barrier(0);
-        second_half_pre();
-        __builtin_amdgcn_s_barrier();
-        asm volatile("" ::: "memory");
-        slot = slot == 2 ? 0 : slot + 1;
-        __builtin_amdgcn_sched_barrier(0);
-        second_half(std::false_type(), 0, slot * D::STAGE);
-        SCFGP_WAIT_FRAGS("lgkmcnt(0)", 0);
-        __builtin_amdgcn_sched_barrier(0);
-        first_half(slot * D::STAGE);
-    }
-    SCFGP_WAIT_FRAGS("lgkmcnt(0)", 1);
-    __builtin_amdgcn_sched_barrier(0);
-    static_for<NM>([&](auto ic) { mfma_one(H1(), ic); });
-#undef SCFGP_WAIT_FRAGS
-    __syncthreads();
-#ifdef SCFGP_TRACE
-    const unsigned long long tr_l1 = __builtin_amdgcn_s_memrealtime();
-#endif
-    constexpr int SLOTS = BN >= 128 ? BN / 128 : 1;
-    const int vslot = slot0 + SLOTS * jt;
-    int tid = (int)threadIdx.x;
-    asm volatile("" : "+v"(tid));
-    apply_epilogue<Cfg, EPI, EPI == 0 || EPI == 3, true>(acc, Phi, V, vpart, p, q, y, alpha, ut, K, Kp, Np, rb, cbase, vslot, smem_raw, mu, tid);
-    if (SLOTS == 2 && (EPI == 0 || EPI == 3) && tid < D::BM) {
-        vpart[(int64_t)(vslot + 1) * Np + rb * D::BM + tid] = 0.0;
-        if (mu) mu[(int64_t)(vslot + 1) * Np + rb * D::BM + tid] = 0.0;
-    }
-#ifdef SCFGP_TRACE
-    __syncthreads();
-    if (threadIdx.x == 0 && blockIdx.x < ATRACE_CAP) {
-        unsigned long long* rec = g_atrace[EPI * ATRACE_CAP + blockIdx.x];
-        rec[0] = tr_t0; rec[1] = __builtin_amdgcn_s_memrealtime();
-        rec[2] = ((unsigned long long)__builtin_amdgcn_s_getreg((20 << 0) | (0 << 6) | (3 << 11)) & 0xF) | ((unsigned long long)jt << 8) |
-                                  ((unsigned long long)nst << 20);
-        rec[3] = tr_l0; rec[4] = tr_l1;
-    }
-#endif
-}
+    constexpr bool EPL = false;
+#include "apply_dma_body.h"
+}
+template <int EPI>
+SCFGP_APPLY_DMA_ATTRS(float, 256)
+void apply_epi_lds_kernel(const float* __restrict__ Phi, const float* __restrict__ Bm, float* V,
+                          double* __restrict__ vpart, const double* __restrict__ p, const double* __restrict__ q,
+                          const double* __restrict__ y, const double* __restrict__ alpha, const double* __restrict__ ut,
+                          int K, int Kp, int64_t Np, int njt, double* __restrict__ mu, int col0, int slot0, int64_t rb0) {
+    typedef float T;
+    constexpr int BN = 256;
+    constexpr bool EPL = true;
+#include "apply_dma_body.h"
+}
+#undef SCFGP_APPLY_DMA_ATTRS
 
 template <typename T> struct ApplyPlan {
     static constexpr int NW = 2;
@@ -304,6 +159,17 @@
                        Phi, Bm, V, vpart, p, q, y, alpha, ut, g.K, g.Kp, g.Np, njt, mu, col0, slot0, rb0);
     return (int)(njt * nrb);
 }
+template <int EPI>
+static int apply_epi_lds_launch(const Geom& g, int njt, const float* Phi, const float* Bm, float* V, double* vpart,
+                                const double* p, const double* q, const double* y, const double* alpha, const double* ut,
+                                double* mu, hipStream_t st, int64_t nrb) {
+    typedef ApplyDma<float, 256> D;
+    if (njt <= 0 || nrb <= 0) return 0;
+    allow_big_lds(apply_epi_lds_kernel<EPI>, D::LDS_BYTES + D::EPI_SPARE);
+    hipLaunchKernelGGL((apply_epi_lds_kernel<EPI>), dim3((unsigned)(njt * nrb)), dim3(64 * D::WAVES), D::LDS_BYTES + D::EPI_SPARE, st,
+                       Phi, Bm, V, vpart, p, q, y, alpha, ut, g.K, g.Kp, g.Np, njt, mu, 0, 0, (int64_t)0);
+    return (int)(njt * nrb);
+}
 static int apply_num_cus() {
     static int n = 0;
     if (n == 0) {
@@ -316,7 +182,7 @@
 template <typename T, int EPI>
 static int apply_launch(const Geom& g, const T* Phi, const T* Bm, T* V, double* vpart, const double* p, const double* q,
                         const double* y, const double* alpha, const double* ut, double* mu, hipStream_t st,
-                        int dma = 0, const T* BmT = nullptr, const F16Operands* f16 = nullptr) {
+                        int dma = 0, const T* BmT = nullptr, const F16Operands* f16 = nullptr, int epi_lds = 0) {
     if (!BmT) BmT = Bm;
     const ApplyPlan<T> pl(g.K);
     int nb = 0;
@@ -342,7 +208,11 @@
                     }
                     return nb;
                 }
-                nb += apply_dma_launch<T, EPI, 256>(g, n256, 0, 0, Phi, BmT, V, vpart, p, q, y, alpha, ut, mu, st, 0, nrb - tail_rb);
+                if constexpr (EPI == 0 || EPI == 1) {
+                    if (epi_lds) nb += apply_epi_lds_launch<EPI>(g, n256, Phi, BmT, V, vpart, p, q, y, alpha, ut, mu, st, nrb - tail_rb);
+                    else nb += apply_dma_launch<T, EPI, 256>(g, n256, 0, 0, Phi, BmT, V, vpart, p, q, y, alpha, ut, mu, st, 0, nrb - tail_rb);
+                } else
+                    nb += apply_dma_launch<T, EPI, 256>(g, n256, 0, 0, Phi, BmT, V, vpart, p, q, y, alpha, ut, mu, st, 0, nrb - tail_rb);
             }
             nb += apply_dma_launch<T, EPI, 128>(g, pl.count[0] - 2 * n256, 256 * n256, 2 * n256, Phi, BmT, V, vpart, p, q, y, alpha, ut, mu, st, 0, nrb - tail_rb);
             nb += apply_dma_launch<T, EPI, 64>(g, pl.count[1], pl.col0[1], pl.jt0[1], Phi, BmT, V, vpart, p, q, y, alpha, ut, mu, st, 0, nrb - tail_rb);
@@ -360,8 +230,8 @@
 
 template <typename T>
 void ApplyKernels<T>::apply_v(const Geom& g, const T* Phi, const T* Bm, T* V, double* vpart, const double* alpha, double* mu,
-                              hipStream_t st, int dma, const F16Operands* f16) {
-    apply_launch<T, 0>(g, Phi, Bm, V, vpart, nullptr, nullptr, nullptr, alpha, nullptr, mu, st, dma, nullptr, f16);
+                              hipStream_t st, int dma, const F16Operands* f16, int epi_lds) {
+    apply_launch<T, 0>(g, Phi, Bm, V, vpart, nullptr, nullptr, nullptr, alpha, nullptr, mu, st, dma, nullptr, f16, epi_lds);
 }
 template <typename T>
 void ApplyKernels<T>::apply_predict(const Geom& g, const T* Phi, const T* LiT, double* vpart, const double* alpha, double* mu,
@@ -387,8 +257,8 @@
 }
 template <typename T>
 void ApplyKernels<T>::apply_phibar(const Geom& g, const T* Phi, const T* Abar, T* V, const double* p, const double* q,
-                                   const double* y, const double* alpha, const double* ut, hipStream_t st, int dma, const F16Operands* f16) {
-    apply_launch<T, 1>(g, Phi, Abar, V, nullptr, p, q, y, alpha, ut, nullptr, st, dma, nullptr, f16);
+                                   const double* y, const double* alpha, const double* ut, hipStream_t st, int dma, const F16Operands* f16, int epi_lds) {
+    apply_launch<T, 1>(g, Phi, Abar, V, nullptr, p, q, y, alpha, ut, nullptr, st, dma, nullptr, f16, epi_lds);
 }
 
 template <typename T> static int apply_njt(const Geom& g) { return ApplyPlan<T>(g.K).total; }
diff --git a/scfgp_amd/csrc/apply_dma_body.h b/scfgp_amd/csrc/apply_dma_body.h
--- /dev/null
+++ b/scfgp_amd/csrc/apply_dma_body.h
@@ -0,0 +1,203 @@
+    typedef ApplyDma<T, BN> D;
+    static_assert(!EPL || (D::EPI_SPARE > 0 && (EPI == 0 || EPI == 1)), "the LDS image: fp32 256-wide tiles, epilogues 0 and 1");
+    typedef typename D::Cfg Cfg;
+    typedef T half_t __attribute__((ext_vector_type(2)));
+    typedef std::integral_constant<int, 0> H0;
+    typedef std::integral_constant<int, 1> H1;
+    constexpr int DPW = D::DMA_PER_WAVE, NRD = Cfg::TM + Cfg::TN, NM = 2 * Cfg::TM * Cfg::TN, PRE = D::PRE;
+    static_assert(Cfg::TM == 4 && (Cfg::TN == 4 || Cfg::TN == 2), "fragment lists of the wait statements");
+    static_assert(PRE + DPW + NRD <= NM, "one fetch or read per MFMA behind the barrier");
+    SMEM_DECL;
+    char* smem = smem_raw;
+#ifdef SCFGP_TRACE
+    const unsigned long long tr_t0 = __builtin_amdgcn_s_memrealtime();
+#endif
+    const unsigned wid = xcd_remap(blockIdx.x, gridDim.x);
+    const int jt = EPI == 3 || EPI == 4 ? (int)((wid % njt + wid / njt) % njt) : (int)(wid % njt);
+    const int64_t rb = rb0 + wid / njt;
+    const int cbase = col0 + jt * D::BN;
+    const int lane = threadIdx.x & 63, wave = __builtin_amdgcn_readfirstlane(threadIdx.x >> 6);
+    const char* src[DPW]; unsigned loff[DPW]; int dst[DPW];
+#pragma unroll
+    for (int u = 0; u < DPW; ++u) {
+        const int t = wave * DPW + u, x0 = D::ROWS_PER_DMA * t, l = lane / D::CPR, c = (lane % D::CPR) ^ D::swz(x0 + l);
+        const int xb = x0 - D::BM, xcol = (xb & ~(D::WN - 1)) + Cfg::TN * (xb & 15) + ((xb >> 4) & (Cfg::TN - 1));
+        const T* rowp = x0 < D::BM ? Phi + (rb * D::BM + x0) * Kp : Bm + (int64_t)(cbase + xcol) * Kp;
+        src[u] = reinterpret_cast<const char*>(rowp) + (EPI == 4 ? (cbase / 16) * D::ROWB : 0);
+        loff[u] = (unsigned)((x0 < D::BM ? l : Cfg::TN * l) * Kp * D::ES + c * 16);
+        dst[u] = t * 1024;
+    }
+    const auto fetch_one = [&](auto uc, int slot) {
+        constexpr int u = decltype(uc)::value;
+        __builtin_amdgcn_global_load_lds((gbl_void*)(src[u] + loff[u]), (lds_void*)(smem + slot * D::STAGE + dst[u]), 16, 0, 0);
+        src[u] += D::ROWB;
+    };
+    const int i = lane & 15, qg = lane >> 4;
+    const int wm0 = (wave / Cfg::WGN) * Cfg::WM, wn0 = (wave % Cfg::WGN) * Cfg::WN;
+    const int hoff0 = sizeof(T) == 4 ? (((qg >> 1) ^ D::swz(i)) << 4) + 8 * (qg & 1) : ((2 * qg) ^ D::swz(i)) << 4;
+    const int hoff1 = sizeof(T) == 4 ? (((2 + (qg >> 1)) ^ D::swz(i)) << 4) + 8 * (qg & 1) : ((2 * qg + 1) ^ D::swz(i)) << 4;
+    const int ring = (int)(uintptr_t)smem, aoff = ring + (wm0 + i) * D::ROWB, boff = ring + D::BM * D::ROWB + (wn0 + i) * D::ROWB;
+    const int ra[2] = {aoff + hoff0, aoff + hoff1}, rbb[2] = {boff + hoff0, boff + hoff1};
+    half_t ha[2][Cfg::TM], hb[2][Cfg::TN];
+    typename Cfg::MTr::acc_t acc[Cfg::TM][Cfg::TN];
+    acc_zero<Cfg>(acc);
+    const int nst_all = (K + 15) / 16, nst_tri = (cbase + D::BN + 15) / 16;
+    const int nst = (EPI == 3 && nst_tri < nst_all ? nst_tri : nst_all) - (EPI == 4 ? cbase / 16 : 0);
+#define SCFGP_LDS_READ(dst, addr, off)                                                                              \
+    do {                                                                                                             \
+        if constexpr (sizeof(T) == 4) asm volatile("ds_read_b64 %0, %1 offset:%2" : "=v"(dst) : "v"(addr), "n"(off));   \
+        else asm volatile("ds_read_b128 %0, %1 offset:%2" : "=v"(dst) : "v"(addr), "n"(off));                           \
+    } while (0)
+    const auto read_one = [&](auto hc, auto rc, int stage) {
+        constexpr int h = decltype(hc)::value, R = decltype(rc)::value;
+        if constexpr (R < Cfg::TM) SCFGP_LDS_READ(ha[h][R], stage + ra[h], R * 16 * D::ROWB);
+        else SCFGP_LDS_READ(hb[h][R - Cfg::TM], stage + rbb[h], (R - Cfg::TM) * 16 * D::ROWB);
+    };
+#undef SCFGP_LDS_READ
+#define SCFGP_WAIT_FRAGS(what, h)                                                                                                   \
+    do {                                                                                                                            \
+        if constexpr (Cfg::TN == 4)                                                                                                 \
+            asm volatile("s_waitcnt " what : "+v"(ha[h][0]), "+v"(ha[h][1]), "+v"(ha[h][2]), "+v"(ha[h][3]),                        \
+                                             "+v"(hb[h][0]), "+v"(hb[h][1]), "+v"(hb[h][2]), "+v"(hb[h][3]) :: "memory");           \
+        else                                                                                                                        \
+            asm volatile("s_waitcnt " what : "+v"(ha[h][0]), "+v"(ha[h][1]), "+v"(ha[h][2]), "+v"(ha[h][3]),                        \
+                                             "+v"(hb[h][0]), "+v"(hb[h][1]) :: "memory");                                           \
+    } while (0)
+    const auto mfma_one = [&](auto hc, auto ic) {
+        constexpr int h = decltype(hc)::value, I = decltype(ic)::value, j = I / (Cfg::TM * Cfg::TN), tm = I / Cfg::TN % Cfg::TM, tn = I % Cfg::TN;
+        Cfg::MTr::mfma(acc[tm][tn], ha[h][tm][j], hb[h][tn][j]);
+        __builtin_amdgcn_sched_barrier(0);
+    };
+    const auto second_half_pre = [&]() { static_for<PRE>([&](auto ic) { mfma_one(H1(), ic); }); };
+    typedef std::integral_constant<int, 2> EpiFetch;
+    constexpr int EPI_NPF = 2 * EpiLdsImage::PIECES;
+    static_assert(!EPL || NRD + EPI_NPF <= NM - PRE, "one piece per MFMA behind the barrier");
+    [[maybe_unused]] EpiLdsImage img{};
+    [[maybe_unused]] int earea[2];
+    const auto epi_fetch = [&](auto nc) {
+        constexpr int n = decltype(nc)::value, tm = n / EpiLdsImage::PIECES, r = n % EpiLdsImage::PIECES;
+        __builtin_amdgcn_global_load_lds((gbl_void*)(img.g + (16 * tm + r) * img.rowb + img.loff),
+                                         (lds_void*)(smem + earea[tm] + r * EpiLdsImage::PIECE_BYTES), 16, 0, 0);
+        __builtin_amdgcn_sched_barrier(0);
+    };
+    const auto second_half = [&](auto fc, int fslot, int next) {
+        static_for<NM - PRE>([&](auto ic) {
+            constexpr int I = decltype(ic)::value, FC = (int)decltype(fc)::value;
+            mfma_one(H1(), std::integral_constant<int, I + PRE>());
+            if constexpr (I < DPW) {
+                if constexpr (FC == 1) { fetch_one(ic, fslot); __builtin_amdgcn_sched_barrier(0); }
+                else if constexpr (FC == 2) epi_fetch(ic);
+            } else if constexpr (I - DPW < NRD) {
+                read_one(H0(), std::integral_constant<int, I - DPW>(), next);
+                __builtin_amdgcn_sched_barrier(0);
+            } else if constexpr (FC == 2 && I - NRD < EPI_NPF)
+                epi_fetch(std::integral_constant<int, I - NRD>());
+        });
+    };
+    const auto first_half = [&](int next) {
+        static_for<NM>([&](auto ic) {
+            mfma_one(H0(), ic);
+            if constexpr (decltype(ic)::value < NRD) { read_one(H1(), ic, next); __builtin_amdgcn_sched_barrier(0); }
+        });
+    };
+    static_for<DPW>([&](auto uc) { fetch_one(uc, 0); });
+    if (nst > 1) static_for<DPW>([&](auto uc) { fetch_one(uc, 1); });
+    if (nst > 2) static_for<DPW>([&](auto uc) { fetch_one(uc, 2); });
+    if (nst > 2) asm volatile("s_waitcnt vmcnt(%0)" :: "n"(2 * DPW) : "memory");
+    else if (nst > 1) asm volatile("s_waitcnt vmcnt(%0)" :: "n"(DPW) : "memory");
+    else asm volatile("s_waitcnt vmcnt(0)" ::: "memory");
+    __builtin_amdgcn_s_barrier();
+    asm volatile("" ::: "memory");
+#ifdef SCFGP_TRACE
+    const unsigned long long tr_l0 = __builtin_amdgcn_s_memrealtime();
+#endif
+    static_for<NRD>([&](auto rc) { read_one(H0(), rc, 0); });
+    static_for<NRD>([&](auto rc) { read_one(H1(), rc, 0); });
+    SCFGP_WAIT_FRAGS("lgkmcnt(0)", 0);
+    __builtin_amdgcn_sched_barrier(0);
+    static_for<NM>([&](auto ic) { mfma_one(H0(), ic); });
+    int slot = 0, s = 0;
+    for (; s + 3 < nst; ++s) {
+        asm volatile("s_waitcnt vmcnt(%0)" :: "n"(DPW) : "memory");
+        SCFGP_WAIT_FRAGS("lgkmcnt(0)", 1);
+        __builtin_amdgcn_sched_barrier(0);
+        second_half_pre();
+        __builtin_amdgcn_s_barrier();
+        asm volatile("" ::: "memory");
+        const int fslot = slot;
+        slot = slot == 2 ? 0 : slot + 1;
+        __builtin_amdgcn_sched_barrier(0);
+        second_half(std::true_type(), fslot, slot * D::STAGE);
+        SCFGP_WAIT_FRAGS("lgkmcnt(0)", 0);
+        __builtin_amdgcn_sched_barrier(0);
+        first_half(slot * D::STAGE);
+    }
+    SCFGP_WAIT_FRAGS("lgkmcnt(0)", 1);
+    for (; s + (EPL ? 2 : 1) < nst; ++s) {
+        if (s + 2 < nst) asm volatile("s_waitcnt vmcnt(%0)" :: "n"(DPW) : "memory");
+        else asm volatile("s_waitcnt vmcnt(0)" ::: "memory");
+        SCFGP_WAIT_FRAGS("lgkmcnt(0)", 1);
+        __builtin_amdgcn_sched_barrier(0);
+        second_half_pre();
+        __builtin_amdgcn_s_barrier();
+        asm volatile("" ::: "memory");
+        slot = slot == 2 ? 0 : slot + 1;
+        __builtin_amdgcn_sched_barrier(0);
+        second_half(std::false_type(), 0, slot * D::STAGE);
+        SCFGP_WAIT_FRAGS("lgkmcnt(0)", 0);
+        __builtin_amdgcn_sched_barrier(0);
+        first_half(slot * D::STAGE);
+    }
+    if constexpr (EPL) {
+        asm volatile("s_waitcnt vmcnt(0)" ::: "memory");
+        SCFGP_WAIT_FRAGS("lgkmcnt(0)", 1);
+        __builtin_amdgcn_sched_barrier(0);
+        second_half_pre();
+        __builtin_amdgcn_s_barrier();
+        asm volatile("" ::: "memory");
+        slot = slot == 2 ? 0 : slot + 1;
+        const int fs = slot + 1 + wave / (D::WAVES / 2);
+        earea[0] = D::LDS_BYTES + wave * D::EPI_AREA;
+        earea[1] = (fs >= 3 ? fs - 3 : fs) * D::STAGE + wave % (D::WAVES / 2) * D::EPI_AREA;
+        img.g = reinterpret_cast<const char*>((EPI == 0 ? Phi : V) + (rb * D::BM + wm0) * Kp + cbase + wn0);
+        img.rowb = (int64_t)Kp * D::ES;
+        img.loff = (unsigned)((4 * qg * Kp + 4 * i) * D::ES);
+        img.lds[0] = ring + earea[0]; img.lds[1] = ring + earea[1];
+        __builtin_amdgcn_sched_barrier(0);
+        second_half(EpiFetch(), 0, slot * D::STAGE);
+        SCFGP_WAIT_FRAGS("lgkmcnt(0)", 0);
+        __builtin_amdgcn_sched_barrier(0);
+        first_half(slot * D::STAGE);
+        ++s;
+    }
+    SCFGP_WAIT_FRAGS("lgkmcnt(0)", 1);
+    __builtin_amdgcn_sched_barrier(0);
+    static_for<NM>([&](auto ic) { mfma_one(H1(), ic); });
+#undef SCFGP_WAIT_FRAGS
+    if constexpr (EPL) asm volatile("s_waitcnt vmcnt(0)" ::: "memory");
+    __syncthreads();
+#ifdef SCFGP_TRACE
+    const unsigned long long tr_l1 = __builtin_amdgcn_s_memrealtime();
+#endif
+    constexpr int SLOTS = BN >= 128 ? BN / 128 : 1;
+    const int vslot = slot0 + SLOTS * jt;
+    int tid = (int)threadIdx.x;
+    asm volatile("" : "+v"(tid));
+    if constexpr (EPL)
+        apply_epilogue<Cfg, EPI, EPI == 0, true, EpiLdsImage>(acc, Phi, V, vpart, p, q, y, alpha, ut, K, Kp, Np, rb, cbase, vslot, smem_raw + slot * D::STAGE, mu, tid, img);
+    else
+        apply_epilogue<Cfg, EPI, EPI == 0 || EPI == 3, true>(acc, Phi, V, vpart, p, q, y, alpha, ut, K, Kp, Np, rb, cbase, vslot, smem_raw, mu, tid);
+    if (SLOTS == 2 && (EPI == 0 || EPI == 3) && tid < D::BM) {
+        vpart[(int64_t)(vslot + 1) * Np + rb * D::BM + tid] = 0.0;
+        if (mu) mu[(int64_t)(vslot + 1) * Np + rb * D::BM + tid] = 0.0;
+    }
+#ifdef SCFGP_TRACE
+    __syncthreads();
+    if (threadIdx.x == 0 && blockIdx.x < ATRACE_CAP) {
+        unsigned long long* rec = g_atrace[EPI * ATRACE_CAP + blockIdx.x];
+        rec[0] = tr_t0; rec[1] = __builtin_amdgcn_s_memrealtime();
+        rec[2] = ((unsigned long long)__builtin_amdgcn_s_getreg((20 << 0) | (0 << 6) | (3 << 11)) & 0xF) | ((unsigned long long)jt << 8) |
+                                  ((unsigned long long)nst << 20);
+        rec[3] = tr_l0; rec[4] = tr_l1;
+    }
+#endif
diff --git a/scfgp_amd/csrc/apply_epilogue.h b/scfgp_amd/csrc/apply_epilogue.h
--- a/scfgp_amd/csrc/apply_epilogue.h
+++ b/scfgp_amd/csrc/apply_epilogue.h
@@ -102,13 +102,50 @@
         }
     }
 }
-template <class Cfg, int EPI, bool MU = false, bool VEC4 = false>
+struct EpiGlobal { static constexpr bool ON = false; };
+struct EpiLdsImage {
+    static constexpr bool ON = true;
+    static constexpr int PIECES = 4, ROWS = 4, PIECE_BYTES = 1024;
+    const char* g;
+    int64_t rowb;
+    unsigned loff;
+    int lds[2];
+    __device__ __forceinline__ void refill(int tm) const {
+        const char* b = g + 16 * tm * rowb;
+        const int a = lds[tm & 1];
+        unsigned keep;
+        asm volatile("s_mov_b32 %0, m0\n\t"
+                     "s_mov_b32 m0, %6\n\ts_nop 0\n\tglobal_load_lds_dwordx4 %1, %2\n\t"
+                     "s_mov_b32 m0, %7\n\ts_nop 0\n\tglobal_load_lds_dwordx4 %1, %3\n\t"
+                     "s_mov_b32 m0, %8\n\ts_nop 0\n\tglobal_load_lds_dwordx4 %1, %4\n\t"
+                     "s_mov_b32 m0, %9\n\ts_nop 0\n\tglobal_load_lds_dwordx4 %1, %5\n\t"
+                     "s_mov_b32 m0, %0"
+                     : "=&s"(keep)
+                     : "v"(loff), "s"(b), "s"(b + rowb), "s"(b + 2 * rowb), "s"(b + 3 * rowb),
+                       "s"(a), "s"(a + PIECE_BYTES), "s"(a + 2 * PIECE_BYTES), "s"(a + 3 * PIECE_BYTES)
+                     : "memory");
+    }
+    __device__ __forceinline__ void take(int tm, int lane, v4f (&x)[4]) const {
+        static_assert(PIECES == 4 && ROWS == 4, "the four reads and the four fetches below");
+        if (tm == 0) __builtin_amdgcn_s_waitcnt(0x0F70);
+        if (tm == 2) asm volatile("s_waitcnt vmcnt(%0)" ::"n"(PIECES + 2 * ROWS) : "memory");
+        if (tm == 3) asm volatile("s_waitcnt vmcnt(%0)" ::"n"(2 * ROWS) : "memory");
+        const int a = lds[tm & 1] + 16 * lane;
+        asm volatile("ds_read_b128 %0, %4\n\tds_read_b128 %1, %4 offset:1024\n\tds_read_b128 %2, %4 offset:2048\n\t"
+                     "ds_read_b128 %3, %4 offset:3072\n\ts_waitcnt lgkmcnt(0)"
+                     : "=&v"(x[0]), "=&v"(x[1]), "=&v"(x[2]), "=&v"(x[3]) : "v"(a) : "memory");
+        if (tm < 2) refill(tm + 2);
+        __builtin_amdgcn_sched_barrier(0);
+    }
+};
+template <class Cfg, int EPI, bool MU = false, bool VEC4 = false, class Img = EpiGlobal>
 __device__ __forceinline__ void apply_epilogue(
     const typename Cfg::MTr::acc_t (&acc)[Cfg::TM][Cfg::TN], const typename Cfg::T* __restrict__ Phi, typename Cfg::T* V,
     double* __restrict__ vpart, const double* __restrict__ p, const double* __restrict__ q, const double* __restrict__ y,
     const double* __restrict__ alpha, const double* __restrict__ ut, int K, int Kp, int64_t Np, int64_t rb, int cbase, int jtg,
-    char* smem_raw, double* __restrict__ mupart = nullptr, int tid = (int)threadIdx.x) {
+    char* smem_raw, double* __restrict__ mupart = nullptr, int tid = (int)threadIdx.x, const Img img = Img()) {
     typedef typename Cfg::T T;
+    static_assert(!Img::ON || (VEC4 && sizeof(T) == 4 && (EPI == 0 || EPI == 1)), "the LDS image feeds the fp32 VEC4 epilogues 0 and 1");
     if constexpr (VEC4 && sizeof(T) == 8) {
         apply_epilogue_vec2<Cfg, EPI, MU>(acc, Phi, V, vpart, p, q, y, alpha, ut, K, Kp, Np, rb, cbase, jtg, smem_raw, mupart, tid);
         return;
@@ -135,10 +172,11 @@
             for (int tm = 0; tm < Cfg::TM; ++tm) {
                 v4f ph[4];
                 int64_t off[4];
+                if constexpr (Img::ON) img.take(tm, co.lane, ph);
 #pragma unroll
                 for (int r = 0; r < 4; ++r) {
                     off[r] = (rb * Cfg::BM + co.row(tm, r)) * Kp + jg;
-                    if (EPI == 0) ph[r] = *reinterpret_cast<const v4f*>(Phi + off[r]);
+                    if constexpr (!Img::ON) { if (EPI == 0) ph[r] = *reinterpret_cast<const v4f*>(Phi + off[r]); }
                 }
 #pragma unroll
                 for (int r = 0; r < 4; ++r) {
@@ -183,10 +221,11 @@
             for (int tm = 0; tm < Cfg::TM; ++tm) {
                 v4f vv[4];
                 int64_t off[4];
+                if constexpr (Img::ON) img.take(tm, co.lane, vv);
 #pragma unroll
                 for (int r = 0; r < 4; ++r) {
                     off[r] = (rb * Cfg::BM + co.row(tm, r)) * Kp + jg;
-                    vv[r] = *reinterpret_cast<const v4f*>(V + off[r]);
+                    if constexpr (!Img::ON) vv[r] = *reinterpret_cast<const v4f*>(V + off[r]);
                 }
 #pragma unroll
                 for (int r = 0; r < 4; ++r) {
diff --git a/scfgp_amd/csrc/kernels.h b/scfgp_amd/csrc/kernels.h
--- a/scfgp_amd/csrc/kernels.h
+++ b/scfgp_amd/csrc/kernels.h
@@ -68,14 +68,15 @@
 template <typename T>
 struct ApplyKernels {
     static void apply_v(const Geom& g, const T* Phi, const T* Bm, T* V, double* vpart, const double* alpha, double* mupart,
-                        hipStream_t st, int dma = 0, const F16Operands* f16 = nullptr);
+                        hipStream_t st, int dma = 0, const F16Operands* f16 = nullptr, int epi_lds = 0);
     static void apply_predict(const Geom& g, const T* Phi, const T* LiT, double* vpart, const double* alpha, double* mupart,
                               hipStream_t st);
     static void apply_c(const Geom& g, const T* Phi, const T* LiT, const T* Li, T* C, double* vpart, const double* alpha,
                         const double* beta, double* mupart, hipStream_t st, int dma = 0);
     static void apply_vc(const Geom& g, const T* C, const T* Li, const T* LiT, T* V, hipStream_t st, int dma = 0);
     static void apply_phibar(const Geom& g, const T* Phi, const T* Abar, T* V, const double* p, const double* q,
-                             const double* y, const double* alpha, const double* ut, hipStream_t st, int dma = 0, const F16Operands* f16 = nullptr);
+                             const double* y, const double* alpha, const double* ut, hipStream_t st, int dma = 0, const F16Operands* f16 = nullptr,
+                             int epi_lds = 0);
     static void apply_plain(const Geom& g, const T* A, const T* Bm, T* Out, int Kc, int ncols, hipStream_t st);
     static void rowstats(const Geom& g, const double* mupart, const double* vpart, const double* y,
                          const Scal* sc, double* p, double* q, double* partial, int nblocks, hipStream_t st);
diff --git a/scfgp_amd/csrc/scfgp_api.hip b/scfgp_amd/csrc/scfgp_api.hip
--- a/scfgp_amd/csrc/scfgp_api.hip
+++ b/scfgp_amd/csrc/scfgp_api.hip
@@ -358,7 +358,7 @@
             ProfScope ps(c, "apply_v");
             F16Operands f16 = c->f16ops();
             if (want_grad && c->f16_gram()) f16.V16 = c->d_V16g;
-            SK::apply_v(g, (const T*)c->d_Phi, (const T*)c->d_BT, (T*)c->d_V, c->d_vpart, c->alpha(), c->d_mu, c->st, c->dma(), c->f16_on() ? &f16 : nullptr);
+            SK::apply_v(g, (const T*)c->d_Phi, (const T*)c->d_BT, (T*)c->d_V, c->d_vpart, c->alpha(), c->d_mu, c->st, c->dma(), c->f16_on() ? &f16 : nullptr, c->apply_epi_lds);
         }
         const int nb = (int)std::min<int64_t>(g.Np / 4, 2048);
         { ProfScope ps(c, "rowstats");
@@ -387,7 +387,7 @@
         { ProfScope ps(c, "apply_phibar");
           const F16Operands f16 = c->f16ops();
           SK::apply_phibar(g, (const T*)c->d_Phi, (const T*)c->d_AbarT, (T*)c->d_V, c->d_p, c->d_q, c->d_y, c->alpha(), c->ut(), c->st, c->dma(),
-                           c->f16_on() ? &f16 : nullptr);
+                           c->f16_on() ? &f16 : nullptr, c->apply_epi_lds);
           write_status(c->x3_scalars(), 0.0, 0.0, 0.0, 0.0, c->st); }
         const int ntm = c->Dpp / XT, ntn = g.Jp / XT;
         const int64_t chunk = c->dtype == SCFGP_F32 ? c->gram_chunk : 0;
@@ -980,6 +980,8 @@
     else if (s == "gram_taper") c->gram_taper = (int)value;
     else if (s == "apply_dma") { if (value < -1 || value > 2) { c->err = "apply_dma: -1 auto, 0 off, 1 = 128-wide tiles, 2 = 256-wide (fp32)"; return SCFGP_EARG; }
                                  c->apply_dma = (int)value; }
+    else if (s == "apply_epi_lds") { if (value < 0 || value > 1) { c->err = "apply_epi_lds: 0 the epilogue re-reads its tile from global memory, 1 from an LDS image"; return SCFGP_EARG; }
+                                     c->apply_epi_lds = (int)value; }
     else if (s == "gram_chunk") c->gram_chunk = value;
     else if (s == "f16_gram") c->f16gram = (int)value;
     else if (s == "lowrank_bwd") c->lowrank_bwd = (int)value;
```
